# mFinn27/Template-Matching-and-Regression-MapReduce

Measured on AMD Instinct MI355X. Metric: images/sec (whole node) match+regress+NMS; % HBM/MFMA roofline at 1/2/4/8 GPU, higher is better.
Workload: dtype fp32; 1 GPU; config B: 64x SAM feats 256x64x64 (->128x128), 3 exemplars, templates 3x3-15x15, fp32, cls 0.1, IoU 0.5; config=B, images_per_gpu=64, exemplars=3, parallelism=dp1, decoder=split, decoder_precision=fp32

## Files before the change

include/tmr.h:

```cpp
#ifndef TMR_H_
#define TMR_H_

#include <stdint.h>

#ifdef __cplusplus
extern "C" {
#endif

#define TMR_ABI_VERSION 3

enum {
    TMR_OK = 0,
    TMR_E_INVALID = -1,
    TMR_E_HIP = -2,
    TMR_E_UNSUPPORTED = -3
};

enum { TMR_TEMPLATE_ROI_ALIGN = 0, TMR_TEMPLATE_PROTOTYPE = 1 };

typedef struct tmr_unit {
    int32_t image;
    int32_t type;
    int32_t ht, wt;
    float roi[4];
    int32_t pbox[4];
    int64_t tmpl_offset;
    int32_t row_offset;
    int32_t pad_;
} tmr_unit_t;

typedef struct tmr_peak_param {
    float thr;
    float scale_w, scale_h;
    int32_t mask;
    int32_t mode;
    int32_t pad_;
} tmr_peak_param_t;

int tmr_version(void);
const char *tmr_strerror(int rc);

enum {
    TMR_SIZE_TEMPLATE_SPLIT = 1,
    TMR_SIZE_HEADS_PARTIALS = 2,
    TMR_SIZE_XPACK = 3,
    TMR_SIZE_WPACK = 4,
    TMR_SIZE_ACC = 5,
    TMR_SIZE_NMS_WORK = 6,
    TMR_SIZE_STATS_WORK = 7,
    TMR_SIZE_GT_WORK = 8
};
int64_t tmr_size(int kind, int64_t d0, int64_t d1, int64_t d2, int64_t d3, int64_t d4, int64_t d5);

int tmr_upsample2x(const float *feat, int BC, int Hin, int Win, float *out, void *stream);

int tmr_templates(const float *f, int B, int C, int H, int W, const tmr_unit_t *units, int U,
                  int max_ht, int max_wt, float *templates, void *stream);

#define TMR_XCORR_AUTO 0
#define TMR_XCORR_VALU 1
#define TMR_XCORR_MFMA 2
typedef struct tmr_xcorr_args {
    const float *f;
    const float *templates;
    const tmr_unit_t *units;
    const int32_t *img_units;
    const float *scale;
    void *out;
    float *relu_out;
    float *work;
    float *out_absmax;
    const void *tmpl_split;
    int64_t total_rows;
    int32_t B, C, H, W;
    int32_t U, max_ht, max_wt;
    int32_t squeeze;
    int32_t algo, min_k, prec, out_bf16;
} tmr_xcorr_args_t;
int tmr_xcorr(const tmr_xcorr_args_t *args, void *stream);
#define TMR_XCORR_KERNEL_VALU 0
#define TMR_XCORR_KERNEL_ROWS15 1
#define TMR_XCORR_KERNEL_ROWS31 2
#define TMR_XCORR_KERNEL_MFMA 3
typedef struct tmr_xcorr_plan {
    int32_t kernel, band_rows, col_groups, out16;
} tmr_xcorr_plan_t;
int tmr_xcorr_plan(const tmr_xcorr_args_t *args, tmr_xcorr_plan_t *plan);
int tmr_template_split(const float *templates, const tmr_unit_t *units, int U, int C,
                       int64_t total_rows, int prec, void *out, void *stream);

int tmr_heads_reduce(const float *partials, int N, int tile_n, int U, int H, int W,
                     const float *head_bias, float *o, float *b, void *stream);

#define TMR_PREC_F16X3 0
#define TMR_PREC_BF16 1
#define TMR_PREC_F16 2
int tmr_absmax_rows(const float *x, int S, int64_t n, int accumulate, float *out, void *stream);
int tmr_scale_merge(const float *img_max, const float *unit_max, const int32_t *unit_image, int B, int U,
                    float *out_img, float *out_unit, void *stream);
#define TMR_XPACK_UPSAMPLE 1
#define TMR_XPACK_ONES 2
int tmr_split_xpack(const float *x, int S, int C, int H, int W, int up, int ks, int prec,
                    const float *xmax, int xmax_per_sample, void *out, void *stream);
int tmr_split_xpack16(const void *x, int S, int C, int H, int W, int ks, int prec, void *out,
                      void *stream);
int tmr_split_fold_proj(const float *wd, int N, int Cw, int Cp, int ks, const float *proj_w,
                        const float *proj_b, int Cin, float *out, void *stream);
int tmr_split_wpack(const float *w, int N, int C0, int C1, int ks, int prec, const float *wmax,
                    void *out, void *stream);
#define TMR_SPLIT_TILED_OUT 1
#define TMR_SPLIT_TILED_INIT 2
#define TMR_SPLIT_INIT_BCAST 4
#define TMR_SPLIT_OUT_BF16 8
#define TMR_SPLIT_INIT_BF16 16
#define TMR_SPLIT_XMAX_PER_UNIT 32
#define TMR_SPLIT_XMAX_PER_PIXEL 64
#define TMR_SPLIT_UNITS_PER_IMAGE_SHIFT 8
#define TMR_SPLIT_TILE_FIRST_SHIFT 16
#define TMR_SPLIT_TILE_COUNT_SHIFT 24
#define TMR_SPLIT_TILE_WINDOW(first, count) \
    (((first) << TMR_SPLIT_TILE_FIRST_SHIFT) | ((count) << TMR_SPLIT_TILE_COUNT_SHIFT))
int tmr_pixel_absmax(const float *x, int S, int C, int64_t HW, float *out, void *stream);
int tmr_split_conv(const void *xp0, int C0, const int32_t *unit_image, const void *xp1, int C1, int U,
                   int H, int W, int ks, int prec, const void *wpack, const float *wmax, const float *xmax,
                   const float *bias, int N, int leaky, const float *headw, const float *acc_init,
                   float *out, int flags, void *stream);

#define TMR_POINTS_TILE 64
int tmr_split_conv_points(const void *xp0, int C0, const int32_t *unit_image, const void *xp1, int C1, int U,
                          int H, int W, int ks, int prec, const void *wpack, const float *wmax, const float *xmax,
                          const float *bias, int N, int leaky, const float *headw, const float *head_bias,
                          const float *acc_init, const float *box, const int32_t *tiles, int ntiles, float *b,
                          int flags, void *stream);

int tmr_maxpool3x3(const float *x, int64_t planes, int H, int W, int mask9, float *out, void *stream);

#define TMR_PEAKS_PROB_SCRATCH 2
#define TMR_PEAKS_FIND_ONLY 8
#define TMR_PEAKS_DECODE_ONLY 16
int tmr_peaks_decode(const float *o, int input_is_prob, const float *reg, int U, int H, int W,
                     const tmr_peak_param_t *params, float *prob, float *logits, float *box,
                     float *ref, int32_t *counts, const void *exp_table, void *stream);

typedef struct tmr_gt_unit {
    int32_t image;
    int32_t pad_x, pad_y;
    int32_t mode;
    float scale_w, scale_h;
    int32_t pad_[2];
} tmr_gt_unit_t;
#define TMR_GT_ASSIGN 1
#define TMR_GT_LOSS 2
#define TMR_GT_GATHER 4
#define TMR_GT_ROWS 8
#define TMR_GT_SLICES 16
typedef struct tmr_gt_loss_args {
    const float *o;
    const float *reg;
    const float *boxes;
    const int32_t *box_off;
    const tmr_gt_unit_t *units;
    const void *exp_table;
    void *work;
    float *gt_map;
    int32_t *target;
    int32_t *counts;
    double *sums;
    const int64_t *samp_off;
    const int64_t *row_off;
    float *obj_out;
    float *label_out;
    float *rows_pred;
    float *rows_gt;
    double positive_threshold, negative_threshold;
    int64_t n_samples, n_rows;
    int32_t U, NI, H, W;
    int32_t G_total, min_boxes;
    int32_t last_level, focal;
    int32_t phase, pad_;
} tmr_gt_loss_args_t;
int tmr_gt_loss(const tmr_gt_loss_args_t *args, void *stream);

int tmr_nms(const float *logits, const float *box, const float *ref, const int32_t *counts,
            const int64_t *unit_off, const int32_t *seg_units, const int64_t *cand_off,
            const int64_t *nb_off,
            int G, int64_t total_cand, int64_t max_cand, int64_t sum_nb, double iou_threshold,
            float *out_logits, float *out_boxes, float *out_refs, int64_t *out_keep,
            int32_t *kept, void *work, void *stream);
#define TMR_NMS_SMALL 256
int tmr_nms_small(const float *logits, const float *box, const float *ref, const int32_t *counts,
                  const int64_t *unit_off, const int32_t *seg_units, int G, double iou_threshold,
                  float *out_logits, float *out_boxes, float *out_refs, int64_t *out_keep,
                  int32_t *kept, void *stream);

int tmr_feature_stats(const float *x, int B, int64_t n, void *work, double *out, void *stream);

int64_t tmr_exp_table_encode(const uint32_t *exc, int64_t n, uint8_t *out, int64_t cap);
int64_t tmr_exp_table_decode(const uint8_t *blob, int64_t nbytes, uint32_t *out, int64_t cap);

#ifdef __cplusplus
}
#endif
#endif
```

profiles/kernel_resources.py:

```python
import json
import os
import re
import subprocess
import sys
import tempfile

REPO = os.path.dirname(os.path.dirname(os.path.abspath(__file__)))
sys.path.insert(0, REPO)
from tmr_import import load_package

CSRC = os.path.join(REPO, "template-matching-and-regression-mapreduce_amd", "csrc")
OUT = os.path.join(REPO, "profiles", "points_kloop", "resources.json")
PRECS = {0: "F16X3", 1: "BF16", 2: "F16"}
PARENT = {
    "F16X3": {"vgprs": 256, "vgpr_spills": 146, "scratch_bytes_per_lane": 252, "occupancy": 2},
    "BF16": {"vgprs": 256, "vgpr_spills": 10, "scratch_bytes_per_lane": 44, "occupancy": 2},
    "F16": {"vgprs": 256, "vgpr_spills": 110, "scratch_bytes_per_lane": 204, "occupancy": 2},
}
FIELDS = {"VGPRs": "vgprs", "AGPRs": "agprs", "VGPRs Spill": "vgpr_spills", "SGPRs Spill": "sgpr_spills",
          "ScratchSize [bytes/lane]": "scratch_bytes_per_lane", "Occupancy [waves/SIMD]": "occupancy"}


def makefile_flags():
    var = {"EXTRA": ""}
    for line in open(os.path.join(CSRC, "Makefile")):
        m = re.match(r"^(\w+)\s*\??=\s*(.*)$", line.rstrip("\n"))
        if m and m.group(1) not in var:
            var[m.group(1)] = m.group(2)
    expand = lambda s: re.sub(r"\$\((\w+)\)", lambda m: expand(var.get(m.group(1), "")), s)
    return os.environ.get("HIPCC", expand(var["HIPCC"])), expand(var["FLAGS"]).split()


def remarks(hipcc, flags):
    with tempfile.TemporaryDirectory() as tmp:
        cmd = [hipcc, *flags, "--cuda-device-only", "-Rpass-analysis=kernel-resource-usage", "-c",
               os.path.join(CSRC, "conv_split.hip"), "-o", os.path.join(tmp, "conv_split.o")]
        return subprocess.run(cmd, check=True, capture_output=True, text=True).stderr


def parse(text):
    out, cur = {}, None
    for line in text.splitlines():
        m = re.search(r"remark: +([^:]+): (.*?) \[-Rpass-analysis", line)
        if not m:
            continue
        key, val = m.group(1).strip(), m.group(2).strip()
        if key == "Function Name":
            k = re.search(r"split_points_kernelILi3ELi(\d)EE", val)
            cur = out.setdefault(PRECS[int(k.group(1))], {}) if k else None
        elif cur is not None and key in FIELDS:
            cur[FIELDS[key]] = int(val)
    return out


def main():
    out_path = sys.argv[1] if len(sys.argv) > 1 else OUT
    hipcc, flags = makefile_flags()
    kernels = parse(remarks(hipcc, flags))
    assert sorted(kernels) == sorted(PRECS.values()), kernels
    load_package()
    from tmr_amd import buildinfo
    rec = {"kernel": "split_points_kernel<3, PREC>", "flags": flags, "source_digest": buildinfo.source_digest("heads"),
           "kernels": kernels, "parent": PARENT}
    os.makedirs(os.path.dirname(out_path), exist_ok=True)
    with open(out_path, "w") as f:
        json.dump(rec, f, indent=1)
        f.write("\n")
    for p, k in kernels.items():
        print(p, json.dumps(k))


if __name__ == "__main__":
    main()
```

profiles/points_crossover.py:

```python
import json
import os
import sys

import numpy as np
import torch

REPO = os.path.dirname(os.path.dirname(os.path.abspath(__file__)))
sys.path.insert(0, REPO)
import bench
from tmr_amd import synth

tmr = bench.tmr


def events(fn, reps=3):
    out = []
    for _ in range(reps):
        s, e = torch.cuda.Event(enable_timing=True), torch.cuda.Event(enable_timing=True)
        s.record()
        fn()
        e.record()
        e.synchronize()
        out.append(s.elapsed_time(e))
    return out


def measure(config):
    cfg = bench.CONFIGS[config]
    dev = torch.device("cuda", 0)
    H = W = 2 * cfg["hf"]
    prec = cfg.get("precision", "fp32")
    eng = tmr.TMREngine(synth.reference_state_dict(0, device=dev), tmr.PathConfig(precision=prec))
    eng.use_graphs = False
    eng.box_at_peaks = "always"
    B, E = cfg["batch"], cfg["E"]
    feats = torch.from_numpy(synth.sam_features(1000, B, bench.CIN, H // 2, W // 2)).to(dev)
    ex, _ = synth.exemplar_set(2000, B, E, H, W, cfg["kmin"], cfg["kmax"])
    eng.detect(feats, ex, cls_ths=cfg["cls"], iou_threshold=cfg["iou"])
    rec = {}
    points, dense = eng.box_at_points, eng.box_dense

    def both(box, tiles):
        rec["points_ms_all"] = events(lambda: points(box, tiles))
        rec["dense_ms_all"] = events(dense)
        rec["tiles"] = len(tiles)
        points(box, tiles)

    eng.box_at_points = both
    eng.detect(feats, ex, cls_ths=cfg["cls"], iou_threshold=cfg["iou"])
    torch.cuda.synchronize()
    assert eng.last_box_route == "points" and "tiles" in rec
    n, pixels = eng.last_points, B * E * H * W
    pm, dm = min(rec["points_ms_all"]), min(rec["dense_ms_all"])
    direct = eng.last_points_flops / (pm * 1e-3) / 1e12
    out = dict(points=n, pixels=pixels, fraction=n / pixels, tiles=rec["tiles"], points_ms=pm, dense_ms=dm,
               ns_per_point=pm * 1e6 / n, ns_per_pixel=dm * 1e6 / pixels,
               crossover=(dm / pixels) / (pm / n), points_direct_tflops=direct,
               points_executed_tflops=direct * bench.SPLIT_TERMS[prec],
               points_ms_all=rec["points_ms_all"], dense_ms_all=rec["dense_ms_all"])
    return out


def main():
    out_path = sys.argv[1]
    res = {}
    for c in sys.argv[2:] or ["B", "C", "D", "E"]:
        res[c] = measure(c)
        print(c, json.dumps({k: res[c][k] for k in ("points", "points_ms", "dense_ms", "crossover")}), flush=True)
        with open(out_path, "w") as f:
            json.dump(res, f, indent=1)
    assert all(np.isfinite(r["crossover"]) for r in res.values())


if __name__ == "__main__":
    main()
```

template-matching-and-regression-mapreduce_amd/_lib.py:

```python
from __future__ import annotations

import ctypes
import os
import threading

import numpy as np
import torch

_HERE = os.path.dirname(os.path.abspath(__file__))
LIB_PATH = os.path.join(_HERE, "libtmr.so")
if os.environ.get("TMR_LIB_VARIANT"):
    LIB_PATH = os.path.join(_HERE, "libtmr_%s.so" % os.environ["TMR_LIB_VARIANT"])
HEADER = os.path.join(os.path.dirname(_HERE), "include", "tmr.h")

_lock = threading.Lock()
_lib = None

UNIT_DTYPE = np.dtype({
    "names": ["image", "type", "ht", "wt", "roi", "pbox", "tmpl_offset", "row_offset", "pad_"],
    "formats": [np.int32, np.int32, np.int32, np.int32, (np.float32, 4), (np.int32, 4), np.int64,
                np.int32, np.int32],
    "offsets": [0, 4, 8, 12, 16, 32, 48, 56, 60],
    "itemsize": 64,
})
PEAK_DTYPE = np.dtype({
    "names": ["thr", "scale_w", "scale_h", "mask", "mode", "pad_"],
    "formats": [np.float32, np.float32, np.float32, np.int32, np.int32, np.int32],
    "offsets": [0, 4, 8, 12, 16, 20],
    "itemsize": 24,
})

GT_UNIT_DTYPE = np.dtype({
    "names": ["image", "pad_x", "pad_y", "mode", "scale_w", "scale_h", "pad_"],
    "formats": [np.int32, np.int32, np.int32, np.int32, np.float32, np.float32, (np.int32, 2)],
    "offsets": [0, 4, 8, 12, 16, 20, 24],
    "itemsize": 32,
})

TEMPLATE_ROI_ALIGN = 0
TEMPLATE_PROTOTYPE = 1

PREC_CODES = {"fp32": 0, "bf16": 1, "f16": 2}
SPLIT_TILED_OUT, SPLIT_TILED_INIT, SPLIT_INIT_BCAST = 1, 2, 4
SPLIT_OUT_BF16, SPLIT_INIT_BF16 = 8, 16
SPLIT_XMAX_PER_UNIT = 32
SPLIT_XMAX_PER_PIXEL = 64
PEAKS_PROB_SCRATCH = 2
SPLIT_UNITS_PER_IMAGE_SHIFT = 8
SPLIT_TILE_FIRST_SHIFT, SPLIT_TILE_COUNT_SHIFT = 16, 24
PEAKS_FIND_ONLY, PEAKS_DECODE_ONLY = 8, 16
POINTS_TILE = 64
XCORR_ALGOS = {"auto": 0, "valu": 1, "mfma": 2}
XPACK_UPSAMPLE, XPACK_ONES = 1, 2
SIZE_KINDS = {"template_split": 1, "heads_partials": 2, "xpack": 3, "wpack": 4, "acc": 5, "nms_work": 6,
              "stats_work": 7, "gt_work": 8}
GT_ASSIGN, GT_LOSS, GT_GATHER, GT_ROWS = 1, 2, 4, 8
GT_SLICES = 16
ABI_VERSION = 3

_P = ctypes.c_void_p
_I = ctypes.c_int
_L = ctypes.c_int64
_D = ctypes.c_double


class XcorrArgs(ctypes.Structure):
    _fields_ = [("f", _P), ("templates", _P), ("units", _P), ("img_units", _P), ("scale", _P), ("out", _P),
                ("relu_out", _P), ("work", _P), ("out_absmax", _P), ("tmpl_split", _P), ("total_rows", _L),
                ("B", ctypes.c_int32), ("C", ctypes.c_int32), ("H", ctypes.c_int32), ("W", ctypes.c_int32),
                ("U", ctypes.c_int32), ("max_ht", ctypes.c_int32), ("max_wt", ctypes.c_int32),
                ("squeeze", ctypes.c_int32), ("algo", ctypes.c_int32), ("min_k", ctypes.c_int32),
                ("prec", ctypes.c_int32), ("out_bf16", ctypes.c_int32)]


class XcorrPlan(ctypes.Structure):
    _fields_ = [("kernel", ctypes.c_int32), ("band_rows", ctypes.c_int32), ("col_groups", ctypes.c_int32),
                ("out16", ctypes.c_int32)]


XCORR_KERNELS = {0: "valu", 1: "rows15", 2: "rows31", 3: "mfma"}


class GtLossArgs(ctypes.Structure):
    _fields_ = [("o", _P), ("reg", _P), ("boxes", _P), ("box_off", _P), ("units", _P), ("exp_table", _P),
                ("work", _P), ("gt_map", _P), ("target", _P), ("counts", _P), ("sums", _P), ("samp_off", _P),
                ("row_off", _P), ("obj_out", _P), ("label_out", _P), ("rows_pred", _P), ("rows_gt", _P),
                ("positive_threshold", _D), ("negative_threshold", _D), ("n_samples", _L), ("n_rows", _L),
                ("U", ctypes.c_int32), ("NI", ctypes.c_int32), ("H", ctypes.c_int32), ("W", ctypes.c_int32),
                ("G_total", ctypes.c_int32), ("min_boxes", ctypes.c_int32), ("last_level", ctypes.c_int32),
                ("focal", ctypes.c_int32), ("phase", ctypes.c_int32), ("pad_", ctypes.c_int32)]


SIGNATURES = {
    "tmr_version": (_I, []),
    "tmr_strerror": (ctypes.c_char_p, [_I]),
    "tmr_upsample2x": (_I, [_P, _I, _I, _I, _P, _P]),
    "tmr_templates": (_I, [_P, _I, _I, _I, _I, _P, _I, _I, _I, _P, _P]),
    "tmr_size": (_L, [_I, _L, _L, _L, _L, _L, _L]),
    "tmr_xcorr": (_I, [ctypes.POINTER(XcorrArgs), _P]),
    "tmr_xcorr_plan": (_I, [ctypes.POINTER(XcorrArgs), ctypes.POINTER(XcorrPlan)]),
    "tmr_template_split": (_I, [_P, _P, _I, _I, _L, _I, _P, _P]),
    "tmr_heads_reduce": (_I, [_P, _I, _I, _I, _I, _I, _P, _P, _P, _P]),
    "tmr_absmax_rows": (_I, [_P, _I, _L, _I, _P, _P]),
    "tmr_scale_merge": (_I, [_P, _P, _P, _I, _I, _P, _P, _P]),
    "tmr_pixel_absmax": (_I, [_P, _I, _I, _L, _P, _P]),
    "tmr_split_xpack": (_I, [_P, _I, _I, _I, _I, _I, _I, _I, _P, _I, _P, _P]),
    "tmr_split_xpack16": (_I, [_P, _I, _I, _I, _I, _I, _I, _P, _P]),
    "tmr_split_fold_proj": (_I, [_P, _I, _I, _I, _I, _P, _P, _I, _P, _P]),
    "tmr_split_wpack": (_I, [_P, _I, _I, _I, _I, _I, _P, _P, _P]),
    "tmr_split_conv": (_I, [_P, _I, _P, _P, _I, _I, _I, _I, _I, _I, _P, _P, _P, _P, _I, _I, _P, _P, _P, _I,
                            _P]),
    "tmr_split_conv_points": (_I, [_P, _I, _P, _P, _I, _I, _I, _I, _I, _I, _P, _P, _P, _P, _I, _I, _P, _P, _P,
                                   _P, _P, _I, _P, _I, _P]),
    "tmr_peaks_decode": (_I, [_P, _I, _P, _I, _I, _I, _P, _P, _P, _P, _P, _P, _P, _P]),
    "tmr_maxpool3x3": (_I, [_P, _L, _I, _I, _I, _P, _P]),
    "tmr_nms": (_I, [_P, _P, _P, _P, _P, _P, _P, _P, _I, _L, _L, _L, _D, _P, _P, _P, _P, _P, _P, _P]),
    "tmr_nms_small": (_I, [_P, _P, _P, _P, _P, _P, _I, _D, _P, _P, _P, _P, _P, _P]),
    "tmr_feature_stats": (_I, [_P, _I, _L, _P, _P, _P]),
    "tmr_gt_loss": (_I, [ctypes.POINTER(GtLossArgs), _P]),
    "tmr_exp_table_encode": (_L, [_P, _L, _P, _L]),
    "tmr_exp_table_decode": (_L, [_P, _L, _P, _L]),
}


class MaskBoxesArgs(ctypes.Structure):
    _fields_ = [("masks", _P), ("logits", _P), ("iou", _P), ("scaler", _P), ("boxes", _P), ("refs", _P),
                ("logits_out", _P), ("work", _P), ("N", _L), ("h", ctypes.c_int32), ("w", ctypes.c_int32),
                ("H", ctypes.c_int32), ("W", ctypes.c_int32), ("mode", ctypes.c_int32), ("pad_", ctypes.c_int32)]


EXT_HEADER = os.path.join(os.path.dirname(_HERE), "include", "tmr_refine.h")
EXT_SIGNATURES = {
    "tmr_mask_boxes": (_I, [ctypes.POINTER(MaskBoxesArgs), _P]),
    "tmr_mask_boxes_plan": (_I, [ctypes.POINTER(MaskBoxesArgs), ctypes.POINTER(ctypes.c_int32),
                                 ctypes.POINTER(ctypes.c_int32), ctypes.POINTER(ctypes.c_int32)]),
}
REFINE_FORWARD, REFINE_SCALED = 0, 1
MASK_BOXES_WORK_PER_MASK = 16


class CocoMatchArgs(ctypes.Structure):
    _fields_ = [("det_off", _P), ("det_box", _P), ("det_area", _P), ("gt_off", _P), ("gt_box", _P),
                ("gt_area", _P), ("gt_crowd", _P), ("area_rng", _P), ("iou_thr", _P), ("dt_match", _P),
                ("dt_ignore", _P), ("gt_ignore", _P), ("gt_match", _P), ("sum_d", _L), ("sum_g", _L),
                ("I", ctypes.c_int32), ("A", ctypes.c_int32), ("T", ctypes.c_int32), ("max_d", ctypes.c_int32),
                ("max_g", ctypes.c_int32), ("pad_", ctypes.c_int32)]


class CocoMatchPlan(ctypes.Structure):
    _fields_ = [("variant", ctypes.c_int32), ("tile_cap", ctypes.c_int32), ("list_cap", ctypes.c_int32),
                ("threads", ctypes.c_int32), ("lds_bytes", ctypes.c_int32), ("blocks", ctypes.c_int32)]


COCO_HEADER = os.path.join(os.path.dirname(_HERE), "include", "tmr_coco.h")
COCO_SIGNATURES = {
    "tmr_coco_match": (_I, [ctypes.POINTER(CocoMatchArgs), _P]),
    "tmr_coco_match_plan": (_I, [ctypes.POINTER(CocoMatchArgs), ctypes.POINTER(CocoMatchPlan)]),
}
COCO_VARIANTS = {0: "lds", 1: "global"}
COCO_T_MAX, COCO_D_MAX, COCO_G_MAX = 16, 4096, 65536


class MaskHeadArgs(ctypes.Structure):
    _fields_ = [("src", _P), ("hyper", _P), ("w1", _P), ("w2", _P), ("wpack", _P), ("b1", _P), ("g", _P),
                ("beta", _P), ("b2", _P), ("masks", _P), ("N", _L), ("h", ctypes.c_int32), ("w", ctypes.c_int32),
                ("C", ctypes.c_int32), ("eps", ctypes.c_float)]


class MaskHeadPlan(ctypes.Structure):
    _fields_ = [("variant", ctypes.c_int32), ("tile_pixels", ctypes.c_int32), ("threads", ctypes.c_int32),
                ("lds_bytes", ctypes.c_int32), ("tiles", ctypes.c_int32), ("blocks", ctypes.c_int32)]


MASKHEAD_HEADER = os.path.join(os.path.dirname(_HERE), "include", "tmr_maskhead.h")
MASKHEAD_SIGNATURES = {
    "tmr_mask_head_prep": (_I, [ctypes.POINTER(MaskHeadArgs), _P]),
    "tmr_mask_head": (_I, [ctypes.POINTER(MaskHeadArgs), _P]),
    "tmr_mask_head_plan": (_I, [ctypes.POINTER(MaskHeadArgs), ctypes.POINTER(MaskHeadPlan)]),
}
MASK_HEAD_VARIANTS = {0: "mfma128"}
MASK_HEAD_WPACK_BYTES = 9 * 32768 + 64
MASK_HEAD_DIM = 256


class TwoWayPoolArgs(ctypes.Structure):
    _fields_ = [("keys", _P), ("pe", _P), ("qf", _P), ("ctx", _P), ("work", _P), ("N", _L), ("Nk", _L), ("P", _L),
                ("C", ctypes.c_int32), ("H", ctypes.c_int32), ("T", ctypes.c_int32), ("pad_", ctypes.c_int32)]


class TwoWayUpdateArgs(ctypes.Structure):
    _fields_ = [("keys_in", _P), ("pe", _P), ("A", _P), ("c", _P), ("B", _P), ("bo", _P), ("g", _P), ("beta", _P),
                ("keys_out", _P), ("N", _L), ("Nk", _L), ("P", _L), ("C", ctypes.c_int32), ("H", ctypes.c_int32),
                ("T", ctypes.c_int32), ("eps", ctypes.c_float)]


class TwoWayPlan(ctypes.Structure):
    _fields_ = [("variant", ctypes.c_int32), ("tile_pixels", ctypes.c_int32), ("chunk_pixels", ctypes.c_int32),
                ("chunks", ctypes.c_int32), ("threads", ctypes.c_int32), ("lds_bytes", ctypes.c_int32),
                ("blocks", ctypes.c_int32), ("pad_", ctypes.c_int32)]


TWOWAY_HEADER = os.path.join(os.path.dirname(_HERE), "include", "tmr_twoway.h")
TWOWAY_SIGNATURES = {
    "tmr_twoway_pool": (_I, [ctypes.POINTER(TwoWayPoolArgs), _P]),
    "tmr_twoway_update": (_I, [ctypes.POINTER(TwoWayUpdateArgs), _P]),
    "tmr_twoway_pool_plan": (_I, [ctypes.POINTER(TwoWayPoolArgs), ctypes.POINTER(TwoWayPlan)]),
    "tmr_twoway_update_plan": (_I, [ctypes.POINTER(TwoWayUpdateArgs), ctypes.POINTER(TwoWayPlan)]),
}
TWOWAY_VARIANTS = {0: "f32mfma"}
TWOWAY_DIM, TWOWAY_HEADS, TWOWAY_ROWS = 256, 8, 64
TWOWAY_POOL_CHUNK = 512


def twoway_pool_work_bytes(N: int, P: int) -> int:
    return N * ((P + TWOWAY_POOL_CHUNK - 1) // TWOWAY_POOL_CHUNK) * TWOWAY_ROWS * (TWOWAY_DIM + 2) * 4


class TMRError(RuntimeError):
    pass


def load() -> ctypes.CDLL:
    global _lib
    if _lib is not None:
        return _lib
    with _lock:
        if _lib is not None:
            return _lib
        if not os.path.exists(LIB_PATH):
            raise TMRError(
                f"libtmr.so not found at {LIB_PATH}; build it with "
                "`python -c 'import __graft_entry__ as g; g.build()'` (no CPU fallback exists)")
        lib = ctypes.CDLL(LIB_PATH)
        for name, (res, args) in (list(SIGNATURES.items()) + list(EXT_SIGNATURES.items())
                                  + list(COCO_SIGNATURES.items()) + list(MASKHEAD_SIGNATURES.items())
                                  + list(TWOWAY_SIGNATURES.items())):
            fn = getattr(lib, name)
            fn.restype = res
            fn.argtypes = args
        if lib.tmr_version() != ABI_VERSION:
            raise TMRError("libtmr.so ABI version mismatch")
        _lib = lib
        return lib


def split_tile_window(first: int, count: int) -> int:
    if not (0 <= first < 256 and 0 <= count < 128):
        raise TMRError("tile window out of range")
    return (first << SPLIT_TILE_FIRST_SHIFT) | (count << SPLIT_TILE_COUNT_SHIFT)


def split_tile_window_of(flags: int):
    return (flags >> SPLIT_TILE_FIRST_SHIFT) & 0xff, (flags >> SPLIT_TILE_COUNT_SHIFT) & 0x7f


def check(rc: int, what: str = "") -> None:
    if rc != 0:
        msg = load().tmr_strerror(rc).decode()
        raise TMRError(f"{what}: {msg} (rc={rc})" if what else msg)


def ptr(t) -> int | None:
    if t is None:
        return None
    if not t.is_cuda:
        raise TMRError("tmr_amd kernels run on the GPU only; got a CPU tensor")
    if not t.is_contiguous():
        raise TMRError("tmr_amd kernels need contiguous tensors")
    return t.data_ptr()


def stream(device=None) -> int:
    return torch.cuda.current_stream(device).cuda_stream


def call(name: str, *args) -> None:
    check(getattr(load(), name)(*args), name)


def size(kind: str, *dims) -> int:
    d = [int(x) for x in dims] + [0] * (6 - len(dims))
    n = int(load().tmr_size(SIZE_KINDS[kind], *d))
    if n < 0:
        raise TMRError(f"tmr_size({kind}, {dims}): invalid dimensions")
    return n


def _fill(struct, what: str, fields: dict):
    unknown = set(fields) - {n for n, _ in struct._fields_ if n != "pad_"}
    if unknown:
        raise TMRError(f"{what} has no field(s) {sorted(unknown)}")
    a = struct()
    for k, v in fields.items():
        if v is not None:
            setattr(a, k, v)
    return a


def xcorr(stream=None, **fields) -> None:
    check(load().tmr_xcorr(ctypes.byref(_fill(XcorrArgs, "tmr_xcorr_args_t", fields)), stream), "tmr_xcorr")


def xcorr_plan_rc(**fields):
    plan = XcorrPlan()
    fields.pop("stream", None)
    rc = load().tmr_xcorr_plan(ctypes.byref(_fill(XcorrArgs, "tmr_xcorr_args_t", fields)), ctypes.byref(plan))
    if rc != 0:
        return rc, None
    return rc, (XCORR_KERNELS[plan.kernel], plan.band_rows, plan.col_groups, plan.out16)


def xcorr_plan(**fields):
    rc, plan = xcorr_plan_rc(**fields)
    check(rc, "tmr_xcorr_plan")
    return plan


def gt_loss_args(**fields) -> GtLossArgs:
    return _fill(GtLossArgs, "tmr_gt_loss_args_t", fields)


def gt_loss(stream_=None, **fields) -> None:
    check(load().tmr_gt_loss(ctypes.byref(gt_loss_args(**fields)), stream_), "tmr_gt_loss")


def mask_boxes(stream_=None, **fields) -> None:
    check(load().tmr_mask_boxes(ctypes.byref(_fill(MaskBoxesArgs, "tmr_mask_boxes_args_t", fields)), stream_),
          "tmr_mask_boxes")


def mask_boxes_plan(**fields):
    out = [ctypes.c_int32() for _ in range(3)]
    check(load().tmr_mask_boxes_plan(ctypes.byref(_fill(MaskBoxesArgs, "tmr_mask_boxes_args_t", fields)),
                                     *(ctypes.byref(o) for o in out)), "tmr_mask_boxes_plan")
    return tuple(o.value for o in out)


def coco_match(stream_=None, **fields) -> None:
    check(load().tmr_coco_match(ctypes.byref(_fill(CocoMatchArgs, "tmr_coco_match_args_t", fields)), stream_),
          "tmr_coco_match")


def coco_match_plan_rc(**fields):
    plan = CocoMatchPlan()
    rc = load().tmr_coco_match_plan(ctypes.byref(_fill(CocoMatchArgs, "tmr_coco_match_args_t", fields)),
                                    ctypes.byref(plan))
    if rc != 0:
        return rc, None
    out = {n: getattr(plan, n) for n, _ in CocoMatchPlan._fields_}
    out["variant"] = COCO_VARIANTS[plan.variant]
    return rc, out


def coco_match_plan(**fields):
    rc, plan = coco_match_plan_rc(**fields)
    check(rc, "tmr_coco_match_plan")
    return plan


def mask_head_prep(stream_=None, **fields) -> None:
    check(load().tmr_mask_head_prep(ctypes.byref(_fill(MaskHeadArgs, "tmr_mask_head_args_t", fields)), stream_),
          "tmr_mask_head_prep")


def mask_head(stream_=None, **fields) -> None:
    check(load().tmr_mask_head(ctypes.byref(_fill(MaskHeadArgs, "tmr_mask_head_args_t", fields)), stream_),
          "tmr_mask_head")


def mask_head_plan_rc(**fields):
    plan = MaskHeadPlan()
    fields.setdefault("C", MASK_HEAD_DIM)
    rc = load().tmr_mask_head_plan(ctypes.byref(_fill(MaskHeadArgs, "tmr_mask_head_args_t", fields)),
                                   ctypes.byref(plan))
    if rc != 0:
        return rc, None
    out = {n: getattr(plan, n) for n, _ in MaskHeadPlan._fields_}
    out["variant"] = MASK_HEAD_VARIANTS[plan.variant]
    return rc, out


def mask_head_plan(**fields):
    rc, plan = mask_head_plan_rc(**fields)
    check(rc, "tmr_mask_head_plan")
    return plan


def _twoway_defaults(fields):
    fields.setdefault("C", TWOWAY_DIM)
    fields.setdefault("H", TWOWAY_HEADS)
    if "Nk" not in fields:
        fields["Nk"] = fields.get("N", 0) or 1
    return fields


def twoway_pool(stream_=None, **fields) -> None:
    a = _fill(TwoWayPoolArgs, "tmr_twoway_pool_args_t", _twoway_defaults(fields))
    check(load().tmr_twoway_pool(ctypes.byref(a), stream_), "tmr_twoway_pool")


def twoway_update(stream_=None, **fields) -> None:
    a = _fill(TwoWayUpdateArgs, "tmr_twoway_update_args_t", _twoway_defaults(fields))
    check(load().tmr_twoway_update(ctypes.byref(a), stream_), "tmr_twoway_update")


def _twoway_plan_rc(fn, struct, what, fields):
    plan = TwoWayPlan()
    rc = getattr(load(), fn)(ctypes.byref(_fill(struct, what, _twoway_defaults(fields))), ctypes.byref(plan))
    if rc != 0:
        return rc, None
    out = {n: getattr(plan, n) for n, _ in TwoWayPlan._fields_ if n != "pad_"}
    out["variant"] = TWOWAY_VARIANTS[plan.variant]
    return rc, out


def twoway_pool_plan_rc(**fields):
    return _twoway_plan_rc("tmr_twoway_pool_plan", TwoWayPoolArgs, "tmr_twoway_pool_args_t", fields)


def twoway_update_plan_rc(**fields):
    return _twoway_plan_rc("tmr_twoway_update_plan", TwoWayUpdateArgs, "tmr_twoway_update_args_t", fields)


def twoway_pool_plan(**fields):
    rc, plan = twoway_pool_plan_rc(**fields)
    check(rc, "tmr_twoway_pool_plan")
    return plan


def twoway_update_plan(**fields):
    rc, plan = twoway_update_plan_rc(**fields)
    check(rc, "tmr_twoway_update_plan")
    return plan


def require_gpu(t: torch.Tensor, name: str = "input") -> None:
    if not isinstance(t, torch.Tensor) or not t.is_cuda:
        raise TMRError(f"{name} must be a tensor on a HIP device (MI355X); no CPU path exists")
```

template-matching-and-regression-mapreduce_amd/csrc/conv_split.hip:

```cpp
#include <algorithm>
#include <type_traits>

#include "tmr_common.h"

namespace {

typedef _Float16 h8 __attribute__((ext_vector_type(8)));
typedef __bf16 b8 __attribute__((ext_vector_type(8)));
typedef float f32x4 __attribute__((ext_vector_type(4)));
typedef __bf16 b4 __attribute__((ext_vector_type(4)));
typedef __attribute__((address_space(3))) void *lds_ptr_t;


constexpr int BM = 128;
constexpr int TH = 16;
constexpr int TW = 32;
constexpr int LDS_KB = 160;
constexpr int PXG = 8, NG = 4;
constexpr int NWAVES = 8;
constexpr int NTHREADS = NWAVES * 64;
constexpr int WNS = (NWAVES == 8 || TH == 8) ? 2 : 1;
static_assert(TH == 4 * NWAVES / WNS, "a wave owns 4 output rows");
constexpr int NIN = 8 / WNS;
constexpr int ACCW = NIN * 8 * 64 * 4;
constexpr int NHEAD = 5;
constexpr int CCH = 32;
constexpr int P = 4;
constexpr int XREC = 64;
constexpr int WPL = BM * 16;

template <int PREC> struct Prec;
template <> struct Prec<TMR_PREC_F16X3> {
    static constexpr int HALVES = 2;
    static constexpr int WREC = 128;
    static constexpr bool SCALED = true;
    typedef _Float16 E;
    typedef h8 V;
};
template <> struct Prec<TMR_PREC_BF16> {
    static constexpr int HALVES = 1;
    static constexpr int WREC = 64;
    static constexpr bool SCALED = false;
    typedef __bf16 E;
    typedef b8 V;
};
template <> struct Prec<TMR_PREC_F16> {
    static constexpr int HALVES = 1;
    static constexpr int WREC = 64;
    static constexpr bool SCALED = true;
    typedef _Float16 E;
    typedef h8 V;
};

__device__ __forceinline__ float split_scale(const float *m) {
    if (!m) return 1.0f;
    const float v = *m;
    if (!(v > 0.0f && v <= 3.0e38f)) return 1.0f;
    int e;
    frexpf(v, &e);
    return ldexpf(1.0f, min(max(14 - e, -63), 63));
}

__device__ __forceinline__ void wait_vmcnt(int n) {
    switch (n) {
        case 0: asm volatile("s_waitcnt vmcnt(0)" ::: "memory"); break;
        case 1: asm volatile("s_waitcnt vmcnt(1)" ::: "memory"); break;
        case 2: asm volatile("s_waitcnt vmcnt(2)" ::: "memory"); break;
        case 3: asm volatile("s_waitcnt vmcnt(3)" ::: "memory"); break;
        case 4: asm volatile("s_waitcnt vmcnt(4)" ::: "memory"); break;
        case 5: asm volatile("s_waitcnt vmcnt(5)" ::: "memory"); break;
        case 6: asm volatile("s_waitcnt vmcnt(6)" ::: "memory"); break;
        case 7: asm volatile("s_waitcnt vmcnt(7)" ::: "memory"); break;
        case 8: asm volatile("s_waitcnt vmcnt(8)" ::: "memory"); break;
        case 9: asm volatile("s_waitcnt vmcnt(9)" ::: "memory"); break;
        case 10: asm volatile("s_waitcnt vmcnt(10)" ::: "memory"); break;
        case 11: asm volatile("s_waitcnt vmcnt(11)" ::: "memory"); break;
        default: asm volatile("s_waitcnt vmcnt(12)" ::: "memory"); break;
    }
}

__device__ __forceinline__ void buffer_lds16(__amdgpu_buffer_rsrc_t r, lds_ptr_t dst, int voff, int soff) {
    __builtin_amdgcn_raw_ptr_buffer_load_lds(r, dst, 16, voff, soff, 0, 0);
}

template <typename V>
__device__ __forceinline__ V buffer_load16(__amdgpu_buffer_rsrc_t r, uint32_t voff, uint32_t soff) {
    return __builtin_bit_cast(V, __builtin_amdgcn_raw_buffer_load_b128(r, (int)voff, (int)soff, 0));
}

__device__ __forceinline__ f32x4 mma(h8 a, h8 b, f32x4 c) {
    return __builtin_amdgcn_mfma_f32_16x16x32_f16(a, b, c, 0, 0, 0);
}
__device__ __forceinline__ f32x4 mma(b8 a, b8 b, f32x4 c) {
    return __builtin_amdgcn_mfma_f32_16x16x32_bf16(a, b, c, 0, 0, 0);
}

template <int PREC>
__device__ __forceinline__ void split_record(const float (&v)[CCH], float s,
                                             typename Prec<PREC>::V (&hi)[P],
                                             typename Prec<PREC>::V (&lo)[P]) {
    typedef typename Prec<PREC>::E E;
#pragma unroll
    for (int g = 0; g < P; ++g)
#pragma unroll
        for (int j = 0; j < 8; ++j) {
            const float xs = v[g * 8 + j] * s;
            const E h = (E)xs;
            hi[g][j] = h;
            if (Prec<PREC>::HALVES == 2) lo[g][j] = (E)(xs - (float)h);
        }
}

constexpr int WH_BITS = 8;

template <int PREC>
__device__ __forceinline__ void split_record_w(const float (&v)[CCH], float s,
                                               typename Prec<PREC>::V (&hi)[P],
                                               typename Prec<PREC>::V (&lo)[P]) {
    typedef typename Prec<PREC>::E E;
    if constexpr (Prec<PREC>::HALVES != 2 || WH_BITS >= 11) {
        split_record<PREC>(v, s, hi, lo);
    } else {
#pragma unroll
        for (int g = 0; g < P; ++g)
#pragma unroll
            for (int j = 0; j < 8; ++j) {
                const float xs = v[g * 8 + j] * s;
                const E h = (E)tmr_round_sig_bits(xs, WH_BITS);
                hi[g][j] = h;
                lo[g][j] = (E)(xs - (float)h);
            }
    }
}

struct SArgs {
    const char *x0;
    const char *x1;
    const int32_t *unit_image;
    const char *wp;
    const float *wmax, *xmax;
    const float *bias, *headw, *acc_init;
    float *out, *partials;
    int NC0, NC1, U, H, W, N, NT, MT, TXN, Hp, Wp, Npad, leaky;
    int flags;
    int EI;
    int NT0, NTW;
};

template <int PREC>
__device__ __forceinline__ float split_sxw(const SArgs &a, int u) {
    const float *xm = (a.xmax && !(a.flags & TMR_SPLIT_XMAX_PER_PIXEL))
                          ? a.xmax + ((a.flags & TMR_SPLIT_XMAX_PER_UNIT) ? u : 0) : nullptr;
    return Prec<PREC>::SCALED ? split_scale(xm) * split_scale(a.wmax) : 1.0f;
}

typedef float f2 __attribute__((ext_vector_type(2)));
__device__ __forceinline__ f2 head_act(f2 acc, f2 inv2, f2 bn2, int leaky) {
    f2 v = __builtin_elementwise_fma(acc, inv2, bn2);
    if (leaky) {
        const f2 m = v * (f2){0.01f, 0.01f};
        v = (f2){fmaxf(v.x, m.x), fmaxf(v.y, m.y)};
    }
    return v;
}
__device__ __forceinline__ void head_fma(f2 v, const f2 (&hw2)[NHEAD], f2 (&hs)[NHEAD]) {
#pragma unroll
    for (int k = 0; k < NHEAD; ++k) hs[k] = __builtin_elementwise_fma(v, hw2[k], hs[k]);
}

template <int KS, int PREC>
struct Geo {
    static constexpr int HR = TH + KS - 1, HC = TW + KS - 1;
    static constexpr int T = KS * KS;
    static constexpr int NPIX = (HR * HC + 15) / 16 * 16;
    static constexpr int HPL = NPIX * 16;
    static constexpr int NIH = (P * HPL + 1023) / 1024;
    static constexpr int MPW = (NIH + NWAVES - 1) / NWAVES;
    static constexpr int HB = MPW * NWAVES * 1024;
    static constexpr int NPLW = Prec<PREC>::WREC / 16;
    static constexpr int WB1 = NPLW * WPL;
    static constexpr bool fits(int tps, int nwb) {
        return 2 * HB + nwb * tps * WB1 <= LDS_KB * 1024;
    }
    static constexpr int TPS = T == 1 ? 1 : fits(3, 2) ? 3 : fits(2, 2) ? 2 : 1;
    static constexpr int NWB = fits(TPS, 3) ? 3 : 2;
    static constexpr int SPC = (T + TPS - 1) / TPS;
    static constexpr int WB = TPS * WB1;
    static constexpr int Q = (MPW + SPC - 1) / SPC;
    static constexpr size_t LDS = 2 * (size_t)HB + NWB * (size_t)WB;
    static constexpr bool LO3 = PREC == TMR_PREC_F16X3 && NWB == 2 && T > 1;
    static constexpr int SPCL = LO3 ? (T + 2 * TPS - 1) / (2 * TPS) : SPC;
    static constexpr int TPSL = LO3 ? (T + SPCL - 1) / SPCL : TPS;
    static constexpr int SPCC = Prec<PREC>::HALVES == 2 ? SPC + SPCL : SPC;
    static constexpr int tps(int part) { return part ? TPSL : TPS; }
    static constexpr int spc(int part) { return part ? SPCL : SPC; }
    static constexpr int wb1(int part) { return (LO3 && part) ? WB1 / 2 : WB1; }
    static constexpr int qh(int part) { return (MPW + spc(part) - 1) / spc(part); }
    static constexpr int nhp(int part, int sg) {
        return MPW - sg * qh(part) < qh(part) ? (MPW - sg * qh(part) > 0 ? MPW - sg * qh(part) : 0) : qh(part);
    }
    static constexpr int ntapp(int part, int sg) { return T - sg * tps(part) < tps(part) ? T - sg * tps(part) : tps(part); }
    static constexpr int ipt(bool lo) { return lo ? 8 : NPLW * 2; }
    static constexpr int nh(int sg) { return MPW - sg * Q < Q ? (MPW - sg * Q > 0 ? MPW - sg * Q : 0) : Q; }
    static constexpr bool lo_of(int sgx, int part, int halves) { return halves == 2 && ((sgx / SPC + part) & 1); }
    static constexpr int nw(int sg, int part, int halves) {
        return (T - ((sg + NWB - 1) % SPC) * TPS < TPS ? T - ((sg + NWB - 1) % SPC) * TPS : TPS) *
               ipt(lo_of(sg + NWB - 1, part, halves)) / NWAVES;
    }
    static constexpr int allowed(int sg, int part, int halves) {
        int n = 0;
        for (int j = 0; j <= NWB - 3; ++j) {
            int s = sg - j, p = part;
            if (s < 0) { s += SPC; p = halves == 2 ? part ^ 1 : part; }
            n += nh(s) + nw(s, p, halves);
        }
        if (sg == SPC - 1) {
            int last = 0;
            for (int s = 0; s < SPC; ++s)
                if (nh(s) > 0) last = s;
            int after = 0;
            for (int s = last; s < SPC; ++s) after += nw(s, part, halves);
            n = n < after ? n : after;
        }
        return n;
    }
    static_assert(fits(TPS, NWB), "LDS");
};

template <int KS, int PREC, int EPI>
__global__ __launch_bounds__(NTHREADS) void split_conv_kernel(SArgs a) {
    typedef Prec<PREC> PR;
    typedef typename PR::V V;
    typedef Geo<KS, PREC> G;
    constexpr int HC = G::HC, T = G::T, MPW = G::MPW, Q = G::Q;
    constexpr int HB = G::HB, WB = G::WB, WB1 = G::WB1, NWB = G::NWB;
    constexpr int TPS = G::TPS, SPC = G::SPC, HPL = G::HPL, NPIX = G::NPIX;
    constexpr int HALVES = PR::HALVES, WREC = PR::WREC;
    constexpr int D = NWB - 1;
    extern __shared__ __attribute__((aligned(16))) char lds[];
    char *Hs = lds;
    char *Ws = lds + 2 * HB;

    const int tid = threadIdx.x;
    const int lane = tid & 63;
    const int wave = __builtin_amdgcn_readfirstlane(tid >> 6);
    const int l16 = lane & 15, kg = lane >> 4;
    const int wn = wave % WNS, wpix = wave / WNS;

    const int nblk = gridDim.x, orig = blockIdx.x;
    const int q8 = nblk >> 3, r8 = nblk & 7, xcd = orig & 7;
    const int L = (xcd < r8 ? xcd * (q8 + 1) : r8 * (q8 + 1) + (xcd - r8) * q8) + (orig >> 3);
    int nt, mt, u;
    {
        const int per_unit = a.NTW * a.MT;
        const int ub = L / (a.EI * per_unit), rr = L - ub * a.EI * per_unit;
        u = ub * a.EI + rr % a.EI;
        const int r = rr / a.EI;
        if (a.MT % PXG == 0 && a.NTW % NG == 0) {
            const int gsz = PXG * a.NTW;
            const int pg = r / gsz, r2 = r - pg * gsz;
            const int ng = r2 / (PXG * NG), r3 = r2 - ng * (PXG * NG);
            mt = pg * PXG + r3 / NG;
            nt = ng * NG + r3 % NG;
        } else {
            nt = r % a.NTW;
            mt = r / a.NTW;
        }
        nt += a.NT0;
    }
    const int ty0 = (mt / a.TXN) * TH, tx0 = (mt % a.TXN) * TW;
    const int img = a.unit_image ? a.unit_image[u] : u;
    const int NC = a.NC0 + a.NC1;


    auto hoff = [&](int m) -> int {
        const int e = (wave + NWAVES * m) * 64 + lane;
        int q = e / NPIX, p = e % NPIX;
        if (q >= P || p >= G::HR * HC) q = p = 0;
        const int hy = p / HC, hx = p % HC;
        return ((q * a.Hp + ty0 + hy) * a.Wp + (tx0 + hx)) * 16;
    };
    const uint32_t cstride = (uint32_t)a.Hp * a.Wp * XREC;
    const int h0 = a.NC0 * HALVES, h1 = a.NC1 * HALVES;
    const __amdgpu_buffer_rsrc_t xr0 = __builtin_amdgcn_make_buffer_rsrc(
        (void *)(h0 ? a.x0 + (size_t)img * h0 * cstride : a.x1), (short)0, h0 * cstride, 0x00020000);
    const __amdgpu_buffer_rsrc_t xr1 = __builtin_amdgcn_make_buffer_rsrc(
        (void *)(h1 ? a.x1 + (size_t)u * h1 * cstride : a.x0), (short)0, h1 * cstride, 0x00020000);
    auto halo_dma1 = [&](int hc, int m) {
        const bool s0 = hc < h0;
        const uint32_t soff = (uint32_t)(s0 ? hc : hc - h0) * cstride;
        char *dst = Hs + (hc & 1) * HB;
        buffer_lds16(s0 ? xr0 : xr1, (lds_ptr_t)(dst + (wave + NWAVES * m) * 1024), hoff(m), soff);
    };
    const uint32_t tapstride = (uint32_t)NC * a.Npad * WREC;
    const __amdgpu_buffer_rsrc_t wr = __builtin_amdgcn_make_buffer_rsrc(
        (void *)a.wp, (short)0, T * tapstride, 0x00020000);
    const int wlane = lane * 16;
    const uint32_t wnt = (uint32_t)nt * BM * 16;
    auto w_src = [&](int g, int ipt, int m) -> uint32_t {
        const int hc = g / SPC, t0 = (g - hc * SPC) * TPS;
        const int c = hc / HALVES;
        const uint32_t src = (uint32_t)t0 * tapstride + (uint32_t)c * a.Npad * WREC + wnt;
        const int i = wave + NWAVES * m;
        const int tl = i / ipt, wi = i - tl * ipt;
        return src + (uint32_t)tl * tapstride + (uint32_t)(wi >> 1) * a.Npad * 16 + (wi & 1) * 64 * 16;
    };
    auto w_dst = [&](int g, int ipt, int m) -> char * {
        const int i = wave + NWAVES * m;
        const int tl = i / ipt, wi = i - tl * ipt;
        return Ws + (g % NWB) * WB + tl * WB1 + wi * 1024;
    };
    auto w_dma1 = [&](int g, int ipt, int m) {
        buffer_lds16(wr, (lds_ptr_t)w_dst(g, ipt, m), wlane, w_src(g, ipt, m));
    };
    auto w_dma3 = [&](int cx, int px, int sgx, int ipt, int m) {
        const int i = wave + NWAVES * m;
        const int tl = i / ipt, wi = i - tl * ipt;
        const uint32_t src = (uint32_t)(sgx * G::tps(px) + tl) * tapstride + (uint32_t)cx * a.Npad * WREC + wnt +
                             (uint32_t)(wi >> 1) * a.Npad * 16 + (wi & 1) * 64 * 16;
        const int gbx = cx * G::SPCC + (px ? SPC : 0) + sgx;
        char *dst = Ws + (gbx % NWB) * WB + tl * G::wb1(px) + wi * 1024;
        buffer_lds16(wr, (lds_ptr_t)dst, wlane, src);
    };

    const float sxw = split_sxw<PREC>(a, u);
    const int HW = a.H * a.W;
    f32x4 acc[NIN][8];
    const int islab = (a.flags & TMR_SPLIT_INIT_BCAST) ? 0 : img;
    const size_t tile_off = ((((size_t)islab * a.NT + nt) * a.MT + mt) * NWAVES + wave) * ACCW;
    if (a.acc_init && (a.flags & TMR_SPLIT_TILED_INIT) && (a.flags & TMR_SPLIT_INIT_BF16)) {
        const b4 *ai = reinterpret_cast<const b4 *>(a.acc_init) + tile_off / 4 + lane;
#pragma unroll
        for (int in = 0; in < NIN; ++in)
#pragma unroll
            for (int jp = 0; jp < 8; ++jp)
                acc[in][jp] = __builtin_convertvector(ai[(in * 8 + jp) * 64], f32x4) * sxw;
    } else if (a.acc_init && (a.flags & TMR_SPLIT_TILED_INIT)) {
        const f32x4 *ai = reinterpret_cast<const f32x4 *>(a.acc_init + tile_off) + lane;
#pragma unroll
        for (int in = 0; in < NIN; ++in)
#pragma unroll
            for (int jp = 0; jp < 8; ++jp) acc[in][jp] = ai[(in * 8 + jp) * 64] * sxw;
    } else if (a.acc_init) {
        const float *ai = a.acc_init + (size_t)islab * a.N * HW;
#pragma unroll
        for (int jp = 0; jp < 8; ++jp) {
            const int y = ty0 + wpix * 4 + (jp >> 1), x = tx0 + (jp & 1) * 16 + l16;
            const bool pin = y < a.H && x < a.W;
            const int pix = min(y, a.H - 1) * a.W + min(x, a.W - 1);
#pragma unroll
            for (int in = 0; in < NIN; ++in)
#pragma unroll
                for (int r = 0; r < 4; ++r) {
                    const int n = nt * BM + wn * 64 + in * 16 + 4 * kg + r;
                    const float v = ai[(size_t)min(n, a.N - 1) * HW + pix];
                    acc[in][jp][r] = (pin && n < a.N) ? v * sxw : 0.0f;
                }
        }
    } else {
#pragma unroll
        for (int in = 0; in < NIN; ++in)
#pragma unroll
            for (int jp = 0; jp < 8; ++jp)
#pragma unroll
                for (int r = 0; r < 4; ++r) acc[in][jp][r] = 0.0f;
    }

    const int aoff = kg * WPL + (wn * 64 + l16) * 16;
    const int boff = kg * HPL + (wpix * 4 * HC + l16) * 16;

    auto ipt_of = [](bool lo_) { return lo_ ? 8 : G::NPLW * 2; };
#pragma unroll
    for (int m = 0; m < MPW; ++m) halo_dma1(0, m);
#pragma unroll
    for (int g0 = 0; g0 < D; ++g0) {
        const bool lo0 = HALVES == 2 && ((g0 / SPC) & 1);
        const int nt0 = min(TPS, T - (g0 % SPC) * TPS) * ipt_of(lo0) / NWAVES;
#pragma unroll
        for (int m = 0; m < nt0; ++m) w_dma1(g0, ipt_of(lo0), m);
    }
    asm volatile("s_waitcnt vmcnt(0)" ::: "memory");
    __builtin_amdgcn_s_barrier();
    for (int c = 0; c < NC; ++c) {
        auto half_chunk = [&](auto part_c) {
            constexpr int part = decltype(part_c)::value;
            constexpr bool lo = part == 1;
            const int hc = c * HALVES + part;
            const char *hl = Hs + (hc & 1) * HB;
            auto step = [&](auto sg_c) {
                constexpr int sg = decltype(sg_c)::value;
                constexpr bool L3 = G::LO3;
                constexpr int TPSx = L3 ? G::tps(part) : TPS;
                const int g = L3 ? c * G::SPCC + (part ? SPC : 0) + sg : hc * SPC + sg;
                constexpr bool lastx = sg + 1 >= G::spc(part);
                constexpr int pn = lastx ? 1 - part : part, sgn = lastx ? 0 : sg + 1;
                constexpr int nh = L3 ? G::nhp(part, sg) : G::nh(sg);
                constexpr bool loD = L3 ? pn == 1 : G::lo_of(sg + D, part, HALVES);
                constexpr int nw = L3 ? G::ntapp(pn, sgn) * G::ipt(pn == 1) / NWAVES : G::nw(sg, part, HALVES);
                constexpr int NSLOT = nh + nw;
                auto dma_slot = [&](int k) {
                    if constexpr (L3) {
                        if (k < nh)
                            halo_dma1(hc + 1, sg * G::qh(part) + k);
                        else
                            w_dma3(lastx && part == 1 ? c + 1 : c, pn, sgn, ipt_of(loD), k - nh);
                    } else {
                        if (k < nh)
                            halo_dma1(hc + 1, sg * Q + k);
                        else
                            w_dma1(g + D, ipt_of(loD), k - nh);
                    }
                };
                const char *wl = Ws + (g % NWB) * WB;
                constexpr int NA = (HALVES == 2 && !lo) ? 2 * NIN : NIN;
                constexpr int DB = NA >= 8 ? 1 : 2;
                constexpr int APG = NA >= 8 ? NA / 8 : 1;
                constexpr int NB = DB + 1;
                constexpr int ntap = L3 ? G::ntapp(part, sg) : (T - sg * TPS < TPS ? T - sg * TPS : TPS);
                constexpr int WB1x = L3 ? G::wb1(part) : WB1;
                auto afrag = [&](int tl, int i) -> V {
                    return *reinterpret_cast<const V *>(wl + tl * WB1x + (i / NIN) * 4 * WPL + aoff +
                                                        (i % NIN) * 256);
                };
                auto bfrag = [&](int tap, int jp) -> V {
                    const int ky = tap / KS, kx = tap % KS;
                    return *reinterpret_cast<const V *>(
                        hl + boff + (((jp >> 1) + ky) * HC + kx + (jp & 1) * 16) * 16);
                };
                V aw[2][NA];
                V bx[NB];
#pragma unroll
                for (int i = 0; i < NA; ++i) aw[0][i] = afrag(0, i);
#pragma unroll
                for (int d = 0; d < DB; ++d) bx[d] = bfrag(sg * TPSx, d);
                __builtin_amdgcn_sched_group_barrier(0x100, NA + DB, 0);
#pragma unroll
                for (int tl = 0; tl < TPSx; ++tl) {
                    if (tl >= ntap) break;
                    const int tap = sg * TPSx + tl;
                    const bool more = tl + 1 < ntap;
#pragma unroll
                    for (int jp = 0; jp < 8; ++jp) {
                        const int q = tl * 8 + jp, qn = q + DB;
                        const bool rb = jp + DB < 8 || more;
                        if (rb) bx[qn % NB] = jp + DB < 8 ? bfrag(tap, jp + DB) : bfrag(tap + 1, jp + DB - 8);
                        const int na = (more && jp * APG < NA) ? APG : 0;
#pragma unroll
                        for (int j = 0; j < APG; ++j)
                            if (j < na) aw[(tl + 1) & 1][jp * APG + j] = afrag(tl + 1, jp * APG + j);
                        const int k = q - 1;
                        const bool dm = k >= 0 && k < NSLOT;
                        if (dm) dma_slot(k);
                        const V b = bx[q % NB];
#pragma unroll
                        for (int i = 0; i < NA; ++i)
                            acc[i % NIN][jp] = mma(aw[tl & 1][i], b, acc[i % NIN][jp]);
                        const int nr = (rb ? 1 : 0) + na;
                        if (nr == 3)
                            __builtin_amdgcn_sched_group_barrier(0x100, 3, 0);
                        else if (nr == 2)
                            __builtin_amdgcn_sched_group_barrier(0x100, 2, 0);
                        else if (nr == 1)
                            __builtin_amdgcn_sched_group_barrier(0x100, 1, 0);
                        if (dm) __builtin_amdgcn_sched_group_barrier(0x020, 1, 0);
                        __builtin_amdgcn_sched_group_barrier(0x008, NA, 0);
                    }
                }
#pragma unroll
                for (int k = 0; k < 16; ++k)
                    if (k >= ntap * 8 - 1 && k < NSLOT) dma_slot(k);
                __builtin_amdgcn_sched_barrier(0);
                if constexpr (D == 1)
                    asm volatile("s_waitcnt vmcnt(0)" ::: "memory");
                else
                    wait_vmcnt(G::allowed(sg, part, HALVES));
                __builtin_amdgcn_s_barrier();
            };
            [&]<int... SG>(std::integer_sequence<int, SG...>) {
                (step(std::integral_constant<int, SG>{}), ...);
            }(std::make_integer_sequence<int, G::LO3 ? G::spc(part) : SPC>{});
        };
        half_chunk(std::integral_constant<int, 0>{});
        if constexpr (HALVES == 2) half_chunk(std::integral_constant<int, 1>{});
    }
    asm volatile("s_waitcnt vmcnt(0)" ::: "memory");

    const float inv = 1.0f / sxw;
    if (EPI == 0 && (a.flags & TMR_SPLIT_TILED_OUT) && (a.flags & TMR_SPLIT_OUT_BF16)) {
        b4 *o = reinterpret_cast<b4 *>(a.out) + ((((size_t)u * a.NT + nt) * a.MT + mt) * NWAVES + wave) * ACCW / 4 +
                lane;
#pragma unroll
        for (int in = 0; in < NIN; ++in)
#pragma unroll
            for (int jp = 0; jp < 8; ++jp)
                __builtin_nontemporal_store(__builtin_convertvector(acc[in][jp] * inv, b4), o + (in * 8 + jp) * 64);
        return;
    }
    if (EPI == 0 && (a.flags & TMR_SPLIT_TILED_OUT)) {
        f32x4 *o = reinterpret_cast<f32x4 *>(
                       a.out + ((((size_t)u * a.NT + nt) * a.MT + mt) * NWAVES + wave) * ACCW) +
                   lane;
#pragma unroll
        for (int in = 0; in < NIN; ++in)
#pragma unroll
            for (int jp = 0; jp < 8; ++jp) {
                __builtin_nontemporal_store(acc[in][jp] * inv, o + (in * 8 + jp) * 64);
            }
        return;
    }
    float *red = reinterpret_cast<float *>(lds);
    float *sb = red + 4 * 8 * NHEAD * 16;
    float *shw = sb + BM;
    if (tid < BM) {
        const int n = nt * BM + tid;
        sb[tid] = n < a.N ? a.bias[n] : 0.0f;
    }
    if (EPI == 1)
        for (int e = tid; e < BM * NHEAD; e += NTHREADS) shw[e] = a.headw[(size_t)nt * BM * NHEAD + e];
    __syncthreads();
    if constexpr (EPI == 0) {
        float invp[8];
#pragma unroll
        for (int jp = 0; jp < 8; ++jp) {
            invp[jp] = inv;
            const int y = ty0 + wpix * 4 + (jp >> 1), x = tx0 + (jp & 1) * 16 + l16;
            if (PR::SCALED && (a.flags & TMR_SPLIT_XMAX_PER_PIXEL) && y < a.H && x < a.W)
                invp[jp] = 1.0f / (split_scale(a.xmax + ((size_t)u * a.H + y) * a.W + x) * split_scale(a.wmax));
        }
#pragma unroll
        for (int in = 0; in < NIN; ++in)
#pragma unroll
            for (int r = 0; r < 4; ++r) {
                const int nl = wn * 64 + in * 16 + 4 * kg + r;
                const int n = nt * BM + nl;
                const bool nin = n < a.N;
                const float bn = sb[nl];
#pragma unroll
                for (int jp = 0; jp < 8; ++jp) {
                    const int y = ty0 + wpix * 4 + (jp >> 1), x = tx0 + (jp & 1) * 16 + l16;
                    float v = acc[in][jp][r] * invp[jp] + bn;
                    if (a.leaky) v = v >= 0.0f ? v : v * 0.01f;
                    if (nin && y < a.H && x < a.W) a.out[((size_t)u * a.N + n) * HW + (size_t)y * a.W + x] = v;
                }
            }
        return;
    }
    f2 hs2[4][NHEAD];
#pragma unroll
    for (int q = 0; q < 4; ++q)
#pragma unroll
        for (int k = 0; k < NHEAD; ++k) hs2[q][k] = (f2){0.0f, 0.0f};
    const f2 inv2 = {inv, inv};
#pragma unroll
    for (int in = 0; in < NIN; ++in)
#pragma unroll
        for (int r = 0; r < 4; ++r) {
            const int nl = wn * 64 + in * 16 + 4 * kg + r;
            const f2 bn2 = {sb[nl], sb[nl]};
            f2 hw2[NHEAD];
#pragma unroll
            for (int k = 0; k < NHEAD; ++k) hw2[k] = (f2){shw[nl * NHEAD + k], shw[nl * NHEAD + k]};
#pragma unroll
            for (int q = 0; q < 4; ++q)
                head_fma(head_act((f2){acc[in][2 * q][r], acc[in][2 * q + 1][r]}, inv2, bn2, a.leaky), hw2, hs2[q]);
            __builtin_amdgcn_sched_barrier(0);
        }
    float X[40];
#pragma unroll
    for (int q = 0; q < 4; ++q)
#pragma unroll
        for (int k = 0; k < NHEAD; ++k) {
            X[2 * (5 * q + k)] = hs2[q][k].x;
            X[2 * (5 * q + k) + 1] = hs2[q][k].y;
        }
    float Y[20], Z[10];
#pragma unroll
    for (int m = 0; m < 20; ++m) {
        const auto s = __builtin_amdgcn_permlane16_swap(__float_as_uint(X[2 * m]), __float_as_uint(X[2 * m + 1]),
                                                         false, false);
        Y[m] = __uint_as_float(s[0]) + __uint_as_float(s[1]);
    }
#pragma unroll
    for (int p = 0; p < 10; ++p) {
        const auto s = __builtin_amdgcn_permlane32_swap(__float_as_uint(Y[2 * p]), __float_as_uint(Y[2 * p + 1]),
                                                         false, false);
        Z[p] = __uint_as_float(s[0]) + __uint_as_float(s[1]);
    }
    __syncthreads();
    if (WNS == 2 && wn == 1) {
#pragma unroll
        for (int p = 0; p < 10; ++p) red[((wpix * 10 + p) * 4 + kg) * 16 + l16] = Z[p];
    }
    __syncthreads();
    if (wn == 0) {
#pragma unroll
        for (int p = 0; p < 10; ++p) {
            const int j = 4 * p + kg, m = j >> 1, q = m / NHEAD, k = m - q * NHEAD;
            const int jp = 2 * q + (j & 1);
            const int y = ty0 + wpix * 4 + (jp >> 1), x = tx0 + (jp & 1) * 16 + l16;
            const float v = Z[p] + (WNS == 2 ? red[((wpix * 10 + p) * 4 + kg) * 16 + l16] : 0.0f);
            if (y < a.H && x < a.W) a.partials[(((size_t)nt * NHEAD + k) * a.U + u) * HW + (size_t)y * a.W + x] = v;
        }
    }
}

template <int KS, int PREC, int EPI>
int launch_split(SArgs a, hipStream_t s) {
    constexpr size_t lds = Geo<KS, PREC>::LDS;
    static_assert(lds <= 160 * 1024, "LDS");
    static_assert((4 * 8 * NHEAD * 16 + BM * (NHEAD + 1)) * 4 <= lds, "epilogue scratch");
    auto kern = split_conv_kernel<KS, PREC, EPI>;
    if (tmr_set_max_lds((const void *)kern, lds) !=
        hipSuccess)
        return TMR_E_HIP;
    const int64_t blocks = (int64_t)a.NTW * a.MT * a.U;
    if (blocks <= 0) return TMR_OK;
    TMR_REQUIRE(blocks < (1ll << 31));
    hipLaunchKernelGGL(kern, dim3((unsigned)blocks), dim3(NTHREADS), lds, s, a);
    TMR_CHECK_LAUNCH();
    return TMR_OK;
}

template <int KS, int EPI>
int dispatch_prec(int prec, const SArgs &a, hipStream_t s) {
    switch (prec) {
        case TMR_PREC_F16X3: return launch_split<KS, TMR_PREC_F16X3, EPI>(a, s);
        case TMR_PREC_BF16: return launch_split<KS, TMR_PREC_BF16, EPI>(a, s);
        case TMR_PREC_F16: return launch_split<KS, TMR_PREC_F16, EPI>(a, s);
        default: return TMR_E_INVALID;
    }
}

template <int EPI>
int dispatch_ks(int ks, int prec, const SArgs &a, hipStream_t s) {
    switch (ks) {
        case 1: return dispatch_prec<1, EPI>(prec, a, s);
        case 3: return dispatch_prec<3, EPI>(prec, a, s);
        case 5: return dispatch_prec<5, EPI>(prec, a, s);
        case 7: return dispatch_prec<7, EPI>(prec, a, s);
        default: return TMR_E_INVALID;
    }
}

constexpr int PT = TMR_POINTS_TILE;
constexpr int PP = 2 * PT;
constexpr int PCG = PP / 16;
constexpr int PTW = NWAVES / WNS;
static_assert(PT == 64 && 4 * PP == NTHREADS, "points block: one store lane per head and point");
static_assert(WNS == 2 && NWAVES == 2 * P, "points block: a wave per 64-channel half; gathers dealt by (piece, half)");

__device__ __forceinline__ int lane_now() {
    int l;
    asm volatile("v_mbcnt_lo_u32_b32 %0, -1, 0\n\tv_mbcnt_hi_u32_b32 %0, -1, %0" : "=v"(l));
    return l;
}
__device__ __forceinline__ int lane_read(int v, int src) { return __builtin_amdgcn_ds_bpermute(src << 2, v); }
__device__ __forceinline__ float lane_read(float v, int src) {
    return __builtin_bit_cast(float, lane_read(__builtin_bit_cast(int, v), src));
}

struct PArgs {
    SArgs s;
    const float *head_bias;
    const float *box;
    const int32_t *tiles;
    int ntiles;
    float *b;
};

template <int KS, int PREC>
__global__ __launch_bounds__(NTHREADS) void split_points_kernel(PArgs pa) {
    typedef Prec<PREC> PR;
    typedef typename PR::V V;
    constexpr int T = KS * KS, HALVES = PR::HALVES, WREC = PR::WREC;
    constexpr int NF = NIN;
    constexpr int NS = HALVES == 2 ? 3 * T : T;
    const SArgs &a = pa.s;
    constexpr int BB = T * P * PP * 16;
    extern __shared__ __attribute__((aligned(16))) char plds[];
    char *Bs = plds;
    float(*red)[4][PP] = reinterpret_cast<float(*)[4][PP]>(plds + 2 * BB);
    float(*xch)[4][PP] = reinterpret_cast<float(*)[4][PP]>(plds + BB);
    static_assert(PTW * 4 * PP * sizeof(float) <= BB, "the odd waves' sums fit a B buffer");

    const int tid = threadIdx.x;
    const int lane = tid & 63;
    const int wave = __builtin_amdgcn_readfirstlane(tid >> 6);
    const int wh = wave & 1, wt = wave >> 1;
    const int l16 = lane & 15, kg = lane >> 4;
    const int HW = a.H * a.W;
    int tu[2], tfirst[2], tcnt[2], timg[2];
    float sxw[2];
#pragma unroll
    for (int hh = 0; hh < 2; ++hh) {
        const int64_t ti = 2 * (int64_t)blockIdx.x + hh;
        const bool have = ti < pa.ntiles;
        const int32_t *tl = pa.tiles + 3 * (have ? ti : ti - hh);
        tu[hh] = __builtin_amdgcn_readfirstlane(min(max(tl[0], 0), a.U - 1));
        tfirst[hh] = __builtin_amdgcn_readfirstlane(min(max(tl[1], 0), HW - 1));
        tcnt[hh] = __builtin_amdgcn_readfirstlane(have ? min(max(tl[2], 0), PT) : 0);
        timg[hh] = __builtin_amdgcn_readfirstlane(a.unit_image ? a.unit_image[tu[hh]] : tu[hh]);
        sxw[hh] = __builtin_bit_cast(
            float, __builtin_amdgcn_readfirstlane(__builtin_bit_cast(int, split_sxw<PREC>(a, tu[hh]))));
    }
    const int NC = a.NC0 + a.NC1, NHC = NC * HALVES;
    auto pixel = [&](int u, int first, int cnt, int p) {
        const int *pixi = reinterpret_cast<const int *>(pa.box) + 4 * (size_t)u * HW;
        return min(max(pixi[4 * (size_t)min(first + (p < cnt ? p : 0), HW - 1)], 0), HW - 1);
    };
    const int gu = wh ? tu[1] : tu[0], gfirst = wh ? tfirst[1] : tfirst[0], gcnt = wh ? tcnt[1] : tcnt[0];
    const int gimg = wh ? timg[1] : timg[0];

    const uint32_t cstride = (uint32_t)a.Hp * a.Wp * XREC;
    const int h0 = a.NC0 * HALVES, h1 = a.NC1 * HALVES;
    auto uniform_ptr = [](const char *p) {
        const uint64_t v = (uint64_t)p;
        return (const char *)((uint64_t)(uint32_t)__builtin_amdgcn_readfirstlane((int)(uint32_t)v) |
                              (uint64_t)(uint32_t)__builtin_amdgcn_readfirstlane((int)(uint32_t)(v >> 32)) << 32);
    };
    const char *xb0 = uniform_ptr(h0 ? a.x0 + (size_t)gimg * h0 * cstride : a.x1);
    const char *xb1 = uniform_ptr(h1 ? a.x1 + (size_t)gu * h1 * cstride : a.x0);
    const uint32_t tapstride = (uint32_t)NC * a.Npad * WREC;
    const __amdgpu_buffer_rsrc_t wr = __builtin_amdgcn_make_buffer_rsrc(
        (void *)a.wp, (short)0, T * tapstride, 0x00020000);
    const int gpix0 = pixel(gu, gfirst, gcnt, lane);
    uint32_t goff[KS];
#pragma unroll
    for (int i = 0; i < KS; ++i) {
        const int g = 64 * i + lane;
        const int pix = lane_read(gpix0, g / KS), y = pix / a.W;
        goff[i] = (uint32_t)(y * a.Wp + (pix - y * a.W) + g % KS) * 16;
    }
    const uint32_t qstride = (uint32_t)a.Hp * a.Wp * 16;
    auto gather = [&](int hc, bool live = true) {
        const int hcl = min(hc, NHC - 1);
        const bool s0 = hcl < h0;
        const uint32_t hs_ = (uint32_t)(s0 ? hcl : hcl - h0) * cstride + wt * qstride;
        const __amdgpu_buffer_rsrc_t xr = __builtin_amdgcn_make_buffer_rsrc(
            (void *)(s0 ? xb0 : xb1), (short)0, live ? (s0 ? h0 : h1) * cstride : 0, 0x00020000);
#pragma unroll
        for (int ky = 0; ky < KS; ++ky)
#pragma unroll
            for (int i = 0; i < KS; ++i)
                buffer_lds16(xr, (lds_ptr_t)(Bs + (hc & 1) * BB + (((ky * P + wt) * PP + wh * PT) * KS + 64 * i) * 16),
                             goff[i], hs_ + (uint32_t)(ky * a.Wp) * 16);
    };
    const int bfo = kg * (PP * KS * 16) + l16 * (KS * 16);
    auto bfrag = [&](int hc, int tap, int j) -> V {
        return *reinterpret_cast<const V *>(Bs + (hc & 1) * BB + (tap / KS) * (P * PP * KS * 16) + bfo +
                                            j * (16 * KS * 16) + (tap % KS) * 16);
    };

    const int npass = a.NTW > PTW ? 2 : 1;
    for (int pass = 0; pass < npass; ++pass) {
        const int wtile = pass * PTW + wt;
        const bool active = wtile < a.NTW;
        const int nt = a.NT0 + (active ? wtile : 0);
        const int lp = lane_now(), l16p = lp & 15, kgp = lp >> 4;
        uint32_t aoff = (uint32_t)kgp * a.Npad * 16 + ((uint32_t)nt * BM + wh * (BM / 2) + l16p) * 16;
        gather(0);

        f32x4 acc[NF][PCG];
        if (a.acc_init) {
            constexpr int HJ = PCG / 2;
            int Wd = a.W, fl = a.flags;
            asm volatile("" : "+s"(Wd), "+s"(fl));
            const int ppix[2] = {pixel(tu[0], tfirst[0], tcnt[0], lp), pixel(tu[1], tfirst[1], tcnt[1], lp)};
            auto group4 = [&](int j) {
                const int hh = j / HJ;
                const int pix = lane_read(ppix[hh], (j % HJ) * 16 + l16p);
                const int py = pix / Wd, px = pix - py * Wd;
                const int islab = (fl & TMR_SPLIT_INIT_BCAST) ? 0 : timg[hh];
                const int mt = (py / TH) * a.TXN + px / TW;
                const int wpix = (py % TH) >> 2, jp = ((py & 3) << 1) | ((px % TW) >> 4);
                static_assert(ACCW / 4 == 1 << 11 && 8 * 64 <= ACCW / 4, "the shifts below");
                const uint32_t row = (uint32_t)(mt * NWAVES + wpix * WNS + wh), in = jp * 64 + kgp * 16 + (px & 15);
                typedef uint32_t u2 __attribute__((ext_vector_type(2)));
                u2 lh = {row << 11 | in, row >> 21};
                asm volatile("" : "+v"(lh));
                return ((size_t)islab * a.NT + nt) * a.MT * NWAVES * (ACCW / 4) + __builtin_bit_cast(uint64_t, lh);
            };
            if (fl & TMR_SPLIT_INIT_BF16) {
#pragma unroll
                for (int j = 0; j < PCG; ++j) {
                    const b4 *ai = reinterpret_cast<const b4 *>(a.acc_init) + group4(j);
#pragma unroll
                    for (int f = 0; f < NF; ++f) {
                        const f2 raw = __builtin_bit_cast(f2, ai[f * 8 * 64]);
                        acc[f][j] = (f32x4){raw.x, raw.y, 0.0f, 0.0f};
                    }
                    __builtin_amdgcn_sched_barrier(0);
                }
#pragma unroll
                for (int j = 0; j < PCG; ++j)
#pragma unroll
                    for (int f = 0; f < NF; ++f)
                        acc[f][j] = __builtin_convertvector(__builtin_bit_cast(b4, (f2){acc[f][j][0], acc[f][j][1]}),
                                                            f32x4) * sxw[j / HJ];
            } else {
#pragma unroll
                for (int j = 0; j < PCG; ++j) {
                    const f32x4 *ai = reinterpret_cast<const f32x4 *>(a.acc_init) + group4(j);
#pragma unroll
                    for (int f = 0; f < NF; ++f) acc[f][j] = ai[f * 8 * 64];
                    __builtin_amdgcn_sched_barrier(0);
                }
#pragma unroll
                for (int j = 0; j < PCG; ++j)
#pragma unroll
                    for (int f = 0; f < NF; ++f) acc[f][j] = acc[f][j] * sxw[j / HJ];
            }
        } else {
            float zf = 0.0f;
            asm volatile("" : "+v"(zf));
#pragma unroll
            for (int f = 0; f < NF; ++f)
#pragma unroll
                for (int j = 0; j < PCG; ++j) acc[f][j] = (f32x4){zf, zf, zf, zf};
        }

        auto st_part = [](int s) { return HALVES == 2 && s >= 2 * T ? 1 : 0; };
        auto st_tap = [](int s) { return HALVES == 2 ? (s >= 2 * T ? s - 2 * T : s / 2) : s; };
        auto st_term = [](int s) { return HALVES == 2 && s < 2 * T ? s & 1 : 0; };
        auto st_newb = [](int s) { return !(HALVES == 2 && s < 2 * T && (s & 1)); };
        auto st_first = [](int s) { return s == 0 || (HALVES == 2 && s == 2 * T); };
        auto st_last = [](int s) { return s == NS - 1 || (HALVES == 2 && s == 2 * T - 1); };
        constexpr int AR = 3;
        static_assert(NS % AR == 0 && NS >= AR, "weight ring");
        V ar[AR][NF];
        uint32_t ts = tapstride, npl = (uint32_t)a.Npad * 16;
        auto load_stage = [&](int c, int s) {
            if (s >= NS) {
                s -= NS;
                c = c + 1 < NC ? c + 1 : c;
            }
            const uint32_t as = (uint32_t)st_tap(s) * ts + (uint32_t)c * npl * (WREC / 16) +
                                (uint32_t)st_term(s) * 4 * npl;
#pragma unroll
            for (int f = 0; f < NF; ++f) ar[s % AR][f] = buffer_load16<V>(wr, aoff + f * 256, as);
        };
#pragma unroll
        for (int s = 0; s < AR - 1; ++s) load_stage(0, s);
        asm volatile("s_waitcnt vmcnt(0)" ::: "memory");
        __syncthreads();
        constexpr int BW = HALVES == 2 ? PCG : PCG / 2;
        static_assert(PCG % BW == 0, "a group's slot is j % BW in every stage");
        V bc[BW];
        for (int c = 0; c < NC; ++c) {
            asm volatile("" : "+v"(aoff));
            asm volatile("" : "+s"(ts), "+s"(npl));
#pragma unroll
            for (int s = 0; s < NS; ++s) {
                const int hc = c * HALVES + st_part(s);
                load_stage(c, s + AR - 1);
                if (st_first(s)) {
                    gather(hc + 1, hc + 1 < NHC);
#pragma unroll
                    for (int j = 0; j < BW; ++j) bc[j] = bfrag(hc, st_tap(s), j);
                }
                __builtin_amdgcn_sched_barrier(0);
#pragma unroll
                for (int j = 0; j < PCG; ++j) {
#pragma unroll
                    for (int f = 0; f < NF; ++f) acc[f][j] = mma(ar[s % AR][f], bc[j % BW], acc[f][j]);
                    if (j + BW < PCG) {
                        bc[j % BW] = bfrag(hc, st_tap(s), j + BW);
                        __builtin_amdgcn_sched_barrier(0);
                    } else if (!st_last(s) && (BW < PCG || st_newb(s + 1))) {
                        bc[j % BW] = bfrag(hc, st_tap(s + 1), j + BW - PCG);
                        __builtin_amdgcn_sched_barrier(0);
                    }
                }
                __builtin_amdgcn_sched_barrier(0);
                if (st_last(s)) {
                    static_assert((AR - 1) * NF == 8 && T > AR - 1, "the counted wait below");
                    asm volatile("s_waitcnt vmcnt(8)" ::: "memory");
                    __syncthreads();
                }
            }
        }

        const int le = lane_now(), kge = le >> 4, l16e = le & 15;
        float se[2] = {sxw[0], sxw[1]};
        asm volatile("" : "+s"(se[0]), "+s"(se[1]));
        f2 hs[PCG / 2][NHEAD];
#pragma unroll
        for (int q = 0; q < PCG / 2; ++q)
#pragma unroll
            for (int k = 0; k < NHEAD; ++k) hs[q][k] = (f2){0.0f, 0.0f};
        float bvs[2][4], hws[2][4][NHEAD];
        auto load_hw = [&](int f) {
#pragma unroll
            for (int r = 0; r < 4; ++r) {
                const int n = nt * BM + wh * (BM / 2) + f * 16 + 4 * kge + r;
                const float bl = a.bias[min(n, a.N - 1)];
                bvs[f & 1][r] = n < a.N ? bl : 0.0f;
#pragma unroll
                for (int k = 0; k < NHEAD; ++k) hws[f & 1][r][k] = a.headw[(size_t)n * NHEAD + k];
            }
        };
        load_hw(0);
#pragma unroll
        for (int f = 0; f < NF; ++f) {
            if (f + 1 < NF) load_hw(f + 1);
            __builtin_amdgcn_sched_barrier(0);
#pragma unroll
            for (int r = 0; r < 4; ++r) {
                const float bv = bvs[f & 1][r];
                const f2 bn2 = {bv, bv};
                f2 hw2[NHEAD];
#pragma unroll
                for (int k = 0; k < NHEAD; ++k) {
                    const float h = hws[f & 1][r][k];
                    hw2[k] = (f2){h, h};
                }
#pragma unroll
                for (int q = 0; q < PCG / 2; ++q) {
                    const float inv = 1.0f / se[q / (PCG / 4)];
                    head_fma(head_act((f2){acc[f][2 * q][r], acc[f][2 * q + 1][r]}, (f2){inv, inv}, bn2, a.leaky), hw2,
                             hs[q]);
                }
            }
            __builtin_amdgcn_sched_barrier(0);
        }
        float z[PCG / 2][4][2];
#pragma unroll
        for (int q = 0; q < PCG / 2; ++q)
#pragma unroll
            for (int k = 0; k < 4; ++k)
#pragma unroll
                for (int e = 0; e < 2; ++e) {
                    const float x = hs[q][k][e];
                    const float y = x + lane_read(x, le ^ 16);
                    z[q][k][e] = y + lane_read(y, le ^ 32);
                }
        if (wh == 1 && kge == 0 && active) {
#pragma unroll
            for (int q = 0; q < PCG / 2; ++q)
#pragma unroll
                for (int k = 0; k < 4; ++k)
#pragma unroll
                    for (int e = 0; e < 2; ++e) xch[wt][k][(2 * q + e) * 16 + l16e] = z[q][k][e];
        }
        __syncthreads();
        if (wh == 0 && kge == 0 && active) {
#pragma unroll
            for (int q = 0; q < PCG / 2; ++q)
#pragma unroll
                for (int k = 0; k < 4; ++k)
#pragma unroll
                    for (int e = 0; e < 2; ++e) {
                        const int p = (2 * q + e) * 16 + l16e;
                        red[wtile][k][p] = z[q][k][e] + xch[wt][k][p];
                    }
        }
    }
    __syncthreads();
    {
        const int te = wave * 64 + lane_now();
        const int k = te / PP, p = te % PP, pl = p % PT;
        if (pl < gcnt) {
            const int pix = pixel(gu, gfirst, gcnt, pl);
            float s = 0.0f;
            for (int t = 0; t < a.NTW; ++t) s += red[t][k][p];
            pa.b[((size_t)gu * 4 + k) * HW + pix] = s + pa.head_bias[k];
        }
    }
}

template <int PREC>
int launch_points(const PArgs &pa, int ntiles, hipStream_t s) {
    constexpr size_t lds = 2 * 9 * P * PP * 16 + NWAVES * 4 * PP * sizeof(float);
    static_assert(lds <= LDS_KB * 1024, "LDS");
    auto kern = split_points_kernel<3, PREC>;
    if (tmr_set_max_lds((const void *)kern, lds) != hipSuccess) return TMR_E_HIP;
    hipLaunchKernelGGL(kern, dim3((unsigned)((ntiles + 1) / 2)), dim3(NTHREADS), lds, s, pa);
    TMR_CHECK_LAUNCH();
    return TMR_OK;
}

inline int prec_halves(int prec) { return prec == TMR_PREC_F16X3 ? 2 : 1; }
inline int prec_wrec(int prec) { return prec == TMR_PREC_F16X3 ? 128 : 64; }
inline bool prec_ok(int prec) {
    return prec == TMR_PREC_F16X3 || prec == TMR_PREC_BF16 || prec == TMR_PREC_F16;
}
inline bool ks_ok(int ks) { return ks == 1 || ks == 3 || ks == 5 || ks == 7; }
inline bool tile_window(int flags, int NT, int &first, int &count) {
    first = (flags >> TMR_SPLIT_TILE_FIRST_SHIFT) & 0xff;
    count = (flags >> TMR_SPLIT_TILE_COUNT_SHIFT) & 0x7f;
    if (count == 0) {
        if (first != 0) return false;
        count = NT;
    }
    return first + count <= NT;
}
inline int pad_h(int H, int ks) { return (int)tmr_cdiv(H, TH) * TH + ks - 1; }
inline int pad_w(int W, int ks) { return (int)tmr_cdiv(W, TW) * TW + ks - 1; }

__device__ __forceinline__ void absmax_commit(float m, unsigned *out) {
    __shared__ float red[4];
    for (int o = 32; o > 0; o >>= 1) m = fmaxf(m, __shfl_xor(m, o));
    if ((threadIdx.x & 63) == 0) red[threadIdx.x >> 6] = m;
    __syncthreads();
    if (threadIdx.x == 0) atomicMax(out, __float_as_uint(fmaxf(fmaxf(red[0], red[1]), fmaxf(red[2], red[3]))));
}

__global__ __launch_bounds__(256) void absmax_rows_kernel(const float *__restrict__ x, int64_t n, int vec,
                                                          unsigned *__restrict__ out) {
    const float *xr = x + (size_t)blockIdx.y * n;
    float m = 0.0f;
    const int64_t step = (int64_t)gridDim.x * blockDim.x;
    if (vec) {
        const float4 *x4 = reinterpret_cast<const float4 *>(xr);
        for (int64_t i = (int64_t)blockIdx.x * blockDim.x + threadIdx.x; i < n / 4; i += step) {
            const float4 v = x4[i];
            m = fmaxf(m, fmaxf(fmaxf(fabsf(v.x), fabsf(v.y)), fmaxf(fabsf(v.z), fabsf(v.w))));
        }
    } else {
        for (int64_t i = (int64_t)blockIdx.x * blockDim.x + threadIdx.x; i < n; i += step)
            m = fmaxf(m, fabsf(xr[i]));
    }
    absmax_commit(m, out + blockIdx.y);
}

constexpr int PA_PIX = 64, PA_GRP = 8;
__global__ __launch_bounds__(PA_PIX * PA_GRP) void pixel_absmax_kernel(const float *__restrict__ x, int S, int C,
                                                                       int64_t HW, float *__restrict__ out) {
    __shared__ float part[PA_GRP][PA_PIX];
    const int lane = threadIdx.x & (PA_PIX - 1), grp = threadIdx.x / PA_PIX;
    const int64_t i = (int64_t)blockIdx.x * PA_PIX + lane;
    float m = 0.0f;
    if (i < (int64_t)S * HW) {
        const int64_t s = i / HW, p = i - s * HW;
        const float *xp = x + (size_t)s * C * HW + p;
#pragma unroll 8
        for (int c = grp; c < C; c += PA_GRP) m = fmaxf(m, fabsf(xp[(size_t)c * HW]));
    }
    part[grp][lane] = m;
    __syncthreads();
    if (grp == 0 && i < (int64_t)S * HW) {
#pragma unroll
        for (int g = 1; g < PA_GRP; ++g) m = fmaxf(m, part[g][lane]);
        out[i] = m;
    }
}

__global__ __launch_bounds__(256) void scale_merge_kernel(const float *__restrict__ img_max,
                                                          const float *__restrict__ unit_max,
                                                          const int32_t *__restrict__ unit_image, int U,
                                                          float *__restrict__ out_img,
                                                          float *__restrict__ out_unit) {
    __shared__ float red[4];
    const int b = blockIdx.x;
    float m = 0.0f;
    for (int u = threadIdx.x; u < U; u += blockDim.x)
        if (unit_image[u] == b) m = fmaxf(m, unit_max[u]);
    for (int o = 32; o > 0; o >>= 1) m = fmaxf(m, __shfl_xor(m, o));
    if ((threadIdx.x & 63) == 0) red[threadIdx.x >> 6] = m;
    __syncthreads();
    m = fmaxf(fmaxf(red[0], red[1]), fmaxf(red[2], red[3]));
    if (img_max) m = fmaxf(m, img_max[b]);
    if (threadIdx.x == 0 && out_img) out_img[b] = m;
    for (int u = threadIdx.x; u < U; u += blockDim.x)
        if (unit_image[u] == b) out_unit[u] = m;
}

template <int PREC, int MODE>
__global__ void xpack_kernel(const float *__restrict__ x, int S, int Cin, int Hin, int Win, int ups,
                             int ones, int H, int W, int NCc, int Hp, int Wp, int pad,
                             const float *__restrict__ xmax, int xms,
                             typename Prec<PREC>::V *__restrict__ out) {
    constexpr int HALVES = Prec<PREC>::HALVES;
    const int64_t total = (int64_t)S * NCc * Hp * Wp;
    const int64_t i = (int64_t)blockIdx.x * blockDim.x + threadIdx.x;
    if (i >= total) return;
    const int xp = (int)(i % Wp);
    int64_t r = i / Wp;
    const int yp = (int)(r % Hp);
    r /= Hp;
    const int c = (int)(r % NCc);
    const int s = (int)(r / NCc);
    const int y = yp - pad, xx = xp - pad;
    const bool in = y >= 0 && y < H && xx >= 0 && xx < W;
    const float *xm = !xmax ? nullptr
                      : xms == 2 ? (in ? xmax + ((size_t)s * H + y) * W + xx : nullptr)
                                 : xmax + (size_t)s * xms;
    const float sc = Prec<PREC>::SCALED ? split_scale(xm) : 1.0f;
    float v[CCH];
#pragma unroll
    for (int k = 0; k < CCH; ++k) {
        const int ch = c * CCH + k;
        float val = 0.0f;
        if (in) {
            if (MODE == 0) {
                if (ch < Cin) val = x[(((size_t)s * Cin + ch) * H + y) * W + xx];
            } else if (ch < Cin) {
                const float *pl = x + ((size_t)s * Cin + ch) * Hin * Win;
                val = ups ? up_value(pl, Hin, Win, y, xx) : pl[(size_t)y * Win + xx];
            } else if (ones && ch == Cin) {
                val = 1.0f;
            }
        }
        v[k] = val;
    }
    typename Prec<PREC>::V hi[P], lo[P];
    split_record<PREC>(v, sc, hi, lo);
    const size_t plane = (size_t)Hp * Wp;
    typename Prec<PREC>::V *o = out + ((size_t)s * NCc + c) * HALVES * P * plane + (size_t)yp * Wp + xp;
#pragma unroll
    for (int q = 0; q < P; ++q) o[q * plane] = hi[q];
    if (HALVES == 2) {
#pragma unroll
        for (int q = 0; q < P; ++q) o[(P + q) * plane] = lo[q];
    }
}

constexpr int XSEG = 128;
constexpr int XPACK16_RPB = 4;
template <int PREC, typename IN = float, int RPB = 1>
__global__ __launch_bounds__(256) void xpack4_kernel(const IN *__restrict__ x, int S, int Cin, int H, int W,
                                                     int NCc, int Hp, int Wp, int pad, int64_t nseg,
                                                     int64_t nbord, const float *__restrict__ xmax, int xms,
                                                     typename Prec<PREC>::V *__restrict__ out) {
    constexpr int HALVES = Prec<PREC>::HALVES;
    typedef typename Prec<PREC>::V V;
    typedef typename Prec<PREC>::E E;
    constexpr int VE = 16 / sizeof(IN);
    constexpr int LPR = CCH * XSEG / VE;
    typedef IN INV __attribute__((ext_vector_type(VE)));
    static_assert(RPB * LPR % 256 == 0 && RPB * XSEG * P % 256 == 0 && XSEG % VE == 0, "xpack4 tiling");
    __shared__ __attribute__((aligned(16))) IN tile[RPB][CCH][XSEG];
    const size_t plane = (size_t)Hp * Wp;
    const int t = threadIdx.x;
    if ((int64_t)blockIdx.x < nseg) {
        const int nsx = (W + XSEG - 1) / XSEG, nyg = (H + RPB - 1) / RPB;
        int64_t r = blockIdx.x;
        const int sx = (int)(r % nsx);
        r /= nsx;
        const int y0 = (int)(r % nyg) * RPB;
        r /= nyg;
        const int c = (int)(r % NCc);
        const int s = (int)(r / NCc);
        const int x0 = sx * XSEG, nx = min(XSEG, W - x0);
        const IN *src = x + ((size_t)s * Cin + (size_t)c * CCH) * H * W + (size_t)y0 * W + x0;
#pragma unroll
        for (int k = 0; k < RPB * LPR / 256; ++k) {
            const int e = t + 256 * k, rr = e / LPR, ch = (e % LPR) / (XSEG / VE), xv = e % (XSEG / VE);
            INV v = {};
            if (VE * xv < nx && c * CCH + ch < Cin && y0 + rr < H)
                v = *reinterpret_cast<const INV *>(src + (size_t)ch * H * W + (size_t)rr * W + VE * xv);
            *reinterpret_cast<INV *>(&tile[rr][ch][VE * xv]) = v;
        }
        __syncthreads();
        const float sc = Prec<PREC>::SCALED ? split_scale(xmax ? xmax + (size_t)s * xms : nullptr) : 1.0f;
        V *o = out + ((size_t)s * NCc + c) * HALVES * P * plane + (size_t)(y0 + pad) * Wp + x0 + pad;
#pragma unroll
        for (int k = 0; k < RPB * XSEG * P / 256; ++k) {
            const int e = t + 256 * k, rr = e / (XSEG * P), q = (e % (XSEG * P)) / XSEG, px = e % XSEG;
            if (px < nx && y0 + rr < H) {
                V hi, lo;
#pragma unroll
                for (int m = 0; m < 8; ++m) {
                    const float xs = (float)tile[rr][q * 8 + m][px] * sc;
                    const E h = (E)xs;
                    hi[m] = h;
                    if (HALVES == 2) lo[m] = (E)(xs - (float)h);
                }
                o[q * plane + (size_t)rr * Wp + px] = hi;
                if (HALVES == 2) o[(P + q) * plane + (size_t)rr * Wp + px] = lo;
            }
        }
        return;
    }
    const int64_t b0 = ((int64_t)blockIdx.x - nseg) * 256 + t;
    if (b0 >= nbord * S * NCc) return;
    const int64_t sc_i = b0 / nbord;
    int64_t b = b0 - sc_i * nbord;
    const int64_t top = (int64_t)pad * Wp, bot = (int64_t)(Hp - H - pad) * Wp;
    int yp, xp;
    if (b < top) {
        yp = (int)(b / Wp), xp = (int)(b % Wp);
    } else if ((b -= top) < bot) {
        yp = H + pad + (int)(b / Wp), xp = (int)(b % Wp);
    } else {
        b -= bot;
        const int side = Wp - W, k = (int)(b % side);
        yp = pad + (int)(b / side), xp = k < pad ? k : W + k;
    }
    V *o = out + (size_t)sc_i * HALVES * P * plane + (size_t)yp * Wp + xp;
    const V z = {};
#pragma unroll
    for (int q = 0; q < HALVES * P; ++q) o[q * plane] = z;
}

__global__ void fold_proj_kernel(const float *__restrict__ wd, int N, int Cw, int Cp, int T,
                                 const float *__restrict__ pw, const float *__restrict__ pb,
                                 int Cin, float *__restrict__ out) {
    const int64_t total = (int64_t)N * (Cin + 1) * T;
    const int64_t i = (int64_t)blockIdx.x * blockDim.x + threadIdx.x;
    if (i >= total) return;
    const int t = (int)(i % T);
    const int64_t r = i / T;
    const int c = (int)(r % (Cin + 1));
    const int n = (int)(r / (Cin + 1));
    const float *w = wd + (size_t)n * Cw * T + t;
    double acc = 0.0;
    if (c < Cin) {
        for (int k = 0; k < Cp; ++k) acc += (double)w[(size_t)k * T] * (double)pw[(size_t)k * Cin + c];
    } else {
        for (int k = 0; k < Cp; ++k) acc += (double)w[(size_t)k * T] * (double)pb[k];
    }
    out[i] = (float)acc;
}

template <int PREC>
__global__ void wpack_kernel(const float *__restrict__ w, int N, int C0, int C1, int ks, int NC0,
                             int NC, int Npad, const float *__restrict__ wmax,
                             typename Prec<PREC>::V *__restrict__ out) {
    const int T = ks * ks;
    const int64_t total = (int64_t)T * NC * Npad;
    const int64_t i = (int64_t)blockIdx.x * blockDim.x + threadIdx.x;
    if (i >= total) return;
    const int n = (int)(i % Npad);
    int64_t r = i / Npad;
    const int c = (int)(r % NC);
    const int tap = (int)(r / NC);
    const int C = C0 + C1;
    const float sc = Prec<PREC>::SCALED ? split_scale(wmax) : 1.0f;
    float v[CCH];
#pragma unroll
    for (int k = 0; k < CCH; ++k) {
        int ch;
        bool ok;
        if (c < NC0) {
            ch = c * CCH + k;
            ok = ch < C0;
        } else {
            const int c1 = (c - NC0) * CCH + k;
            ch = C0 + c1;
            ok = c1 < C1;
        }
        v[k] = (ok && n < N) ? w[((size_t)n * C + ch) * T + tap] : 0.0f;
    }
    typename Prec<PREC>::V hi[P], lo[P];
    split_record_w<PREC>(v, sc, hi, lo);
    constexpr int NP = Prec<PREC>::WREC / 16;
    typename Prec<PREC>::V *o = out + ((size_t)tap * NC + c) * NP * Npad + n;
#pragma unroll
    for (int q = 0; q < P; ++q) o[(size_t)q * Npad] = hi[q];
    if (NP == 8) {
#pragma unroll
        for (int q = 0; q < P; ++q) o[(size_t)(P + q) * Npad] = lo[q];
    }
}

int split_common(const void *xp0, int C0, const int32_t *unit_image, const void *xp1, int C1, int U,
                 int H, int W, int ks, int prec, const void *wpack, const float *wmax,
                 const float *xmax, const float *bias, int N, int leaky, const float *acc_init,
                 float *out, const float *headw, float *partials, int epi, int flags, void *stream) {
    TMR_REQUIRE(prec_ok(prec) && ks_ok(ks));
    TMR_REQUIRE(wpack && bias && U > 0 && H > 0 && W > 0 && N > 0 && C0 >= 0 && C1 >= 0);
    TMR_REQUIRE(C0 + C1 > 0 && (C0 == 0 || xp0) && (C1 == 0 || xp1));
    TMR_REQUIRE(prec == TMR_PREC_BF16 || (wmax && xmax));
    TMR_REQUIRE(!(flags & (TMR_SPLIT_OUT_BF16 | TMR_SPLIT_INIT_BF16)) || prec != TMR_PREC_F16X3);
    TMR_REQUIRE(!(flags & TMR_SPLIT_OUT_BF16) || (flags & TMR_SPLIT_TILED_OUT));
    TMR_REQUIRE(!(flags & TMR_SPLIT_INIT_BF16) || (flags & TMR_SPLIT_TILED_INIT));
    TMR_REQUIRE(!(flags & TMR_SPLIT_XMAX_PER_PIXEL) ||
                (ks == 1 && !epi && !acc_init && !(flags & (TMR_SPLIT_TILED_OUT | TMR_SPLIT_XMAX_PER_UNIT))));
    SArgs a = {};
    a.x0 = static_cast<const char *>(xp0);
    a.x1 = static_cast<const char *>(xp1);
    a.unit_image = unit_image;
    a.wp = static_cast<const char *>(wpack);
    a.wmax = prec == TMR_PREC_BF16 ? nullptr : wmax;
    a.xmax = prec == TMR_PREC_BF16 ? nullptr : xmax;
    a.bias = bias;
    a.headw = headw;
    a.acc_init = acc_init;
    a.out = out;
    a.partials = partials;
    a.NC0 = (int)tmr_cdiv(C0, CCH);
    a.NC1 = (int)tmr_cdiv(C1, CCH);
    a.U = U;
    a.H = H;
    a.W = W;
    a.N = N;
    a.NT = (int)tmr_cdiv(N, BM);
    a.Npad = a.NT * BM;
    a.TXN = (int)tmr_cdiv(W, TW);
    a.MT = a.TXN * (int)tmr_cdiv(H, TH);
    a.Hp = pad_h(H, ks);
    a.Wp = pad_w(W, ks);
    a.leaky = leaky;
    a.flags = flags & 0xff;
    a.EI = std::max(1, (flags >> TMR_SPLIT_UNITS_PER_IMAGE_SHIFT) & 0xff);
    TMR_REQUIRE(U % a.EI == 0);
    TMR_REQUIRE(tile_window(flags, a.NT, a.NT0, a.NTW));
    hipStream_t s = tmr_stream(stream);
    return epi ? dispatch_ks<1>(ks, prec, a, s) : dispatch_ks<0>(ks, prec, a, s);
}

template <int MODE>
int xpack_launch(const float *x, int S, int Cin, int Hin, int Win, int ups, int ones, int H, int W,
                 int ks, int prec, const float *xmax, int xms, void *out, void *stream) {
    const int C = Cin + (MODE == 1 && ones ? 1 : 0);
    const int NCc = (int)tmr_cdiv(C, CCH), Hp = pad_h(H, ks), Wp = pad_w(W, ks);
    const int64_t total = (int64_t)S * NCc * Hp * Wp;
    const dim3 grid((unsigned)tmr_cdiv(total, 256)), blk(256);
    hipStream_t s = tmr_stream(stream);
    if (MODE == 0 && W % 4 == 0 && prec != TMR_PREC_F16X3 && xms != 2) {
        const int64_t nseg = (int64_t)S * NCc * H * tmr_cdiv(W, XSEG), nbord = (int64_t)Hp * Wp - (int64_t)H * W;
        const dim3 g4((unsigned)(nseg + tmr_cdiv(nbord * S * NCc, 256)));
        switch (prec) {
            case TMR_PREC_BF16:
                hipLaunchKernelGGL(xpack4_kernel<TMR_PREC_BF16>, g4, blk, 0, s, x, S, Cin, H, W, NCc, Hp, Wp,
                                   ks / 2, nseg, nbord, nullptr, 0, static_cast<b8 *>(out));
                break;
            default:
                hipLaunchKernelGGL(xpack4_kernel<TMR_PREC_F16>, g4, blk, 0, s, x, S, Cin, H, W, NCc, Hp, Wp,
                                   ks / 2, nseg, nbord, xmax, xms, static_cast<h8 *>(out));
                break;
        }
        TMR_CHECK_LAUNCH();
        return TMR_OK;
    }
    switch (prec) {
        case TMR_PREC_F16X3:
            hipLaunchKernelGGL((xpack_kernel<TMR_PREC_F16X3, MODE>), grid, blk, 0, s, x, S, Cin, Hin, Win,
                               ups, ones, H, W, NCc, Hp, Wp, ks / 2, xmax, xms, static_cast<h8 *>(out));
            break;
        case TMR_PREC_BF16:
            hipLaunchKernelGGL((xpack_kernel<TMR_PREC_BF16, MODE>), grid, blk, 0, s, x, S, Cin, Hin, Win,
                               ups, ones, H, W, NCc, Hp, Wp, ks / 2, nullptr, 0, static_cast<b8 *>(out));
            break;
        default:
            hipLaunchKernelGGL((xpack_kernel<TMR_PREC_F16, MODE>), grid, blk, 0, s, x, S, Cin, Hin, Win,
                               ups, ones, H, W, NCc, Hp, Wp, ks / 2, xmax, xms, static_cast<h8 *>(out));
            break;
    }
    TMR_CHECK_LAUNCH();
    return TMR_OK;
}

}

extern "C" int tmr_absmax_rows(const float *x, int S, int64_t n, int accumulate, float *out, void *stream) {
    TMR_REQUIRE(out && S > 0 && S < 65536 && n >= 0 && (n == 0 || x));
    hipStream_t s = tmr_stream(stream);
    if (!accumulate && hipMemsetAsync(out, 0, sizeof(float) * (size_t)S, s) != hipSuccess) return TMR_E_HIP;
    if (n == 0) return TMR_OK;
    const int vec = (reinterpret_cast<uintptr_t>(x) & 15) == 0 && (n & 3) == 0;
    const int64_t per = vec ? n / 4 : n;
    const int bpr = (int)std::max<int64_t>(1, std::min<int64_t>(tmr_cdiv(per, 256 * 8), std::max(1, 2048 / S)));
    hipLaunchKernelGGL(absmax_rows_kernel, dim3(bpr, S), dim3(256), 0, s, x, n, vec,
                       reinterpret_cast<unsigned *>(out));
    TMR_CHECK_LAUNCH();
    return TMR_OK;
}

extern "C" int tmr_pixel_absmax(const float *x, int S, int C, int64_t HW, float *out, void *stream) {
    TMR_REQUIRE(x && out && S > 0 && C > 0 && HW > 0);
    const int64_t n = (int64_t)S * HW;
    TMR_REQUIRE(tmr_cdiv(n, PA_PIX) < (1LL << 31));
    hipLaunchKernelGGL(pixel_absmax_kernel, dim3((unsigned)tmr_cdiv(n, PA_PIX)), dim3(PA_PIX * PA_GRP), 0,
                       tmr_stream(stream), x, S, C, HW, out);
    TMR_CHECK_LAUNCH();
    return TMR_OK;
}

extern "C" int tmr_scale_merge(const float *img_max, const float *unit_max, const int32_t *unit_image, int B,
                               int U, float *out_img, float *out_unit, void *stream) {
    TMR_REQUIRE(unit_max && unit_image && out_unit && B > 0 && U > 0 && B < (1 << 24));
    hipLaunchKernelGGL(scale_merge_kernel, dim3(B), dim3(256), 0, tmr_stream(stream), img_max, unit_max,
                       unit_image, U, out_img, out_unit);
    TMR_CHECK_LAUNCH();
    return TMR_OK;
}

int64_t tmr_xpack_bytes(int S, int C, int H, int W, int ks, int prec) {
    if (S <= 0 || C <= 0 || H <= 0 || W <= 0 || !ks_ok(ks) || !prec_ok(prec)) return -1;
    return (int64_t)S * tmr_cdiv(C, CCH) * prec_halves(prec) * pad_h(H, ks) * pad_w(W, ks) * XREC;
}

extern "C" int tmr_split_xpack(const float *x, int S, int C, int H, int W, int up, int ks, int prec,
                               const float *xmax, int xmax_per_sample, void *out, void *stream) {
    TMR_REQUIRE(x && out && S > 0 && C > 0 && H > 0 && W > 0 && ks_ok(ks) && prec_ok(prec));
    TMR_REQUIRE((up & ~(TMR_XPACK_UPSAMPLE | TMR_XPACK_ONES)) == 0);
    TMR_REQUIRE(prec == TMR_PREC_BF16 || xmax);
    TMR_REQUIRE(xmax_per_sample >= 0 && xmax_per_sample <= 2);
    if (up == 0) return xpack_launch<0>(x, S, C, H, W, 0, 0, H, W, ks, prec, xmax, xmax_per_sample, out, stream);
    const int ups = (up & TMR_XPACK_UPSAMPLE) ? 1 : 0, ones = (up & TMR_XPACK_ONES) ? 1 : 0;
    return xpack_launch<1>(x, S, C, H, W, ups, ones, ups ? 2 * H : H, ups ? 2 * W : W, ks, prec, xmax,
                           xmax_per_sample, out, stream);
}

extern "C" int tmr_split_xpack16(const void *x, int S, int C, int H, int W, int ks, int prec, void *out,
                                 void *stream) {
    TMR_REQUIRE(x && out && S > 0 && C > 0 && H > 0 && W > 0 && ks_ok(ks) && prec == TMR_PREC_BF16);
    TMR_REQUIRE(W % 8 == 0);
    constexpr int RPB = XPACK16_RPB;
    const int NCc = (int)tmr_cdiv(C, CCH), Hp = pad_h(H, ks), Wp = pad_w(W, ks);
    const int64_t nseg = (int64_t)S * NCc * tmr_cdiv(H, RPB) * tmr_cdiv(W, XSEG);
    const int64_t nbord = (int64_t)Hp * Wp - (int64_t)H * W;
    const dim3 g4((unsigned)(nseg + tmr_cdiv(nbord * S * NCc, 256)));
    hipLaunchKernelGGL((xpack4_kernel<TMR_PREC_BF16, __bf16, RPB>), g4, dim3(256), 0, tmr_stream(stream),
                       static_cast<const __bf16 *>(x), S, C, H, W, NCc, Hp, Wp, ks / 2, nseg, nbord, nullptr, 0,
                       static_cast<b8 *>(out));
    TMR_CHECK_LAUNCH();
    return TMR_OK;
}

extern "C" int tmr_split_fold_proj(const float *wd, int N, int Cw, int Cp, int ks, const float *proj_w,
                                   const float *proj_b, int Cin, float *out, void *stream) {
    TMR_REQUIRE(wd && proj_w && proj_b && out && N > 0 && Cp > 0 && Cw >= Cp && Cin > 0 && ks > 0);
    const int64_t total = (int64_t)N * (Cin + 1) * ks * ks;
    hipLaunchKernelGGL(fold_proj_kernel, dim3((unsigned)tmr_cdiv(total, 256)), dim3(256), 0,
                       tmr_stream(stream), wd, N, Cw, Cp, ks * ks, proj_w, proj_b, Cin, out);
    TMR_CHECK_LAUNCH();
    return TMR_OK;
}

int64_t tmr_acc_floats(int U, int N, int H, int W) {
    if (U <= 0 || N <= 0 || H <= 0 || W <= 0) return -1;
    return (int64_t)U * tmr_cdiv(N, BM) * BM * tmr_cdiv(H, TH) * TH * tmr_cdiv(W, TW) * TW;
}

int64_t tmr_wpack_bytes(int N, int C0, int C1, int ks, int prec) {
    if (N <= 0 || C0 < 0 || C1 < 0 || C0 + C1 <= 0 || !ks_ok(ks) || !prec_ok(prec)) return -1;
    return (int64_t)ks * ks * (tmr_cdiv(C0, CCH) + tmr_cdiv(C1, CCH)) * tmr_cdiv(N, BM) * BM *
           prec_wrec(prec);
}

extern "C" int tmr_split_wpack(const float *w, int N, int C0, int C1, int ks, int prec,
                               const float *wmax, void *out, void *stream) {
    TMR_REQUIRE(w && out && N > 0 && C0 >= 0 && C1 >= 0 && C0 + C1 > 0 && ks_ok(ks) && prec_ok(prec));
    TMR_REQUIRE(prec == TMR_PREC_BF16 || wmax);
    const int NC0 = (int)tmr_cdiv(C0, CCH), NC = NC0 + (int)tmr_cdiv(C1, CCH);
    const int Npad = (int)tmr_cdiv(N, BM) * BM;
    const int64_t total = (int64_t)ks * ks * NC * Npad;
    const dim3 grid((unsigned)tmr_cdiv(total, 256)), blk(256);
    hipStream_t s = tmr_stream(stream);
    switch (prec) {
        case TMR_PREC_F16X3:
            hipLaunchKernelGGL(wpack_kernel<TMR_PREC_F16X3>, grid, blk, 0, s, w, N, C0, C1, ks, NC0,
                               NC, Npad, wmax, static_cast<h8 *>(out));
            break;
        case TMR_PREC_BF16:
            hipLaunchKernelGGL(wpack_kernel<TMR_PREC_BF16>, grid, blk, 0, s, w, N, C0, C1, ks, NC0,
                               NC, Npad, nullptr, static_cast<b8 *>(out));
            break;
        default:
            hipLaunchKernelGGL(wpack_kernel<TMR_PREC_F16>, grid, blk, 0, s, w, N, C0, C1, ks, NC0,
                               NC, Npad, wmax, static_cast<h8 *>(out));
            break;
    }
    TMR_CHECK_LAUNCH();
    return TMR_OK;
}

extern "C" int tmr_split_conv(const void *xp0, int C0, const int32_t *unit_image, const void *xp1, int C1, int U,
                              int H, int W, int ks, int prec, const void *wpack, const float *wmax, const float *xmax,
                              const float *bias, int N, int leaky, const float *headw, const float *acc_init,
                              float *out, int flags, void *stream) {
    TMR_REQUIRE(out);
    if (!headw)
        return split_common(xp0, C0, unit_image, xp1, C1, U, H, W, ks, prec, wpack, wmax, xmax, bias, N, leaky,
                            acc_init, out, nullptr, nullptr, 0, flags, stream);
    TMR_REQUIRE(!(flags & TMR_SPLIT_TILED_OUT));
    return split_common(xp0, C0, unit_image, xp1, C1, U, H, W, ks, prec, wpack, wmax, xmax, bias, N, leaky, acc_init,
                        nullptr, headw, out, 1, flags, stream);
}

extern "C" int tmr_split_conv_points(const void *xp0, int C0, const int32_t *unit_image, const void *xp1, int C1,
                                     int U, int H, int W, int ks, int prec, const void *wpack, const float *wmax,
                                     const float *xmax, const float *bias, int N, int leaky, const float *headw,
                                     const float *head_bias, const float *acc_init, const float *box,
                                     const int32_t *tiles, int ntiles, float *b, int flags, void *stream) {
    TMR_REQUIRE(prec_ok(prec) && ks_ok(ks));
    TMR_REQUIRE(wpack && bias && headw && head_bias && box && b && U > 0 && H > 0 && W > 0 && N > 0);
    TMR_REQUIRE(C0 >= 0 && C1 >= 0 && C0 + C1 > 0 && (C0 == 0 || xp0) && (C1 == 0 || xp1));
    TMR_REQUIRE(prec == TMR_PREC_BF16 || (wmax && xmax));
    TMR_REQUIRE(ntiles >= 0 && (ntiles == 0 || tiles));
    TMR_REQUIRE(!(flags & (TMR_SPLIT_TILED_OUT | TMR_SPLIT_OUT_BF16 | TMR_SPLIT_XMAX_PER_PIXEL)));
    TMR_REQUIRE(!acc_init || (flags & TMR_SPLIT_TILED_INIT));
    TMR_REQUIRE(!(flags & TMR_SPLIT_INIT_BF16) || ((flags & TMR_SPLIT_TILED_INIT) && prec != TMR_PREC_F16X3));
    TMR_REQUIRE((int64_t)H * W < (1ll << 29));
    PArgs pa = {};
    SArgs &a = pa.s;
    a.x0 = static_cast<const char *>(xp0);
    a.x1 = static_cast<const char *>(xp1);
    a.unit_image = unit_image;
    a.wp = static_cast<const char *>(wpack);
    a.wmax = prec == TMR_PREC_BF16 ? nullptr : wmax;
    a.xmax = prec == TMR_PREC_BF16 ? nullptr : xmax;
    a.bias = bias;
    a.headw = headw;
    a.acc_init = acc_init;
    a.NC0 = (int)tmr_cdiv(C0, CCH);
    a.NC1 = (int)tmr_cdiv(C1, CCH);
    a.U = U;
    a.H = H;
    a.W = W;
    a.N = N;
    a.NT = (int)tmr_cdiv(N, BM);
    a.Npad = a.NT * BM;
    a.TXN = (int)tmr_cdiv(W, TW);
    a.MT = a.TXN * (int)tmr_cdiv(H, TH);
    a.Hp = pad_h(H, ks);
    a.Wp = pad_w(W, ks);
    a.leaky = leaky;
    a.flags = flags & 0xff;
    a.EI = 1;
    TMR_REQUIRE(tile_window(flags, a.NT, a.NT0, a.NTW));
    if (ks != 3 || a.NTW > 2 * PTW) return TMR_E_UNSUPPORTED;
    pa.head_bias = head_bias;
    pa.box = box;
    pa.tiles = tiles;
    pa.ntiles = ntiles;
    pa.b = b;
    if (ntiles == 0) return TMR_OK;
    hipStream_t s = tmr_stream(stream);
    switch (prec) {
        case TMR_PREC_F16X3: return launch_points<TMR_PREC_F16X3>(pa, ntiles, s);
        case TMR_PREC_BF16: return launch_points<TMR_PREC_BF16>(pa, ntiles, s);
        default: return launch_points<TMR_PREC_F16>(pa, ntiles, s);
    }
}
```

template-matching-and-regression-mapreduce_amd/decoder_plan.py:

```python
from __future__ import annotations

import os
from dataclasses import dataclass
from typing import Optional, Tuple

import numpy as np
import torch

from ._lib import (SPLIT_INIT_BCAST, SPLIT_INIT_BF16, SPLIT_OUT_BF16, SPLIT_TILED_INIT, SPLIT_TILED_OUT,
                   SPLIT_UNITS_PER_IMAGE_SHIFT, SPLIT_XMAX_PER_UNIT, call, ptr, split_tile_window, stream)

HEADS_IMAGE_MAJOR_MAX = min(255, int(os.environ.get("TMR_HEADS_IMAGE_MAJOR_MAX", "4")))

SCALES_OWN = "own"
SCALES_MERGED = "merged"
SCALES_FTM = "ftm"


def units_per_image(unit_image, B: int) -> int:
    U = len(unit_image)
    E = U // max(B, 1)
    if E <= 1 or E > HEADS_IMAGE_MAJOR_MAX or E * B != U:
        return 1
    ui = np.asarray(unit_image)
    return E if np.array_equal(ui, np.repeat(np.arange(B), E)) else 1


@dataclass(frozen=True)
class DecoderPlan:
    fold: bool
    share: bool
    acc16: bool
    unscaled: bool
    scales: str
    fp_flags: int
    init_flags: int
    epi: int
    skip_tiles: int

    def window(self, ntiles: int) -> Tuple[int, int]:
        return (self.skip_tiles, ntiles - self.skip_tiles) if self.skip_tiles else (0, 0)

    def heads_flags(self, first: int = 0, count: int = 0) -> int:
        return self.init_flags | self.epi | split_tile_window(first, count)

    def points_flags(self) -> int:
        return self.init_flags | split_tile_window(0, self.skip_tiles)


def decoder_plan(cfg, fold_proj: bool, share_fp_half: bool, reuse_image_work: bool, have_feats: bool, U: int,
                 B: int, unit_image, box_later: bool = False, nbt: int = 0) -> DecoderPlan:
    fold = bool(cfg.fusion and fold_proj and have_feats)
    share = bool(share_fp_half and cfg.fusion and (U >= 2 * B or (reuse_image_work and fold)))
    bf16 = cfg.precision == "bf16"
    acc16 = share and bf16
    xpu = 0 if bf16 else SPLIT_XMAX_PER_UNIT
    plane = (SPLIT_TILED_INIT | SPLIT_INIT_BCAST | (SPLIT_INIT_BF16 if bf16 else 0)) if fold else 0
    if share:
        fp_flags = SPLIT_TILED_OUT | (SPLIT_OUT_BF16 if acc16 else 0) | xpu | plane
        init = SPLIT_TILED_INIT | (SPLIT_INIT_BF16 if acc16 else 0)
    else:
        fp_flags, init = 0, plane
    return DecoderPlan(fold, share, acc16, bf16, SCALES_OWN if share else SCALES_MERGED if cfg.fusion else SCALES_FTM,
                       fp_flags, init | xpu, units_per_image(unit_image, B) << SPLIT_UNITS_PER_IMAGE_SHIFT,
                       nbt if box_later else 0)


@dataclass
class HeadsLaunch:
    xp0: Optional[torch.Tensor]
    C0: int
    ui: torch.Tensor
    xp1: torch.Tensor
    C1: int
    U: int
    H: int
    W: int
    ks: int
    pc: int
    wp: tuple
    xmax1: Optional[torch.Tensor]
    bias: torch.Tensor
    N: int
    hw: torch.Tensor
    hb: torch.Tensor
    a0: Optional[torch.Tensor]
    part: torch.Tensor
    plan: DecoderPlan
    b: Optional[torch.Tensor] = None

    def _conv_args(self):
        return (ptr(self.xp0) if self.C0 else None, self.C0, ptr(self.ui), ptr(self.xp1), self.C1, self.U, self.H,
                self.W, self.ks, self.pc, ptr(self.wp[0]), ptr(self.wp[1]), ptr(self.xmax1), ptr(self.bias), self.N,
                1, ptr(self.hw))

    def run(self, first: int = 0, count: int = 0) -> None:
        call("tmr_split_conv", *self._conv_args(), ptr(self.a0), ptr(self.part),
             self.plan.heads_flags(first, count), stream())

    def run_points(self, box: torch.Tensor, tiles: torch.Tensor, ntiles: int) -> None:
        call("tmr_split_conv_points", *self._conv_args(), ptr(self.hb), ptr(self.a0), ptr(box), ptr(tiles), ntiles,
             ptr(self.b), self.plan.points_flags(), stream())
```

template-matching-and-regression-mapreduce_amd/engine.py:

```python
from __future__ import annotations

import contextlib
import weakref
from dataclasses import dataclass
from typing import Dict, Optional, Sequence, Tuple

import numpy as np
import torch

from . import exp_table, graphs, host
from ._lib import (PEAKS_DECODE_ONLY, PEAKS_FIND_ONLY, PEAKS_PROB_SCRATCH, POINTS_TILE, PREC_CODES, SPLIT_OUT_BF16,
                   SPLIT_TILED_OUT, SPLIT_XMAX_PER_PIXEL, UNIT_DTYPE, XCORR_ALGOS, TMRError, call, ptr, require_gpu,
                   size, stream, xcorr)
from .decoder_plan import SCALES_FTM, SCALES_MERGED, HeadsLaunch, decoder_plan
from .graphs import _clone_outputs, _GraphBook, _h2d, _units_to_device
from .operands import absmax
from .operands import (absmax_rows, conv2d_split, fold_proj, pack_split_up, pack_split_w, pack_split_x, pixel_absmax,
                       prec_code, scale_merge)
from .xcorr_cost import mfma_fits, xcorr_choice

NHEAD = 5
NMS_SMALL = 256


@dataclass
class PathConfig:
    emb_dim: int = 512
    fusion: bool = True
    squeeze: bool = False
    box_reg: bool = True
    template_type: str = "roi_align"
    feature_upsample: bool = True
    decoder_num_layer: int = 1
    decoder_kernel_size: int = 3
    no_matcher: bool = False
    precision: str = "fp32"

    @classmethod
    def from_args(cls, args) -> "PathConfig":
        return cls(emb_dim=args.emb_dim, fusion=bool(args.fusion), squeeze=bool(args.squeeze),
                   box_reg=not args.ablation_no_box_regression, template_type=args.template_type,
                   feature_upsample=bool(args.feature_upsample),
                   decoder_num_layer=args.decoder_num_layer,
                   decoder_kernel_size=args.decoder_kernel_size, no_matcher=bool(args.no_matcher),
                   precision=getattr(args, "precision", "fp32"))


@contextlib.contextmanager
def _timed(events: Optional[list]):
    if events is None:
        yield
        return
    ev = (torch.cuda.Event(enable_timing=True), torch.cuda.Event(enable_timing=True))
    ev[0].record()
    yield
    ev[1].record()
    events.append(ev)


def _version_key(ts: Sequence[torch.Tensor]):
    return tuple((t.data_ptr(), t._version, tuple(t.shape)) for t in ts)


class _PackCache:

    def __init__(self):
        self._d: Dict[str, Tuple[tuple, tuple, object]] = {}

    def get(self, name: str, tensors: Sequence[torch.Tensor], build):
        key = _version_key(tensors)
        hit = self._d.get(name)
        if hit is not None and hit[0] == key and all(r() is t for r, t in zip(hit[1], tensors)):
            return hit[2]
        val = build()
        self._d[name] = (key, tuple(weakref.ref(t) for t in tensors), val)
        return val


@dataclass
class _ImageMemo:
    feats: "weakref.ref"
    version: int
    data_ptr: int
    pkey: tuple
    params: tuple
    fp: Optional[torch.Tensor]
    split: object = None
    size: Optional[tuple] = None
    acc0: Optional[torch.Tensor] = None

    def is_for(self, feats: torch.Tensor) -> bool:
        return self.feats() is feats and self.version == feats._version and self.data_ptr == feats.data_ptr()


class TMREngine:

    def __init__(self, params: Dict[str, torch.Tensor], cfg: PathConfig):
        self.P = params
        self.cfg = cfg
        self._cache = _PackCache()
        self.decoder_events = self.xcorr_events = None
        self.xcorr_split_events = []
        self.last_xcorr_flops = self.last_xcorr_bytes = self.last_xcorr_dram_bytes = 0.0
        self.share_fp_half = True
        prec_code(cfg.precision)
        self.fold_proj = True
        self._absmax_memo: Dict[tuple, tuple] = {}
        self.xcorr_algo = "auto"
        self.last_xcorr_algo = None
        self.last_nms_small = False
        self.out_bf16 = True
        self.last_xcorr_out16 = False
        self.reuse_image_work = False
        self._memo: Optional[_ImageMemo] = None
        self._graphs = _GraphBook(self.GRAPH_CACHE)
        self._pnames = None
        self.last_graph = self.last_graph_error = self.last_decoder_algo = None
        self.last_decoder_flops = self.last_shared_flops = 0.0
        self.last_box_route = None
        self.last_points = 0
        self.last_points_flops = 0.0
        self._box_ctx: Optional[HeadsLaunch] = None
        if cfg.decoder_kernel_size not in (1, 3, 5, 7):
            raise TMRError("decoder_kernel_size must be 1, 3, 5 or 7")

    def _dec_layers(self, pre: str):
        return [(self.P[f"{pre}.layer.{2 * l}.weight"], self.P[f"{pre}.layer.{2 * l}.bias"])
                for l in range(self.cfg.decoder_num_layer)]

    def _fused_decoders(self, split_c0: int = 0, fold: bool = False):
        cfg = self.cfg
        layers = [self._dec_layers(pre)[0] for pre in (["decoder_b"] if cfg.box_reg else []) + ["decoder_o"]]
        ow, ob = self.P["objectness_head.head.0.weight"], self.P["objectness_head.head.0.bias"]
        heads = [ow, ob]
        if cfg.box_reg:
            lw, lb = self.P["ltrbs_head.head.0.weight"], self.P["ltrbs_head.head.0.bias"]
            heads += [lw, lb]
        tensors = [t for wb in layers for t in wb] + heads
        if fold:
            pw_, pb_ = self.P["input_proj.0.weight"], self.P["input_proj.0.bias"]
            tensors += [pw_, pb_]

        def build():
            W = torch.cat([w.detach().float() for w, _ in layers], 0).contiguous()
            Bv = torch.cat([b.detach().float() for _, b in layers], 0).contiguous()
            N = W.shape[0]
            npad = ((N + 127) // 128) * 128
            hw = torch.zeros((npad, NHEAD), device=W.device, dtype=torch.float32)
            hb = torch.zeros(NHEAD, device=W.device, dtype=torch.float32)
            n0 = 0
            if cfg.box_reg:
                nb = layers[0][0].shape[0]
                hw[:nb, 0:4] = lw.detach().float().reshape(4, nb).t()
                hb[0:4] = lb.detach().float()
                n0 = nb
            no = layers[-1][0].shape[0]
            hw[n0:n0 + no, 4] = ow.detach().float().reshape(no)
            hb[4] = ob.detach().float().reshape(())
            c0_full = split_c0 or (cfg.emb_dim if cfg.fusion else 0)
            W0, W1, wbias = W[:, :c0_full], W[:, c0_full:], None
            if fold:
                Wf = fold_proj(W, c0_full, pw_, pb_)
                W0, wbias = Wf[:, :-1], Wf[:, -1:].contiguous()
            c0 = W0.shape[1]
            full = split = None
            if split_c0:
                split = (pack_split_w(W0, c0, cfg.precision), pack_split_w(W1, 0, cfg.precision),
                         torch.zeros(N, device=W.device, dtype=torch.float32))
            else:
                full = pack_split_w(torch.cat([W0, W1], 1), c0, cfg.precision)
            return full, Bv, N, W.shape[1], hw.contiguous(), hb.contiguous(), split, wbias

        return self._cache.get(f"fused_dec{split_c0}_{cfg.precision}_{int(fold)}", tensors, build)

    def _bias_plane(self, wbias: torch.Tensor, H: int, W: int) -> torch.Tensor:
        N, _, ks, _ = wbias.shape
        prec = self.cfg.precision

        def build():
            dev = wbias.device
            ones = torch.ones((1, 1, H, W), device=dev, dtype=torch.float32)
            one = torch.ones(1, device=dev, dtype=torch.float32)
            xp = pack_split_x(ones, ks, prec, one)
            wp, wmax = pack_split_w(wbias, 1, prec)
            plane = torch.empty(size("acc", 1, N, H, W), device=dev, dtype=torch.float32)
            zero = torch.zeros(N, device=dev, dtype=torch.float32)
            call("tmr_split_conv", ptr(xp), 1, None, None, 0, 1, H, W, ks, prec_code(prec),
                 ptr(wp), ptr(wmax), ptr(one), ptr(zero), N, 0, None, None, ptr(plane),
                 SPLIT_TILED_OUT | (SPLIT_OUT_BF16 if prec == "bf16" else 0), stream())
            return plane

        return self._cache.get(f"bias_plane_{H}x{W}_{prec}", [wbias], build)

    def _conv(self, name: str, x: torch.Tensor, w: torch.Tensor, b: torch.Tensor, leaky: bool):
        prec = self.cfg.precision
        wp = self._cache.get(f"{name}_split_{prec}", [w], lambda: pack_split_w(w, w.shape[1], prec))
        return conv2d_split(x, w, b, leaky, prec, wp)

    def _feat_absmax(self, feats: torch.Tensor) -> torch.Tensor:
        if self.cfg.precision == "bf16":
            return None
        return self._memo_absmax(feats, "feat", lambda: absmax_rows(feats))

    def _memo_absmax(self, t: torch.Tensor, tag: str, compute):
        key = (t.data_ptr(), tag)
        hit = self._absmax_memo.get(key)
        if hit is not None and hit[0]() is t and hit[1] == t._version:
            return hit[2]
        val = compute()
        self._absmax_memo[key] = (weakref.ref(t), t._version, val)
        return val

    def project(self, feats: torch.Tensor, want_f0: bool = False):
        require_gpu(feats, "features")
        feats = feats.float().contiguous()
        B, Cin, Hin, Win = feats.shape
        self._absmax_memo = {}
        up = self.cfg.feature_upsample
        H, W = (2 * Hin, 2 * Win) if up else (Hin, Win)
        pprec = "bf16" if self.cfg.precision == "bf16" else "fp32"
        pcode = prec_code(pprec)
        pw, pb = self.P["input_proj.0.weight"], self.P["input_proj.0.bias"]
        N, Cw = pw.shape[0], pw.shape[1]
        if Cw != Cin:
            raise TMRError(f"input_proj expects {Cw} channels, got {Cin}")
        wp, wmax = self._cache.get(f"proj_split_{pprec}", [pw], lambda: pack_split_w(pw, Cin, pprec))
        xmax = None if pprec == "bf16" else pixel_absmax(feats)
        if xmax is not None and self.cfg.precision != "bf16":
            self._memo_absmax(feats, "feat", lambda: absmax_rows(xmax))
        xp = pack_split_up(feats, False, 1, pprec, xmax, ones=False)
        fq = torch.empty((B, N, Hin, Win), device=feats.device, dtype=torch.float32)
        call("tmr_split_conv", ptr(xp), Cin, None, None, 0, B, Hin, Win, 1, pcode, ptr(wp),
             ptr(wmax), ptr(xmax), ptr(pb.detach().float().contiguous()), N, 0, None, None, ptr(fq),
             SPLIT_XMAX_PER_PIXEL if xmax is not None else 0, stream())
        if up:
            fp = torch.empty((B, N, H, W), device=feats.device, dtype=torch.float32)
            call("tmr_upsample2x", ptr(fq), B * N, Hin, Win, ptr(fp), stream())
        else:
            fp = fq
        return fp, (self._f0(feats) if want_f0 else None)

    def _f0(self, feats: torch.Tensor) -> torch.Tensor:
        if not self.cfg.feature_upsample:
            return feats
        B, Cin, Hin, Win = feats.shape
        f0 = torch.empty((B, Cin, 2 * Hin, 2 * Win), device=feats.device, dtype=torch.float32)
        call("tmr_upsample2x", ptr(feats.float().contiguous()), B * Cin, Hin, Win, ptr(f0), stream())
        return f0

    def match(self, fp: torch.Tensor, unit_image: Sequence[int], unit_boxes: np.ndarray,
              want_relu: bool = False, allow_bf16: bool = False):
        B, C, H, W = fp.shape
        U = len(unit_image)
        cfg = self.cfg
        units, tfl, mh, mw = host.build_units(unit_boxes, unit_image, H, W, C, cfg.template_type)
        dev = fp.device
        units_d = _units_to_device(units, dev, tag="units")
        img_units = host.image_ranges(unit_image, B)
        img_units_d = _h2d(np.asarray(img_units), dev, tag="img_units")
        tmpl = torch.empty(max(tfl, 1), device=dev, dtype=torch.float32)
        call("tmr_templates", ptr(fp), B, C, H, W, ptr(units_d), U, mh, mw, ptr(tmpl), stream())
        Co = 1 if cfg.squeeze else C
        work = torch.empty((U, C, H, W), device=dev, dtype=torch.float32) if cfg.squeeze else None
        scale = self.P["matcher.scale"].detach().float().contiguous()
        slots = torch.zeros(U, device=dev, dtype=torch.float32)
        min_k = int(min(units["ht"].min(), units["wt"].min()))
        pc = prec_code(cfg.precision)
        choice = self.xcorr_algo
        if choice == "auto":
            choice = xcorr_choice(units["ht"], units["wt"], U / max(1, len(set(unit_image))),
                                  mfma_fits(W, mh, mw), one_term=pc != PREC_CODES["fp32"])
        self.last_xcorr_algo = choice
        algo = XCORR_ALGOS[choice]
        out16 = (allow_bf16 and self.out_bf16 and pc == PREC_CODES["bf16"] and algo == XCORR_ALGOS["mfma"]
                 and not cfg.squeeze and not want_relu and W % 8 == 0)
        self.last_xcorr_out16 = out16
        out = torch.empty((U, Co, H, W), device=dev, dtype=torch.bfloat16 if out16 else torch.float32)
        relu = torch.empty_like(out) if want_relu else None
        tsplit, rows = None, 0
        if algo != XCORR_ALGOS["valu"] and tfl > 0:
            rows = host.tsplit_rows(units)
            tsplit = torch.empty(size("template_split", U, C, rows), device=dev, dtype=torch.uint8)
            with _timed(self.xcorr_split_events if self.xcorr_events is not None else None):
                call("tmr_template_split", ptr(tmpl), ptr(units_d), U, C, rows, pc, ptr(tsplit), stream())
        with _timed(self.xcorr_events):
            xcorr(f=ptr(fp), templates=ptr(tmpl), units=ptr(units_d), img_units=ptr(img_units_d), scale=ptr(scale),
                  out=ptr(out), relu_out=ptr(relu), work=ptr(work), out_absmax=ptr(slots), tmpl_split=ptr(tsplit),
                  total_rows=rows, B=B, C=C, H=H, W=W, U=U, max_ht=mh, max_wt=mw, squeeze=int(cfg.squeeze),
                  algo=algo, min_k=min_k, prec=pc, out_bf16=int(out16), stream=stream())
        ht, wt = units["ht"].astype(np.float64), units["wt"].astype(np.float64)
        self.last_xcorr_flops = float(np.sum(2.0 * C * (H - ht + 1) * (W - wt + 1) * ht * wt))
        self.last_xcorr_bytes = 2.0 * 4 * C * H * W * U
        nimg = len(set(int(i) for i in unit_image))
        self.last_xcorr_dram_bytes = float(C * H * W) * (4.0 * nimg + (2.0 if out16 else 4.0) * U)
        self._memo_absmax(out, "ftm", lambda: slots)
        return out, relu

    def decode(self, fp: torch.Tensor, f_tm: torch.Tensor, unit_image: Sequence[int],
               feats: Optional[torch.Tensor] = None, box_later: bool = False):
        cfg = self.cfg
        ui = _h2d(np.asarray(unit_image, np.int32), f_tm.device, tag="unit_image")
        if cfg.decoder_num_layer != 1:
            return self._decode_stack(fp, f_tm, ui)
        U, C1, H, W = f_tm.shape
        B, dev = fp.shape[0], f_tm.device
        ks, prec, pc = cfg.decoder_kernel_size, cfg.precision, prec_code(cfg.precision)
        p = decoder_plan(cfg, self.fold_proj, self.share_fp_half, self.reuse_image_work, feats is not None, U, B,
                         unit_image, box_later, self._box_tiles() if box_later else 0)
        Cfp = fp.shape[1] if cfg.fusion else 0
        wp, bias, N, Cw, hw, hb, split, wbias = self._fused_decoders(Cfp if p.share else 0, p.fold)
        if Cw != Cfp + C1:
            raise TMRError(f"decoders expect {Cw} input channels, got {Cfp + C1}")
        C0 = feats.shape[1] if p.fold else Cfp
        bplane = self._bias_plane(wbias, H, W) if p.fold else None
        xmax1 = None if p.unscaled else self._memo_absmax(f_tm, "ftm", lambda: absmax_rows(f_tm))
        xp0 = xmax0 = acc0 = None
        if p.scales != SCALES_FTM:
            xmax0 = None if p.unscaled else self._feat_absmax(feats) if p.fold else absmax_rows(fp)
            if p.scales == SCALES_MERGED and not p.unscaled:
                xmax0, xmax1 = scale_merge(xmax0, xmax1, ui, B)
            if p.share and p.fold:
                acc0 = self._acc0_lookup(feats, split, H, W)
            if acc0 is None:
                xp0 = pack_split_up(feats, cfg.feature_upsample, ks, prec, xmax0, ones=False) if p.fold else \
                    pack_split_x(fp, ks, prec, xmax0)
        xp1 = pack_split_x(f_tm, ks, prec, xmax1)
        if p.share:
            wp_fp, wp, zero_b = split
            if acc0 is None:
                acc0 = torch.empty(size("acc", B, N, H, W), device=dev, dtype=torch.float32)
                call("tmr_split_conv", ptr(xp0), C0, None, None, 0, B, H, W, ks, pc, ptr(wp_fp[0]), ptr(wp_fp[1]),
                     ptr(xmax0), ptr(zero_b), N, 0, None, ptr(bplane), ptr(acc0), p.fp_flags, stream())
                if p.fold and self.reuse_image_work:
                    self._acc0_store(feats, split, H, W, acc0)
        part = torch.empty(size("heads_partials", N, U, H, W), device=dev, dtype=torch.float32)
        heads = HeadsLaunch(xp0=None if p.share else xp0, C0=0 if p.share else C0, ui=ui, xp1=xp1, C1=C1, U=U, H=H, W=W,
                            ks=ks, pc=pc, wp=wp, xmax1=xmax1, bias=bias, N=N, hw=hw, hb=hb,
                            a0=acc0 if p.share else bplane, part=part, plan=p)
        first, count = p.window((N + 127) // 128)
        with _timed(self.decoder_events):
            heads.run(first, count)
        n_run = 128 * count if box_later else N
        self.last_decoder_flops = 2.0 * H * W * n_run * (heads.C0 + C1) * ks ** 2 * U
        self.last_shared_flops = 2.0 * H * W * N * C0 * ks ** 2 * B if p.share else 0.0
        self.last_decoder_algo = "split"
        ob = torch.empty(U * (5 if cfg.box_reg else 1) * H * W, device=dev, dtype=torch.float32)
        o = ob[:U * H * W].view(U, 1, H, W)
        b = ob[U * H * W:].view(U, 4, H, W) if cfg.box_reg else None
        call("tmr_heads_reduce", ptr(part[first * NHEAD * U * H * W:]), n_run, 128, U, H, W, ptr(hb), ptr(o),
             None if box_later else ptr(b), stream())
        if box_later:
            heads.b = b
            self._box_ctx = heads
        return o, b

    def _decode_stack(self, fp, f_tm, ui):
        cfg = self.cfg
        x0 = torch.cat([fp.index_select(0, ui.long()), f_tm], 1) if cfg.fusion else f_tm
        res = {}
        for pre in (["decoder_b"] if cfg.box_reg else []) + ["decoder_o"]:
            x = x0
            for l, (w, bb) in enumerate(self._dec_layers(pre)):
                x = self._conv(f"{pre}.{l}", x, w, bb, True)
            res[pre] = x
        ow, ob = self.P["objectness_head.head.0.weight"], self.P["objectness_head.head.0.bias"]
        o = self._conv("obj", res["decoder_o"], ow, ob, False)
        b = None
        if cfg.box_reg:
            lw, lb = self.P["ltrbs_head.head.0.weight"], self.P["ltrbs_head.head.0.bias"]
            b = self._conv("ltrbs", res["decoder_b"], lw, lb, False)
        return o, b

    box_at_peaks = "auto"
    BOX_POINTS_CROSSOVER = {"fp32": 0.57, "bf16": 0.47, "f16": 0.47}

    def _box_tiles(self) -> int:
        return int(self.P["decoder_b.layer.0.weight"].shape[0]) // 128

    def box_at_peaks_ok(self) -> bool:
        cfg = self.cfg
        if self.box_at_peaks == "never" or cfg.decoder_num_layer != 1 or not cfg.box_reg or \
                cfg.decoder_kernel_size != 3 or self.reuse_image_work:
            return False
        if self.box_at_peaks not in ("auto", "always"):
            raise TMRError("box_at_peaks must be 'auto', 'always' or 'never'")
        nb = int(self.P["decoder_b.layer.0.weight"].shape[0])
        return nb % 128 == 0 and 1 <= nb // 128 <= 8

    def box_at_points(self, box: torch.Tensor, tiles: np.ndarray) -> None:
        if len(tiles):
            td = _h2d(np.ascontiguousarray(tiles, np.int32).reshape(-1), box.device)
            self._box_ctx.run_points(box, td, len(tiles))

    def box_dense(self) -> None:
        h = self._box_ctx
        nbt = h.plan.skip_tiles
        h.run(0, nbt)
        scratch_o = torch.empty(h.U * h.H * h.W, device=h.b.device, dtype=torch.float32)
        call("tmr_heads_reduce", ptr(h.part), 128 * nbt, 128, h.U, h.H, h.W, ptr(h.hb), ptr(scratch_o), ptr(h.b),
             stream())

    def _detect_box_at_peaks(self, feats, unit_image, boxes, params):
        r = self._forward_units_eager(feats, [int(i) for i in unit_image], boxes, box_later=True)
        o, b = r["o"], r["b"]
        U, _, H, W = o.shape
        logits, box, ref, counts, _ = self.peaks(o, None, params, want_prob=False, phase="find")
        counts_host = counts.cpu().numpy()
        need = np.where(params["mode"] != 2, counts_host, 0)
        self.last_points = int(need.sum())
        dense = self.box_at_peaks == "auto" and \
            self.last_points > self.BOX_POINTS_CROSSOVER[self.cfg.precision] * U * H * W
        self.last_box_route = "dense" if dense else "points"
        if dense:
            self.box_dense()
            self.last_points_flops = 0.0
        else:
            tiles = host.point_tiles(need, POINTS_TILE)
            self.box_at_points(box, tiles)
            h = self._box_ctx
            self.last_points_flops = 2.0 * 128 * h.plan.skip_tiles * (h.C0 + h.C1) * h.ks ** 2 * POINTS_TILE * len(tiles)
        self._box_ctx = None
        self.peaks(o, b, params, want_prob=False, phase="decode", found=(logits, box, ref, counts))
        return logits, box, ref, counts, counts_host

    def _proj_key(self):
        params = (self.P["input_proj.0.weight"], self.P["input_proj.0.bias"])
        return params, (_version_key(params), self.cfg.precision, self.cfg.feature_upsample)

    def _bind_memo(self, feats: torch.Tensor, fp, split=None, size_=None, acc0=None):
        params, pkey = self._proj_key()
        self._memo = _ImageMemo(weakref.ref(feats), feats._version, feats.data_ptr(), pkey,
                                tuple(weakref.ref(t) for t in params), fp, split, size_, acc0)

    def _fp_lookup(self, feats: torch.Tensor):
        m = self._memo
        params, pkey = self._proj_key()
        hit = m is not None and m.is_for(feats) and m.fp is not None and m.pkey == pkey and \
            all(r() is t for r, t in zip(m.params, params))
        return m.fp if hit else None

    def _acc0_lookup(self, feats, split, H, W):
        m = self._memo
        hit = self.reuse_image_work and m is not None and m.is_for(feats) and m.split is split and m.size == (H, W)
        return m.acc0 if hit else None

    def _acc0_store(self, feats, split, H, W, acc0):
        m = self._memo
        if m is not None and m.is_for(feats):
            m.split, m.size, m.acc0 = split, (H, W), acc0
        else:
            self._bind_memo(feats, None, split, (H, W), acc0)

    def _memo_hit(self, feats: torch.Tensor) -> Optional[_ImageMemo]:
        return self._memo if self._fp_lookup(feats) is not None and self._memo.acc0 is not None else None

    def _forward_units_graphed(self, feats, unit_image, unit_boxes, want_aux):
        if not (self.use_graphs and feats.is_cuda and len(unit_image) <= self.GRAPH_MAX_UNITS) or \
                self.decoder_events is not None or self.xcorr_events is not None or self.cfg.no_matcher or \
                self.cfg.decoder_num_layer != 1 or not (self.cfg.fusion and self.fold_proj):
            return None
        B, Cin, Hin, Win = feats.shape
        H, W = (2 * Hin, 2 * Win) if self.cfg.feature_upsample else (Hin, Win)
        C = int(self.P["input_proj.0.weight"].shape[0])
        boxes = np.asarray(unit_boxes, np.float32).reshape(-1, 4)
        units = host.build_units(boxes, unit_image, H, W, C, self.cfg.template_type)[0]
        hit = self._memo_hit(feats)
        base = self._graph_signature(feats, units, unit_image, False, False, module=True)
        if base is None:
            return None
        sig = base + (bool(want_aux), None if hit is None else (hit.fp.data_ptr(), hit.acc0.data_ptr()))
        g = self._graphs.get(sig)
        self.last_graph = "replay" if g is not None else "eager"
        if g is None:
            if not self._graphs.want_capture(sig):
                return None
            g = self._capture_module(feats, unit_image, boxes, want_aux, hit, self._detect_host_inputs(
                units, unit_image, B, np.zeros(0, np.uint8)))
            self._graphs.put(sig, g)
            if g is None:
                return None
            self.last_graph = "captured"
        host_in = self._detect_host_inputs(units, unit_image, B, np.zeros(0, np.uint8))
        out = g.replay(self, feats.float().contiguous(), host_in, reuse_feats=True)
        if hit is None:
            m = g.memo
            self._bind_memo(feats, m.fp, m.split, m.size, m.acc0)
        return _clone_outputs(out)

    def _capture_module(self, feats, unit_image, boxes, want_aux, hit, host_in):
        saved = self._memo

        def run(static):
            if hit is not None:
                self._bind_memo(static, hit.fp, hit.split, hit.size, hit.acc0)
            else:
                self._memo = None
            return self._forward_units_eager(static, unit_image, boxes, want_aux)

        try:
            g = graphs.capture(self, feats, host_in, run)
            if g is not None and hit is None:
                g.memo = self._memo
                if g.memo is None or g.memo.acc0 is None:
                    self.last_graph_error, g = "the image's first call kept no fp half: the signature stays eager", None
        finally:
            self._memo = saved
        return g

    def forward_units(self, feats: torch.Tensor, unit_image: Sequence[int], unit_boxes,
                      want_aux: bool = False):
        unit_image = [int(i) for i in unit_image]
        if self.reuse_image_work and not graphs.capturing():
            r = self._forward_units_graphed(feats, unit_image, unit_boxes, want_aux)
            if r is not None:
                return r
        return self._forward_units_eager(feats, unit_image, unit_boxes, want_aux)

    def _forward_units_eager(self, feats: torch.Tensor, unit_image: Sequence[int], unit_boxes,
                             want_aux: bool = False, box_later: bool = False):
        fp = self._fp_lookup(feats) if self.reuse_image_work else None
        if fp is not None:
            f0 = self._f0(feats) if want_aux else None
        else:
            fp, f0 = self.project(feats, want_f0=want_aux)
            if self.reuse_image_work:
                m = self._memo
                self._bind_memo(feats, fp, *((m.split, m.size, m.acc0) if m is not None and m.is_for(feats) else ()))
        if self.cfg.no_matcher:
            ui = _h2d(np.asarray(unit_image, np.int64), fp.device, tag="unit_image64")
            f_tm = fp.index_select(0, ui).contiguous()
            relu = torch.relu(f_tm) if want_aux else None
        else:
            split1 = self.cfg.decoder_num_layer == 1
            f_tm, relu = self.match(fp, unit_image, np.asarray(unit_boxes, np.float32), want_aux,
                                    allow_bf16=split1 and not want_aux)
        o, b = self.decode(fp, f_tm, unit_image, feats, box_later=box_later)
        return dict(o=o, b=b, f_tm_relu=relu, f0=f0, fp=fp)

    exp_mode = "reference"

    @staticmethod
    def peaks(o: torch.Tensor, b: Optional[torch.Tensor], params: np.ndarray,
              input_is_prob: bool = False, want_prob: bool = True, phase: Optional[str] = None,
              found=None):
        require_gpu(o, "objectness")
        o = o.float().contiguous()
        U = o.shape[0]
        H, W = o.shape[-2:]
        dev = o.device
        cap = H * W
        prm = _h2d(params.view(np.uint8), dev, tag="peak_params")
        bb = b.float().contiguous() if b is not None else None
        tab = exp_table.device_table(dev) if TMREngine.exp_mode == "reference" else None
        flags = int(input_is_prob) | (0 if want_prob else PEAKS_PROB_SCRATCH)
        if phase == "decode":
            (logits, box, ref, counts), prob, want_prob = found, o, False
            flags |= PEAKS_DECODE_ONLY
        else:
            prob = torch.empty((U, H, W), device=dev, dtype=torch.float32)
            logits = torch.empty((U * cap, 2), device=dev, dtype=torch.float32)
            box = torch.empty((U * cap, 4), device=dev, dtype=torch.float32)
            ref = torch.empty((U * cap, 2), device=dev, dtype=torch.float32)
            counts = torch.empty(U, device=dev, dtype=torch.int32)
            if phase == "find":
                flags |= PEAKS_FIND_ONLY
        call("tmr_peaks_decode", ptr(o), flags, ptr(bb), U, H, W, ptr(prm), ptr(prob), ptr(logits), ptr(box),
             ptr(ref), ptr(counts), ptr(tab), stream())
        return logits, box, ref, counts, (prob if want_prob else None)

    @staticmethod
    def eval_loss(o, b, unit_image: Sequence[int], unit_boxes, gt_boxes, *, positive_threshold: float,
                  negative_threshold: float, focal: bool = False, ablation_no_box_regression: bool = False,
                  regression_scaling_imgsize: bool = False, regression_scaling_WH_only: bool = False,
                  groups: Optional[Sequence[int]] = None):
        from . import gt_loss as gl

        os_ = list(o) if isinstance(o, (list, tuple)) else [o]
        bs_ = list(b) if isinstance(b, (list, tuple)) else [b] * len(os_)
        boxes = np.asarray(unit_boxes, np.float32).reshape(-1, 4)
        gtb = gl.host_boxes(gt_boxes)
        ces, gis, maps = [], [], []
        for lv, (ol, bl) in enumerate(zip(os_, bs_)):
            H, W = ol.shape[-2:]
            units = host.gt_units(boxes, unit_image, H, W, not ablation_no_box_regression,
                                  regression_scaling_imgsize, regression_scaling_WH_only)
            st = gl.assign(ol, None if ablation_no_box_regression else bl, units, gtb, positive_threshold,
                           negative_threshold, lv == len(os_) - 1, focal, with_loss=True)
            ce, gi = gl.group_losses(st.sums, st.counts, groups)
            ces.append(ce); gis.append(gi); maps.append(st.gt_map)
        return dict(loss_ce=torch.stack(ces).mean(0), loss_giou=torch.stack(gis).mean(0),
                    gt_map=maps if isinstance(o, (list, tuple)) else maps[0],
                    sums=st.sums, counts=st.counts, target=st.target)

    @staticmethod
    def nms(logits, box, ref, counts: torch.Tensor, counts_host: np.ndarray,
            unit_off: torch.Tensor, seg_units: np.ndarray, iou_threshold: float,
            want_keep: bool = False):
        dev = logits.device
        G = len(seg_units) - 1
        cand_off, nb_off, max_cand = host.nms_offsets(counts_host, seg_units)
        T = int(cand_off[-1])
        sum_nb = int(nb_off[-1])
        work = torch.empty(max(size("nms_work", T, sum_nb, max_cand, G), 1), device=dev,
                           dtype=torch.uint8)
        parts = [np.asarray(seg_units, np.int32), np.asarray(cand_off, np.int64), np.asarray(nb_off, np.int64)]
        if counts is None:
            parts.append(np.asarray(counts_host, np.int32))
        host_off = not isinstance(unit_off, torch.Tensor)
        if host_off:
            parts.append(np.asarray(unit_off, np.int64))
        offs, o = [], 0
        for a in parts:
            offs.append(o)
            o += (a.nbytes + 7) // 8 * 8
        blob = np.zeros(max(o, 8), np.uint8)
        for a, q in zip(parts, offs):
            blob[q:q + a.nbytes] = a.view(np.uint8)
        blob_d = _h2d(blob, dev)
        views = [blob_d[q:q + a.nbytes].view(torch.int32 if a.dtype == np.int32 else torch.int64)
                 for a, q in zip(parts, offs)]
        seg_d, coff_d, nboff_d = views[:3]
        rest = views[3:]
        if counts is None:
            counts = rest.pop(0)
        if host_off:
            unit_off = rest.pop(0)
        out_l = torch.empty((T, 2), device=dev, dtype=torch.float32)
        out_b = torch.empty((T, 4), device=dev, dtype=torch.float32)
        out_r = torch.empty((T, 2), device=dev, dtype=torch.float32)
        kept = torch.empty(G, device=dev, dtype=torch.int32)
        keep = torch.empty(T, device=dev, dtype=torch.int64) if want_keep else None
        call("tmr_nms", ptr(logits), ptr(box), ptr(ref), ptr(counts), ptr(unit_off), ptr(seg_d),
             ptr(coff_d), ptr(nboff_d), G, T, max_cand, sum_nb, float(iou_threshold), ptr(out_l), ptr(out_b),
             ptr(out_r), ptr(keep) if keep is not None else None, ptr(kept), ptr(work), stream())
        k = kept.cpu().numpy()
        L, Bx, R, K = [], [], [], []
        for g in range(G):
            s, e = int(cand_off[g]), int(cand_off[g]) + int(k[g])
            L.append(out_l[s:e]); Bx.append(out_b[s:e]); R.append(out_r[s:e])
            if keep is not None:
                K.append(keep[s:e])
        return (L, Bx, R, K) if want_keep else (L, Bx, R)

    use_graphs = True
    GRAPH_MAX_UNITS = 32
    GRAPH_CACHE = 8

    def _graph_signature(self, feats: torch.Tensor, units: np.ndarray, unit_image, ablation_b, ablation_c,
                         module: bool = False):
        if not (self.use_graphs and feats.is_cuda and len(unit_image) <= self.GRAPH_MAX_UNITS):
            return None
        if self.decoder_events is not None or self.xcorr_events is not None or \
                (self.reuse_image_work and not module):
            return None
        return (tuple(feats.shape), feats.dtype, str(feats.device), tuple(int(i) for i in unit_image),
                tuple(units["ht"].tolist()), tuple(units["wt"].tolist()), tuple(sorted(vars(self.cfg).items())),
                self.fold_proj, self.share_fp_half, self.xcorr_algo, self.out_bf16, TMREngine.exp_mode,
                bool(ablation_b), bool(ablation_c), self._param_key())

    def _param_key(self):
        P = self.P
        names = self._pnames
        if names is None or names[1] is not P or len(names[0]) != len(P):
            names = self._pnames = (tuple(sorted(P)), P)
        try:
            return tuple((k, P[k].data_ptr(), P[k]._version) for k in names[0])
        except KeyError:
            self._pnames = None
            return self._param_key()

    @staticmethod
    def _detect_host_inputs(units, unit_image, B, params, nms=None) -> Dict[str, np.ndarray]:
        d = {"units": units.view(np.uint8), "img_units": np.asarray(host.image_ranges(unit_image, B)),
             "unit_image": np.asarray(unit_image, np.int32), "unit_image64": np.asarray(unit_image, np.int64),
             "peak_params": params.view(np.uint8)}
        if nms is not None:
            d["nms_unit_off"], d["nms_seg"] = nms[:2]
        return d

    def _forward_peaks(self, feats, unit_image, boxes, params, nms=None):
        r = self.forward_units(feats, unit_image, boxes)
        logits, box, ref, counts, _ = self.peaks(r["o"], r["b"], params, want_prob=False)
        if nms is None:
            return logits, box, ref, counts
        unit_off, seg, iou = nms
        dev = logits.device
        G = len(seg) - 1
        uo = _h2d(unit_off, dev, tag="nms_unit_off")
        sg = _h2d(seg, dev, tag="nms_seg")
        out_l = torch.empty((G * NMS_SMALL, 2), device=dev, dtype=torch.float32)
        out_b = torch.empty((G * NMS_SMALL, 4), device=dev, dtype=torch.float32)
        out_r = torch.empty((G * NMS_SMALL, 2), device=dev, dtype=torch.float32)
        kept = torch.empty(G, device=dev, dtype=torch.int32)
        call("tmr_nms_small", ptr(logits), ptr(box), ptr(ref), ptr(counts), ptr(uo), ptr(sg), G, float(iou),
             ptr(out_l), ptr(out_b), ptr(out_r), None, ptr(kept), stream())
        return logits, box, ref, counts, torch.cat([counts, kept]), out_l, out_b, out_r

    def _detect_refined(self, feats, unit_image, boxes, params, shape, iou_threshold, refiner, image,
                        sam_features, refine_exemplars):
        from .tm_utils import NMS

        if image is None or sam_features is None:
            raise TMRError("detect(refiner=...) needs image and sam_features")
        B, E, cap = shape
        self.last_graph, self.last_nms_small = "eager", False
        if self.box_at_peaks_ok():
            logits, box, ref, _, counts_host = self._detect_box_at_peaks(feats, unit_image, boxes, params)
        else:
            self.last_box_route = None
            logits, box, ref, counts = self._forward_peaks(feats, unit_image, boxes, params)
            counts_host = counts.cpu().numpy()
        rows = np.maximum(counts_host, 1)
        L, Bx, R = [], [], []
        for i in range(B):
            us = range(i * E, (i + 1) * E)
            L.append(torch.cat([logits[u * cap:u * cap + int(rows[u])] for u in us]))
            Bx.append(torch.cat([box[u * cap:u * cap + int(rows[u])] for u in us]))
            R.append(torch.cat([ref[u * cap:u * cap + int(rows[u])] for u in us]))
        if refine_exemplars is not None:
            L, Bx, R = refiner.forward_refine(L, Bx, R, image, refine_exemplars, sam_features)
        else:
            L, Bx, R = refiner(L, Bx, R, image, sam_features)
        return NMS(L, Bx, R, iou_threshold)

    def detect(self, feats: torch.Tensor, exemplars, cls_ths: float, iou_threshold: float,
               ablation_b: bool = False, ablation_c: bool = False, refiner=None, image=None,
               sam_features=None, refine_exemplars=None):
        ex = exemplars.detach().cpu().numpy() if isinstance(exemplars, torch.Tensor) else \
            np.asarray(exemplars)
        ex = ex.astype(np.float32)
        B, E = ex.shape[:2]
        unit_image = np.repeat(np.arange(B), E)
        boxes = ex.reshape(B * E, 4)
        require_gpu(feats, "features")
        Hin, Win = feats.shape[-2:]
        H, W = (2 * Hin, 2 * Win) if self.cfg.feature_upsample else (Hin, Win)
        params = host.peak_params(boxes, H, W, cls_ths, self.cfg.box_reg, ablation_b, ablation_c)
        C = int(self.P["input_proj.0.weight"].shape[0])
        U = B * E
        unit_off = np.arange(U, dtype=np.int64) * (H * W)
        seg = np.arange(0, U + 1, E, dtype=np.int64)
        if refiner is not None:
            return self._detect_refined(feats, unit_image, boxes, params, (B, E, H * W), iou_threshold, refiner,
                                        image, sam_features, refine_exemplars)
        if not (self.use_graphs and U <= self.GRAPH_MAX_UNITS):
            self.last_graph, self.last_nms_small = "eager", False
            if self.box_at_peaks_ok():
                logits, box, ref, counts, counts_host = self._detect_box_at_peaks(feats, unit_image, boxes, params)
            else:
                self.last_box_route = None
                logits, box, ref, counts = self._forward_peaks(feats, unit_image, boxes, params)
                counts_host = counts.cpu().numpy()
            return self.nms(logits, box, ref, counts, counts_host, unit_off, seg, iou_threshold)
        spec = (unit_off, seg.astype(np.int32), iou_threshold)
        units = host.build_units(boxes, unit_image, H, W, C, self.cfg.template_type)[0] \
            if not self.cfg.no_matcher else np.zeros(0, UNIT_DTYPE)
        sig = self._graph_signature(feats, units, unit_image, ablation_b, ablation_c)
        if sig is not None:
            sig = sig + (float(iou_threshold),)
        g = self._graphs.get(sig) if sig is not None else None
        self.last_graph = "replay" if g is not None else "eager"
        if g is None and sig is not None and self._graphs.want_capture(sig):
            g = graphs.capture(self, feats, self._detect_host_inputs(units, unit_image, B, params, spec),
                               lambda static: self._forward_peaks(static, unit_image, boxes, params, spec))
            self._graphs.put(sig, g)
            if g is not None:
                self.last_graph = "captured"
        if g is not None:
            out = g.replay(self, feats.float().contiguous(), self._detect_host_inputs(units, unit_image, B, params, spec))
        else:
            self.last_box_route = None
            out = self._forward_peaks(feats, unit_image, boxes, params, spec)
        logits, box, ref, counts = out[:4]
        ck = out[4].cpu().numpy()
        counts_host, kept = ck[:U], ck[U:]
        self.last_nms_small = bool((kept >= 0).all())
        if not self.last_nms_small:
            return self.nms(logits, box, ref, counts, counts_host, unit_off, seg, iou_threshold)
        ol, ob, orf = (t.clone() for t in out[5:8]) if g is not None else out[5:8]
        s0 = [int(i) * NMS_SMALL for i in range(B)]
        return ([ol[a:a + int(k)] for a, k in zip(s0, kept)], [ob[a:a + int(k)] for a, k in zip(s0, kept)],
                [orf[a:a + int(k)] for a, k in zip(s0, kept)])
```

Baseline: 708.0 images/s.

## Compute box-branch shared feature half only at peak points via chained kernel

Adds a points-chain kernel that runs the shared fp-half conv and the per-unit half together, and only at the detected peak tiles for the box decoder tiles. The dense per-image store of the fp-half for those box output tiles is deferred and skipped when the chain is cheaper. A host cost model picks the route: it compares points times ns-per-point against pixels times ns-per-pixel, applies a MAC floor, and remembers shapes where the chain lost. This removes dense shared-conv work for the box channels but adds a host decision, more kernel complexity and a fallback late store when the chain loses.

```diff
diff --git a/include/tmr.h b/include/tmr.h
--- a/include/tmr.h
+++ b/include/tmr.h
@@ -132,6 +132,7 @@
                           const float *bias, int N, int leaky, const float *headw, const float *head_bias,
                           const float *acc_init, const float *box, const int32_t *tiles, int ntiles, float *b,
                           int flags, void *stream);
+
 
 int tmr_maxpool3x3(const float *x, int64_t planes, int H, int W, int mask9, float *out, void *stream);
 
diff --git a/include/tmr_points_chain.h b/include/tmr_points_chain.h
--- /dev/null
+++ b/include/tmr_points_chain.h
@@ -0,0 +1,21 @@
+#ifndef TMR_POINTS_CHAIN_H
+#define TMR_POINTS_CHAIN_H
+
+#include "tmr.h"
+
+#ifdef __cplusplus
+extern "C" {
+#endif
+
+int tmr_split_conv_points_chain(const void *xp0, int C0, const float *xmax0, const void *wpack_fp,
+                                const float *wmax_fp, const float *bias_plane, const int32_t *unit_image,
+                                const void *xp1, int C1, const float *xmax1, const void *wpack, const float *wmax,
+                                int U, int H, int W, int ks, int prec, const float *bias, int N, int leaky,
+                                const float *headw, const float *head_bias, const float *box,
+                                const int32_t *tiles, int ntiles, float *b, int flags, void *stream);
+
+#ifdef __cplusplus
+}
+#endif
+
+#endif
diff --git a/profiles/kernel_resources.py b/profiles/kernel_resources.py
--- a/profiles/kernel_resources.py
+++ b/profiles/kernel_resources.py
@@ -38,7 +38,11 @@
         return subprocess.run(cmd, check=True, capture_output=True, text=True).stderr
 
 
-def parse(text):
+CHAIN = "split_points_chain_kernel"
+OUT_CHAIN = os.path.join(REPO, "profiles", "points_kloop", "resources_chain.json")
+
+
+def parse(text, kernel="split_points_kernel"):
     out, cur = {}, None
     for line in text.splitlines():
         m = re.search(r"remark: +([^:]+): (.*?) \[-Rpass-analysis", line)
@@ -46,22 +50,31 @@
             continue
         key, val = m.group(1).strip(), m.group(2).strip()
         if key == "Function Name":
-            k = re.search(r"split_points_kernelILi3ELi(\d)EE", val)
-            cur = out.setdefault(PRECS[int(k.group(1))], {}) if k else None
+            if kernel == CHAIN:
+                cur = out.setdefault("F16X3", {}) if re.search(CHAIN + r"ILi3EE", val) else None
+            else:
+                k = re.search(r"split_points_kernelILi3ELi(\d)EE", val)
+                cur = out.setdefault(PRECS[int(k.group(1))], {}) if k else None
         elif cur is not None and key in FIELDS:
             cur[FIELDS[key]] = int(val)
     return out
 
 
 def main():
-    out_path = sys.argv[1] if len(sys.argv) > 1 else OUT
+    argv = sys.argv[1:]
+    chain = argv[:2] == ["--kernel", CHAIN]
+    if chain:
+        argv = argv[2:]
+    out_path = argv[0] if argv else OUT_CHAIN if chain else OUT
     hipcc, flags = makefile_flags()
-    kernels = parse(remarks(hipcc, flags))
-    assert sorted(kernels) == sorted(PRECS.values()), kernels
+    kernels = parse(remarks(hipcc, flags), CHAIN if chain else "split_points_kernel")
+    assert sorted(kernels) == (["F16X3"] if chain else sorted(PRECS.values())), kernels
     load_package()
     from tmr_amd import buildinfo
-    rec = {"kernel": "split_points_kernel<3, PREC>", "flags": flags, "source_digest": buildinfo.source_digest("heads"),
-           "kernels": kernels, "parent": PARENT}
+    rec = {"kernel": "split_points_chain_kernel<3>" if chain else "split_points_kernel<3, PREC>", "flags": flags,
+           "source_digest": buildinfo.source_digest("heads"), "kernels": kernels}
+    if not chain:
+        rec["parent"] = PARENT
     os.makedirs(os.path.dirname(out_path), exist_ok=True)
     with open(out_path, "w") as f:
         json.dump(rec, f, indent=1)
diff --git a/profiles/points_crossover.py b/profiles/points_crossover.py
--- a/profiles/points_crossover.py
+++ b/profiles/points_crossover.py
@@ -61,7 +61,96 @@
     return out
 
 
+CHAIN_CONFIGS = {"B": bench.CONFIGS["B"], "D2": dict(bench.CONFIGS["D"], E=2), "E": bench.CONFIGS["E"]}
+FLOOR_BATCHES = (1, 2, 4, 8, 16, 32, 64)
+
+
+def _chain_engine(cfg, B, mode):
+    dev = torch.device("cuda", 0)
+    H = W = 2 * cfg["hf"]
+    eng = tmr.TMREngine(synth.reference_state_dict(0, device=dev), tmr.PathConfig())
+    eng.use_graphs = False
+    eng.box_at_peaks = "always"
+    eng.box_fp_at_points = mode
+    feats = torch.from_numpy(synth.sam_features(1000, B, bench.CIN, H // 2, W // 2)).to(dev)
+    ex, _ = synth.exemplar_set(2000, B, cfg["E"], H, W, cfg["kmin"], cfg["kmax"])
+    return eng, (lambda: eng.detect(feats, ex, cls_ths=cfg["cls"], iou_threshold=cfg["iou"])), H, W
+
+
+def measure_chain(name):
+    from tmr_amd.decoder_plan import fp_late_bound_macs
+    cfg = CHAIN_CONFIGS[name]
+    B = cfg["batch"]
+    eng, detect, H, W = _chain_engine(cfg, B, "always")
+    detect()
+    rec = {}
+    chain, points, store = eng.box_chain_at_points, eng.box_at_points, eng.box_late_store
+
+    def all_three(box, tiles):
+        rec["chain_ms_all"] = events(lambda: chain(box, tiles))
+        rec["store_ms_all"] = events(store)
+        rec["points_ms_all"] = events(lambda: points(box, tiles))
+        rec["tiles"] = len(tiles)
+        rec["nbt"] = eng._box_ctx.plan.skip_tiles
+
+    eng.box_chain_at_points = all_three
+    detect()
+    torch.cuda.synchronize()
+    assert eng.last_box_route == "points_chain" and "tiles" in rec
+    n, pixels = eng.last_points, B * H * W
+    cm, sm, pm = (min(rec[k]) for k in ("chain_ms_all", "store_ms_all", "points_ms_all"))
+    c_chain, c_store = (cm - pm) * 1e6 / n, sm * 1e6 / pixels
+    return dict(points=n, image_pixels=pixels, fraction_of_unit_pixels=n / (pixels * cfg["E"]), tiles=rec["tiles"],
+                chain_ms=cm, store_ms=sm, points_ms=pm, c_chain_ns_per_point=c_chain, c_store_ns_per_pixel=c_store,
+                rule_takes_chain=bool(n * c_chain < pixels * c_store), saving_ms=sm - (cm - pm),
+                bound_macs=fp_late_bound_macs(B, H, W, rec["nbt"], bench.CIN, 3),
+                **{k: rec[k] for k in rec if k.endswith("_all")})
+
+
+def measure_floor():
+    from tmr_amd.decoder_plan import fp_late_bound_macs
+    cfg, rows = bench.CONFIGS["B"], []
+    for B in FLOOR_BATCHES:
+        row = dict(batch=B)
+        for mode in ("never", "always"):
+            eng, detect, H, W = _chain_engine(cfg, B, mode)
+            detect()
+            detect()
+            torch.cuda.synchronize()
+            row[mode + "_ms_all"] = t = events(detect, reps=5)
+            row[mode + "_route"] = eng.last_box_route
+            row[mode + "_ms"] = float(np.median(t))
+        row["bound_macs"] = fp_late_bound_macs(B, H, W, 8, bench.CIN, 3)
+        row["gain_ms"] = row["never_ms"] - row["always_ms"]
+        row["spread_ms"] = max(max(row[m + "_ms_all"]) - min(row[m + "_ms_all"]) for m in ("never", "always"))
+        row["wins"] = bool(row["gain_ms"] > 3 * row["spread_ms"])
+        rows.append(row)
+        print("floor", json.dumps({k: row[k] for k in ("batch", "never_ms", "always_ms", "spread_ms", "wins")}),
+              flush=True)
+    floor = None
+    for i in range(len(rows) - 1, -1, -1):
+        if not rows[i]["wins"]:
+            break
+        floor = rows[i]["bound_macs"]
+    return dict(rows=rows, floor_macs=floor)
+
+
+def main_chain(out_path):
+    res = {"configs": {}}
+    for c in CHAIN_CONFIGS:
+        res["configs"][c] = r = measure_chain(c)
+        print(c, json.dumps({k: r[k] for k in ("points", "chain_ms", "store_ms", "points_ms", "c_chain_ns_per_point",
+                                               "c_store_ns_per_pixel", "rule_takes_chain")}), flush=True)
+        with open(out_path, "w") as f:
+            json.dump(res, f, indent=1)
+    res["floor"] = measure_floor()
+    with open(out_path, "w") as f:
+        json.dump(res, f, indent=1)
+
+
 def main():
+    if sys.argv[1] == "--chain":
+        return main_chain(sys.argv[2])
     out_path = sys.argv[1]
     res = {}
     for c in sys.argv[2:] or ["B", "C", "D", "E"]:
diff --git a/template-matching-and-regression-mapreduce_amd/_lib.py b/template-matching-and-regression-mapreduce_amd/_lib.py
--- a/template-matching-and-regression-mapreduce_amd/_lib.py
+++ b/template-matching-and-regression-mapreduce_amd/_lib.py
@@ -216,6 +216,13 @@
     return N * ((P + TWOWAY_POOL_CHUNK - 1) // TWOWAY_POOL_CHUNK) * TWOWAY_ROWS * (TWOWAY_DIM + 2) * 4
 
 
+POINTS_CHAIN_HEADER = os.path.join(os.path.dirname(_HERE), "include", "tmr_points_chain.h")
+POINTS_CHAIN_SIGNATURES = {
+    "tmr_split_conv_points_chain": (_I, [_P, _I, _P, _P, _P, _P, _P, _P, _I, _P, _P, _P, _I, _I, _I, _I, _I, _P, _I,
+                                         _I, _P, _P, _P, _P, _I, _P, _I, _P]),
+}
+
+
 class TMRError(RuntimeError):
     pass
 
@@ -234,7 +241,7 @@
         lib = ctypes.CDLL(LIB_PATH)
         for name, (res, args) in (list(SIGNATURES.items()) + list(EXT_SIGNATURES.items())
                                   + list(COCO_SIGNATURES.items()) + list(MASKHEAD_SIGNATURES.items())
-                                  + list(TWOWAY_SIGNATURES.items())):
+                                  + list(TWOWAY_SIGNATURES.items()) + list(POINTS_CHAIN_SIGNATURES.items())):
             fn = getattr(lib, name)
             fn.restype = res
             fn.argtypes = args
diff --git a/template-matching-and-regression-mapreduce_amd/csrc/conv_split.hip b/template-matching-and-regression-mapreduce_amd/csrc/conv_split.hip
--- a/template-matching-and-regression-mapreduce_amd/csrc/conv_split.hip
+++ b/template-matching-and-regression-mapreduce_amd/csrc/conv_split.hip
@@ -2,6 +2,8 @@
 #include <type_traits>
 
 #include "tmr_common.h"
+
+#include "../../include/tmr_points_chain.h"
 
 namespace {
 
@@ -668,8 +670,13 @@
     float *b;
 };
 
-template <int KS, int PREC>
-__global__ __launch_bounds__(NTHREADS) void split_points_kernel(PArgs pa) {
+struct CArgs {
+    const char *wp_fp;
+    const float *wmax_fp, *xmax0;
+};
+
+template <int KS, int PREC, bool CHAIN>
+__device__ __forceinline__ void points_body(const PArgs &pa, const CArgs &ca) {
     typedef Prec<PREC> PR;
     typedef typename PR::V V;
     constexpr int T = KS * KS, HALVES = PR::HALVES, WREC = PR::WREC;
@@ -691,6 +698,7 @@
     const int HW = a.H * a.W;
     int tu[2], tfirst[2], tcnt[2], timg[2];
     float sxw[2];
+    float sx0[2];
 #pragma unroll
     for (int hh = 0; hh < 2; ++hh) {
         const int64_t ti = 2 * (int64_t)blockIdx.x + hh;
@@ -702,8 +710,11 @@
         timg[hh] = __builtin_amdgcn_readfirstlane(a.unit_image ? a.unit_image[tu[hh]] : tu[hh]);
         sxw[hh] = __builtin_bit_cast(
             float, __builtin_amdgcn_readfirstlane(__builtin_bit_cast(int, split_sxw<PREC>(a, tu[hh]))));
-    }
-    const int NC = a.NC0 + a.NC1, NHC = NC * HALVES;
+        sx0[hh] = !CHAIN ? 1.0f : __builtin_bit_cast(
+            float, __builtin_amdgcn_readfirstlane(__builtin_bit_cast(
+                       int, split_scale(ca.xmax0 + timg[hh]) * split_scale(ca.wmax_fp))));
+    }
+    int NC = a.NC0 + a.NC1, NHC = NC * HALVES;
     auto pixel = [&](int u, int first, int cnt, int p) {
         const int *pixi = reinterpret_cast<const int *>(pa.box) + 4 * (size_t)u * HW;
         return min(max(pixi[4 * (size_t)min(first + (p < cnt ? p : 0), HW - 1)], 0), HW - 1);
@@ -720,9 +731,18 @@
     };
     const char *xb0 = uniform_ptr(h0 ? a.x0 + (size_t)gimg * h0 * cstride : a.x1);
     const char *xb1 = uniform_ptr(h1 ? a.x1 + (size_t)gu * h1 * cstride : a.x0);
-    const uint32_t tapstride = (uint32_t)NC * a.Npad * WREC;
-    const __amdgpu_buffer_rsrc_t wr = __builtin_amdgcn_make_buffer_rsrc(
+    uint32_t tapstride = (uint32_t)NC * a.Npad * WREC;
+    __amdgpu_buffer_rsrc_t wr = __builtin_amdgcn_make_buffer_rsrc(
         (void *)a.wp, (short)0, T * tapstride, 0x00020000);
+    int p0 = h0, p1 = h1;
+    auto set_phase = [&](int ph) {
+        NC = ph ? a.NC1 : a.NC0;
+        NHC = NC * HALVES;
+        p0 = ph ? 0 : h0;
+        p1 = ph ? h1 : 0;
+        tapstride = (uint32_t)NC * a.Npad * WREC;
+        wr = __builtin_amdgcn_make_buffer_rsrc((void *)(ph ? a.wp : ca.wp_fp), (short)0, T * tapstride, 0x00020000);
+    };
     const int gpix0 = pixel(gu, gfirst, gcnt, lane);
     uint32_t goff[KS];
 #pragma unroll
@@ -734,10 +754,10 @@
     const uint32_t qstride = (uint32_t)a.Hp * a.Wp * 16;
     auto gather = [&](int hc, bool live = true) {
         const int hcl = min(hc, NHC - 1);
-        const bool s0 = hcl < h0;
-        const uint32_t hs_ = (uint32_t)(s0 ? hcl : hcl - h0) * cstride + wt * qstride;
+        const bool s0 = hcl < p0;
+        const uint32_t hs_ = (uint32_t)(s0 ? hcl : hcl - p0) * cstride + wt * qstride;
         const __amdgpu_buffer_rsrc_t xr = __builtin_amdgcn_make_buffer_rsrc(
-            (void *)(s0 ? xb0 : xb1), (short)0, live ? (s0 ? h0 : h1) * cstride : 0, 0x00020000);
+            (void *)(s0 ? xb0 : xb1), (short)0, live ? (s0 ? p0 : p1) * cstride : 0, 0x00020000);
 #pragma unroll
         for (int ky = 0; ky < KS; ++ky)
 #pragma unroll
@@ -758,67 +778,7 @@
         const int nt = a.NT0 + (active ? wtile : 0);
         const int lp = lane_now(), l16p = lp & 15, kgp = lp >> 4;
         uint32_t aoff = (uint32_t)kgp * a.Npad * 16 + ((uint32_t)nt * BM + wh * (BM / 2) + l16p) * 16;
-        gather(0);
-
         f32x4 acc[NF][PCG];
-        if (a.acc_init) {
-            constexpr int HJ = PCG / 2;
-            int Wd = a.W, fl = a.flags;
-            asm volatile("" : "+s"(Wd), "+s"(fl));
-            const int ppix[2] = {pixel(tu[0], tfirst[0], tcnt[0], lp), pixel(tu[1], tfirst[1], tcnt[1], lp)};
-            auto group4 = [&](int j) {
-                const int hh = j / HJ;
-                const int pix = lane_read(ppix[hh], (j % HJ) * 16 + l16p);
-                const int py = pix / Wd, px = pix - py * Wd;
-                const int islab = (fl & TMR_SPLIT_INIT_BCAST) ? 0 : timg[hh];
-                const int mt = (py / TH) * a.TXN + px / TW;
-                const int wpix = (py % TH) >> 2, jp = ((py & 3) << 1) | ((px % TW) >> 4);
-                static_assert(ACCW / 4 == 1 << 11 && 8 * 64 <= ACCW / 4, "the shifts below");
-                const uint32_t row = (uint32_t)(mt * NWAVES + wpix * WNS + wh), in = jp * 64 + kgp * 16 + (px & 15);
-                typedef uint32_t u2 __attribute__((ext_vector_type(2)));
-                u2 lh = {row << 11 | in, row >> 21};
-                asm volatile("" : "+v"(lh));
-                return ((size_t)islab * a.NT + nt) * a.MT * NWAVES * (ACCW / 4) + __builtin_bit_cast(uint64_t, lh);
-            };
-            if (fl & TMR_SPLIT_INIT_BF16) {
-#pragma unroll
-                for (int j = 0; j < PCG; ++j) {
-                    const b4 *ai = reinterpret_cast<const b4 *>(a.acc_init) + group4(j);
-#pragma unroll
-                    for (int f = 0; f < NF; ++f) {
-                        const f2 raw = __builtin_bit_cast(f2, ai[f * 8 * 64]);
-                        acc[f][j] = (f32x4){raw.x, raw.y, 0.0f, 0.0f};
-                    }
-                    __builtin_amdgcn_sched_barrier(0);
-                }
-#pragma unroll
-                for (int j = 0; j < PCG; ++j)
-#pragma unroll
-                    for (int f = 0; f < NF; ++f)
-                        acc[f][j] = __builtin_convertvector(__builtin_bit_cast(b4, (f2){acc[f][j][0], acc[f][j][1]}),
-                                                            f32x4) * sxw[j / HJ];
-            } else {
-#pragma unroll
-                for (int j = 0; j < PCG; ++j) {
-                    const f32x4 *ai = reinterpret_cast<const f32x4 *>(a.acc_init) + group4(j);
-#pragma unroll
-                    for (int f = 0; f < NF; ++f) acc[f][j] = ai[f * 8 * 64];
-                    __builtin_amdgcn_sched_barrier(0);
-                }
-#pragma unroll
-                for (int j = 0; j < PCG; ++j)
-#pragma unroll
-                    for (int f = 0; f < NF; ++f) acc[f][j] = acc[f][j] * sxw[j / HJ];
-            }
-        } else {
-            float zf = 0.0f;
-            asm volatile("" : "+v"(zf));
-#pragma unroll
-            for (int f = 0; f < NF; ++f)
-#pragma unroll
-                for (int j = 0; j < PCG; ++j) acc[f][j] = (f32x4){zf, zf, zf, zf};
-        }
-
         auto st_part = [](int s) { return HALVES == 2 && s >= 2 * T ? 1 : 0; };
         auto st_tap = [](int s) { return HALVES == 2 ? (s >= 2 * T ? s - 2 * T : s / 2) : s; };
         auto st_term = [](int s) { return HALVES == 2 && s < 2 * T ? s & 1 : 0; };
@@ -839,43 +799,123 @@
 #pragma unroll
             for (int f = 0; f < NF; ++f) ar[s % AR][f] = buffer_load16<V>(wr, aoff + f * 256, as);
         };
-#pragma unroll
-        for (int s = 0; s < AR - 1; ++s) load_stage(0, s);
-        asm volatile("s_waitcnt vmcnt(0)" ::: "memory");
-        __syncthreads();
         constexpr int BW = HALVES == 2 ? PCG : PCG / 2;
         static_assert(PCG % BW == 0, "a group's slot is j % BW in every stage");
         V bc[BW];
-        for (int c = 0; c < NC; ++c) {
-            asm volatile("" : "+v"(aoff));
-            asm volatile("" : "+s"(ts), "+s"(npl));
-#pragma unroll
-            for (int s = 0; s < NS; ++s) {
-                const int hc = c * HALVES + st_part(s);
-                load_stage(c, s + AR - 1);
-                if (st_first(s)) {
-                    gather(hc + 1, hc + 1 < NHC);
-#pragma unroll
-                    for (int j = 0; j < BW; ++j) bc[j] = bfrag(hc, st_tap(s), j);
-                }
-                __builtin_amdgcn_sched_barrier(0);
-#pragma unroll
-                for (int j = 0; j < PCG; ++j) {
-#pragma unroll
-                    for (int f = 0; f < NF; ++f) acc[f][j] = mma(ar[s % AR][f], bc[j % BW], acc[f][j]);
-                    if (j + BW < PCG) {
-                        bc[j % BW] = bfrag(hc, st_tap(s), j + BW);
-                        __builtin_amdgcn_sched_barrier(0);
-                    } else if (!st_last(s) && (BW < PCG || st_newb(s + 1))) {
-                        bc[j % BW] = bfrag(hc, st_tap(s + 1), j + BW - PCG);
+#pragma unroll
+        for (int ph = CHAIN ? 0 : 1; ph < 2; ++ph) {
+            if constexpr (CHAIN) {
+                set_phase(ph);
+                ts = tapstride;
+            }
+            gather(0);
+
+            if (CHAIN && ph) {
+                float i0[2], s1[2] = {sxw[0], sxw[1]};
+#pragma unroll
+                for (int hh = 0; hh < 2; ++hh)
+                    i0[hh] = __builtin_bit_cast(
+                        float, __builtin_amdgcn_readfirstlane(__builtin_bit_cast(int, 1.0f / sx0[hh])));
+#pragma unroll
+                for (int j = 0; j < PCG; ++j)
+#pragma unroll
+                    for (int f = 0; f < NF; ++f) acc[f][j] = acc[f][j] * i0[j / (PCG / 2)];
+#pragma unroll
+                for (int j = 0; j < PCG; ++j)
+#pragma unroll
+                    for (int f = 0; f < NF; ++f) acc[f][j] = acc[f][j] * s1[j / (PCG / 2)];
+            } else if (a.acc_init) {
+                constexpr int HJ = PCG / 2;
+                int Wd = a.W, fl = a.flags;
+                asm volatile("" : "+s"(Wd), "+s"(fl));
+                const int ppix[2] = {pixel(tu[0], tfirst[0], tcnt[0], lp), pixel(tu[1], tfirst[1], tcnt[1], lp)};
+                auto group4 = [&](int j) {
+                    const int hh = j / HJ;
+                    const int pix = lane_read(ppix[hh], (j % HJ) * 16 + l16p);
+                    const int py = pix / Wd, px = pix - py * Wd;
+                    const int islab = (fl & TMR_SPLIT_INIT_BCAST) ? 0 : timg[hh];
+                    const int mt = (py / TH) * a.TXN + px / TW;
+                    const int wpix = (py % TH) >> 2, jp = ((py & 3) << 1) | ((px % TW) >> 4);
+                    static_assert(ACCW / 4 == 1 << 11 && 8 * 64 <= ACCW / 4, "the shifts below");
+                    const uint32_t row = (uint32_t)(mt * NWAVES + wpix * WNS + wh), in = jp * 64 + kgp * 16 + (px & 15);
+                    typedef uint32_t u2 __attribute__((ext_vector_type(2)));
+                    u2 lh = {row << 11 | in, row >> 21};
+                    asm volatile("" : "+v"(lh));
+                    return ((size_t)islab * a.NT + nt) * a.MT * NWAVES * (ACCW / 4) + __builtin_bit_cast(uint64_t, lh);
+                };
+                if (fl & TMR_SPLIT_INIT_BF16) {
+#pragma unroll
+                    for (int j = 0; j < PCG; ++j) {
+                        const b4 *ai = reinterpret_cast<const b4 *>(a.acc_init) + group4(j);
+#pragma unroll
+                        for (int f = 0; f < NF; ++f) {
+                            const f2 raw = __builtin_bit_cast(f2, ai[f * 8 * 64]);
+                            acc[f][j] = (f32x4){raw.x, raw.y, 0.0f, 0.0f};
+                        }
                         __builtin_amdgcn_sched_barrier(0);
                     }
+#pragma unroll
+                    for (int j = 0; j < PCG; ++j)
+#pragma unroll
+                        for (int f = 0; f < NF; ++f)
+                            acc[f][j] = __builtin_convertvector(__builtin_bit_cast(b4, (f2){acc[f][j][0], acc[f][j][1]}),
+                                                                f32x4) * (CHAIN ? sx0[j / HJ] : sxw[j / HJ]);
+                } else {
+#pragma unroll
+                    for (int j = 0; j < PCG; ++j) {
+                        const f32x4 *ai = reinterpret_cast<const f32x4 *>(a.acc_init) + group4(j);
+#pragma unroll
+                        for (int f = 0; f < NF; ++f) acc[f][j] = ai[f * 8 * 64];
+                        __builtin_amdgcn_sched_barrier(0);
+                    }
+#pragma unroll
+                    for (int j = 0; j < PCG; ++j)
+#pragma unroll
+                        for (int f = 0; f < NF; ++f) acc[f][j] = acc[f][j] * (CHAIN ? sx0[j / HJ] : sxw[j / HJ]);
                 }
-                __builtin_amdgcn_sched_barrier(0);
-                if (st_last(s)) {
-                    static_assert((AR - 1) * NF == 8 && T > AR - 1, "the counted wait below");
-                    asm volatile("s_waitcnt vmcnt(8)" ::: "memory");
-                    __syncthreads();
+            } else {
+                float zf = 0.0f;
+                asm volatile("" : "+v"(zf));
+#pragma unroll
+                for (int f = 0; f < NF; ++f)
+#pragma unroll
+                    for (int j = 0; j < PCG; ++j) acc[f][j] = (f32x4){zf, zf, zf, zf};
+            }
+#pragma unroll
+            for (int s = 0; s < AR - 1; ++s) load_stage(0, s);
+            asm volatile("s_waitcnt vmcnt(0)" ::: "memory");
+            __syncthreads();
+            for (int c = 0; c < NC; ++c) {
+                asm volatile("" : "+v"(aoff));
+                asm volatile("" : "+s"(ts), "+s"(npl));
+#pragma unroll
+                for (int s = 0; s < NS; ++s) {
+                    const int hc = c * HALVES + st_part(s);
+                    load_stage(c, s + AR - 1);
+                    if (st_first(s)) {
+                        gather(hc + 1, hc + 1 < NHC);
+#pragma unroll
+                        for (int j = 0; j < BW; ++j) bc[j] = bfrag(hc, st_tap(s), j);
+                    }
+                    __builtin_amdgcn_sched_barrier(0);
+#pragma unroll
+                    for (int j = 0; j < PCG; ++j) {
+#pragma unroll
+                        for (int f = 0; f < NF; ++f) acc[f][j] = mma(ar[s % AR][f], bc[j % BW], acc[f][j]);
+                        if (j + BW < PCG) {
+                            bc[j % BW] = bfrag(hc, st_tap(s), j + BW);
+                            __builtin_amdgcn_sched_barrier(0);
+                        } else if (!st_last(s) && (BW < PCG || st_newb(s + 1))) {
+                            bc[j % BW] = bfrag(hc, st_tap(s + 1), j + BW - PCG);
+                            __builtin_amdgcn_sched_barrier(0);
+                        }
+                    }
+                    __builtin_amdgcn_sched_barrier(0);
+                    if (st_last(s)) {
+                        static_assert((AR - 1) * NF == 8 && T > AR - 1, "the counted wait below");
+                        asm volatile("s_waitcnt vmcnt(8)" ::: "memory");
+                        __syncthreads();
+                    }
                 }
             }
         }
@@ -968,13 +1008,34 @@
     }
 }
 
+template <int KS, int PREC>
+__global__ __launch_bounds__(NTHREADS) void split_points_kernel(PArgs pa) {
+    points_body<KS, PREC, false>(pa, CArgs{});
+}
+
+template <int KS>
+__global__ __launch_bounds__(NTHREADS) void split_points_chain_kernel(PArgs pa, CArgs ca) {
+    points_body<KS, TMR_PREC_F16X3, true>(pa, ca);
+}
+
+constexpr size_t POINTS_LDS = 2 * 9 * P * PP * 16 + NWAVES * 4 * PP * sizeof(float);
+static_assert(POINTS_LDS <= LDS_KB * 1024, "LDS");
+
 template <int PREC>
 int launch_points(const PArgs &pa, int ntiles, hipStream_t s) {
-    constexpr size_t lds = 2 * 9 * P * PP * 16 + NWAVES * 4 * PP * sizeof(float);
-    static_assert(lds <= LDS_KB * 1024, "LDS");
+    constexpr size_t lds = POINTS_LDS;
     auto kern = split_points_kernel<3, PREC>;
     if (tmr_set_max_lds((const void *)kern, lds) != hipSuccess) return TMR_E_HIP;
     hipLaunchKernelGGL(kern, dim3((unsigned)((ntiles + 1) / 2)), dim3(NTHREADS), lds, s, pa);
+    TMR_CHECK_LAUNCH();
+    return TMR_OK;
+}
+
+int launch_points_chain(const PArgs &pa, const CArgs &ca, int ntiles, hipStream_t s) {
+    constexpr size_t lds = POINTS_LDS;
+    auto kern = split_points_chain_kernel<3>;
+    if (tmr_set_max_lds((const void *)kern, lds) != hipSuccess) return TMR_E_HIP;
+    hipLaunchKernelGGL(kern, dim3((unsigned)((ntiles + 1) / 2)), dim3(NTHREADS), lds, s, pa, ca);
     TMR_CHECK_LAUNCH();
     return TMR_OK;
 }
@@ -1526,3 +1587,54 @@
         default: return launch_points<TMR_PREC_F16>(pa, ntiles, s);
     }
 }
+
+extern "C" int tmr_split_conv_points_chain(const void *xp0, int C0, const float *xmax0, const void *wpack_fp,
+                                           const float *wmax_fp, const float *bias_plane,
+                                           const int32_t *unit_image, const void *xp1, int C1, const float *xmax1,
+                                           const void *wpack, const float *wmax, int U, int H, int W, int ks,
+                                           int prec, const float *bias, int N, int leaky, const float *headw,
+                                           const float *head_bias, const float *box, const int32_t *tiles,
+                                           int ntiles, float *b, int flags, void *stream) {
+    TMR_REQUIRE(prec_ok(prec) && ks_ok(ks));
+    TMR_REQUIRE(xp0 && xmax0 && wpack_fp && wmax_fp && unit_image && xp1 && xmax1 && wpack && wmax);
+    TMR_REQUIRE(bias && headw && head_bias && box && b && U > 0 && H > 0 && W > 0 && N > 0 && C0 > 0 && C1 > 0);
+    TMR_REQUIRE(ntiles >= 0 && (ntiles == 0 || tiles));
+    TMR_REQUIRE((flags & 0xffff) == 0);
+    TMR_REQUIRE((int64_t)H * W < (1ll << 29));
+    PArgs pa = {};
+    SArgs &a = pa.s;
+    a.x0 = static_cast<const char *>(xp0);
+    a.x1 = static_cast<const char *>(xp1);
+    a.unit_image = unit_image;
+    a.wp = static_cast<const char *>(wpack);
+    a.wmax = wmax;
+    a.xmax = xmax1;
+    a.bias = bias;
+    a.headw = headw;
+    a.acc_init = bias_plane;
+    a.NC0 = (int)tmr_cdiv(C0, CCH);
+    a.NC1 = (int)tmr_cdiv(C1, CCH);
+    a.U = U;
+    a.H = H;
+    a.W = W;
+    a.N = N;
+    a.NT = (int)tmr_cdiv(N, BM);
+    a.Npad = a.NT * BM;
+    a.TXN = (int)tmr_cdiv(W, TW);
+    a.MT = a.TXN * (int)tmr_cdiv(H, TH);
+    a.Hp = pad_h(H, ks);
+    a.Wp = pad_w(W, ks);
+    a.leaky = leaky;
+    a.flags = TMR_SPLIT_XMAX_PER_UNIT | (bias_plane ? TMR_SPLIT_TILED_INIT | TMR_SPLIT_INIT_BCAST : 0);
+    a.EI = 1;
+    TMR_REQUIRE(tile_window(flags, a.NT, a.NT0, a.NTW));
+    if (prec != TMR_PREC_F16X3 || ks != 3 || a.NTW > 2 * PTW) return TMR_E_UNSUPPORTED;
+    pa.head_bias = head_bias;
+    pa.box = box;
+    pa.tiles = tiles;
+    pa.ntiles = ntiles;
+    pa.b = b;
+    CArgs ca = {static_cast<const char *>(wpack_fp), wmax_fp, xmax0};
+    if (ntiles == 0) return TMR_OK;
+    return launch_points_chain(pa, ca, ntiles, tmr_stream(stream));
+}
diff --git a/template-matching-and-regression-mapreduce_amd/decoder_plan.py b/template-matching-and-regression-mapreduce_amd/decoder_plan.py
--- a/template-matching-and-regression-mapreduce_amd/decoder_plan.py
+++ b/template-matching-and-regression-mapreduce_amd/decoder_plan.py
@@ -37,6 +37,7 @@
     init_flags: int
     epi: int
     skip_tiles: int
+    fp_late: bool = False
 
     def window(self, ntiles: int) -> Tuple[int, int]:
         return (self.skip_tiles, ntiles - self.skip_tiles) if self.skip_tiles else (0, 0)
@@ -47,9 +48,17 @@
     def points_flags(self) -> int:
         return self.init_flags | split_tile_window(0, self.skip_tiles)
 
+    def fp_window(self, ntiles: int, late: bool = False) -> Tuple[int, int]:
+        if not self.fp_late:
+            return (0, 0)
+        return (0, self.skip_tiles) if late else (self.skip_tiles, ntiles - self.skip_tiles)
+
+    def fp_store_flags(self, ntiles: int, late: bool = False) -> int:
+        return self.fp_flags | split_tile_window(*self.fp_window(ntiles, late))
+
 
 def decoder_plan(cfg, fold_proj: bool, share_fp_half: bool, reuse_image_work: bool, have_feats: bool, U: int,
-                 B: int, unit_image, box_later: bool = False, nbt: int = 0) -> DecoderPlan:
+                 B: int, unit_image, box_later: bool = False, nbt: int = 0, fp_late: bool = False) -> DecoderPlan:
     fold = bool(cfg.fusion and fold_proj and have_feats)
     share = bool(share_fp_half and cfg.fusion and (U >= 2 * B or (reuse_image_work and fold)))
     bf16 = cfg.precision == "bf16"
@@ -63,7 +72,12 @@
         fp_flags, init = 0, plane
     return DecoderPlan(fold, share, acc16, bf16, SCALES_OWN if share else SCALES_MERGED if cfg.fusion else SCALES_FTM,
                        fp_flags, init | xpu, units_per_image(unit_image, B) << SPLIT_UNITS_PER_IMAGE_SHIFT,
-                       nbt if box_later else 0)
+                       nbt if box_later else 0,
+                       bool(fp_late and box_later and nbt > 0 and share and fold and cfg.precision == "fp32"))
+
+
+def fp_late_bound_macs(B: int, H: int, W: int, nbt: int, C0: int, ks: int) -> int:
+    return B * H * W * 128 * nbt * C0 * ks * ks
 
 
 @dataclass
@@ -88,6 +102,7 @@
     part: torch.Tensor
     plan: DecoderPlan
     b: Optional[torch.Tensor] = None
+    fp: Optional["FpHalf"] = None
 
     def _conv_args(self):
         return (ptr(self.xp0) if self.C0 else None, self.C0, ptr(self.ui), ptr(self.xp1), self.C1, self.U, self.H,
@@ -101,3 +116,32 @@
     def run_points(self, box: torch.Tensor, tiles: torch.Tensor, ntiles: int) -> None:
         call("tmr_split_conv_points", *self._conv_args(), ptr(self.hb), ptr(self.a0), ptr(box), ptr(tiles), ntiles,
              ptr(self.b), self.plan.points_flags(), stream())
+
+    def run_points_chain(self, box: torch.Tensor, tiles: torch.Tensor, ntiles: int) -> None:
+        f = self.fp
+        call("tmr_split_conv_points_chain", ptr(f.xp0), f.C0, ptr(f.xmax0), ptr(f.wp[0]), ptr(f.wp[1]),
+             ptr(f.bplane), ptr(self.ui), ptr(self.xp1), self.C1, ptr(self.xmax1), ptr(self.wp[0]), ptr(self.wp[1]),
+             self.U, self.H, self.W, self.ks, self.pc, ptr(self.bias), self.N, 1, ptr(self.hw), ptr(self.hb), ptr(box),
+             ptr(tiles), ntiles, ptr(self.b), split_tile_window(0, self.plan.skip_tiles), stream())
+
+
+@dataclass
+class FpHalf:
+    xp0: torch.Tensor
+    C0: int
+    B: int
+    H: int
+    W: int
+    ks: int
+    pc: int
+    wp: tuple
+    xmax0: Optional[torch.Tensor]
+    zero_b: torch.Tensor
+    N: int
+    bplane: Optional[torch.Tensor]
+    acc0: torch.Tensor
+
+    def run(self, flags: int) -> None:
+        call("tmr_split_conv", ptr(self.xp0), self.C0, None, None, 0, self.B, self.H, self.W, self.ks, self.pc,
+             ptr(self.wp[0]), ptr(self.wp[1]), ptr(self.xmax0), ptr(self.zero_b), self.N, 0, None, ptr(self.bplane),
+             ptr(self.acc0), flags, stream())
diff --git a/template-matching-and-regression-mapreduce_amd/engine.py b/template-matching-and-regression-mapreduce_amd/engine.py
--- a/template-matching-and-regression-mapreduce_amd/engine.py
+++ b/template-matching-and-regression-mapreduce_amd/engine.py
@@ -12,7 +12,7 @@
 from ._lib import (PEAKS_DECODE_ONLY, PEAKS_FIND_ONLY, PEAKS_PROB_SCRATCH, POINTS_TILE, PREC_CODES, SPLIT_OUT_BF16,
                    SPLIT_TILED_OUT, SPLIT_XMAX_PER_PIXEL, UNIT_DTYPE, XCORR_ALGOS, TMRError, call, ptr, require_gpu,
                    size, stream, xcorr)
-from .decoder_plan import SCALES_FTM, SCALES_MERGED, HeadsLaunch, decoder_plan
+from .decoder_plan import SCALES_FTM, SCALES_MERGED, FpHalf, HeadsLaunch, decoder_plan, fp_late_bound_macs
 from .graphs import _clone_outputs, _GraphBook, _h2d, _units_to_device
 from .operands import absmax
 from .operands import (absmax_rows, conv2d_split, fold_proj, pack_split_up, pack_split_w, pack_split_x, pixel_absmax,
@@ -121,6 +121,7 @@
         self.last_points = 0
         self.last_points_flops = 0.0
         self._box_ctx: Optional[HeadsLaunch] = None
+        self._fp_late_lost: Dict[tuple, bool] = {}
         if cfg.decoder_kernel_size not in (1, 3, 5, 7):
             raise TMRError("decoder_kernel_size must be 1, 3, 5 or 7")
 
@@ -305,8 +306,10 @@
         U, C1, H, W = f_tm.shape
         B, dev = fp.shape[0], f_tm.device
         ks, prec, pc = cfg.decoder_kernel_size, cfg.precision, prec_code(cfg.precision)
+        nbt = self._box_tiles() if box_later else 0
         p = decoder_plan(cfg, self.fold_proj, self.share_fp_half, self.reuse_image_work, feats is not None, U, B,
-                         unit_image, box_later, self._box_tiles() if box_later else 0)
+                         unit_image, box_later, nbt, box_later and feats is not None and
+                         self._fp_at_points_wanted(B, H, W, nbt, feats.shape[1], ks, U))
         Cfp = fp.shape[1] if cfg.fusion else 0
         wp, bias, N, Cw, hw, hb, split, wbias = self._fused_decoders(Cfp if p.share else 0, p.fold)
         if Cw != Cfp + C1:
@@ -325,24 +328,26 @@
                 xp0 = pack_split_up(feats, cfg.feature_upsample, ks, prec, xmax0, ones=False) if p.fold else \
                     pack_split_x(fp, ks, prec, xmax0)
         xp1 = pack_split_x(f_tm, ks, prec, xmax1)
+        fph, ntiles = None, (N + 127) // 128
         if p.share:
             wp_fp, wp, zero_b = split
             if acc0 is None:
                 acc0 = torch.empty(size("acc", B, N, H, W), device=dev, dtype=torch.float32)
-                call("tmr_split_conv", ptr(xp0), C0, None, None, 0, B, H, W, ks, pc, ptr(wp_fp[0]), ptr(wp_fp[1]),
-                     ptr(xmax0), ptr(zero_b), N, 0, None, ptr(bplane), ptr(acc0), p.fp_flags, stream())
+                fph = FpHalf(xp0, C0, B, H, W, ks, pc, wp_fp, xmax0, zero_b, N, bplane, acc0)
+                fph.run(p.fp_store_flags(ntiles))
                 if p.fold and self.reuse_image_work:
                     self._acc0_store(feats, split, H, W, acc0)
         part = torch.empty(size("heads_partials", N, U, H, W), device=dev, dtype=torch.float32)
         heads = HeadsLaunch(xp0=None if p.share else xp0, C0=0 if p.share else C0, ui=ui, xp1=xp1, C1=C1, U=U, H=H, W=W,
                             ks=ks, pc=pc, wp=wp, xmax1=xmax1, bias=bias, N=N, hw=hw, hb=hb,
-                            a0=acc0 if p.share else bplane, part=part, plan=p)
-        first, count = p.window((N + 127) // 128)
+                            a0=acc0 if p.share else bplane, part=part, plan=p, fp=fph if p.fp_late else None)
+        first, count = p.window(ntiles)
         with _timed(self.decoder_events):
             heads.run(first, count)
         n_run = 128 * count if box_later else N
         self.last_decoder_flops = 2.0 * H * W * n_run * (heads.C0 + C1) * ks ** 2 * U
-        self.last_shared_flops = 2.0 * H * W * N * C0 * ks ** 2 * B if p.share else 0.0
+        n_fp = N - 128 * nbt if p.fp_late else N
+        self.last_shared_flops = 2.0 * H * W * n_fp * C0 * ks ** 2 * B if p.share else 0.0
         self.last_decoder_algo = "split"
         ob = torch.empty(U * (5 if cfg.box_reg else 1) * H * W, device=dev, dtype=torch.float32)
         o = ob[:U * H * W].view(U, 1, H, W)
@@ -374,6 +379,27 @@
     box_at_peaks = "auto"
     BOX_POINTS_CROSSOVER = {"fp32": 0.57, "bf16": 0.47, "f16": 0.47}
 
+    box_fp_at_points = "auto"
+    FP_CHAIN_NS_PER_POINT = 12.0
+    FP_STORE_NS_PER_PIXEL = 9.3
+    FP_AT_POINTS_FLOOR_MACS = 6.1e11
+
+    def _fp_at_points_wanted(self, B: int, H: int, W: int, nbt: int, C0: int, ks: int, U: int = 0) -> bool:
+        mode = self.box_fp_at_points
+        if mode not in ("auto", "always", "never"):
+            raise TMRError("box_fp_at_points must be 'auto', 'always' or 'never'")
+        return mode == "always" or \
+            (mode == "auto" and fp_late_bound_macs(B, H, W, nbt, C0, ks) >= self.FP_AT_POINTS_FLOOR_MACS and
+             not self._fp_late_lost.get((B, U, H, W), False))
+
+    def _fp_chain_wins(self, points: int, B: int, H: int, W: int) -> bool:
+        return points * self.FP_CHAIN_NS_PER_POINT < B * H * W * self.FP_STORE_NS_PER_PIXEL
+
+    def _fp_late_note(self, B: int, U: int, H: int, W: int, wins: bool) -> None:
+        if len(self._fp_late_lost) >= 64:
+            self._fp_late_lost.clear()
+        self._fp_late_lost[(B, U, H, W)] = not wins
+
     def _box_tiles(self) -> int:
         return int(self.P["decoder_b.layer.0.weight"].shape[0]) // 128
 
@@ -391,6 +417,15 @@
         if len(tiles):
             td = _h2d(np.ascontiguousarray(tiles, np.int32).reshape(-1), box.device)
             self._box_ctx.run_points(box, td, len(tiles))
+
+    def box_chain_at_points(self, box: torch.Tensor, tiles: np.ndarray) -> None:
+        if len(tiles):
+            td = _h2d(np.ascontiguousarray(tiles, np.int32).reshape(-1), box.device)
+            self._box_ctx.run_points_chain(box, td, len(tiles))
+
+    def box_late_store(self) -> None:
+        h = self._box_ctx
+        h.fp.run(h.plan.fp_store_flags((h.N + 127) // 128, late=True))
 
     def box_dense(self) -> None:
         h = self._box_ctx
@@ -410,15 +445,25 @@
         self.last_points = int(need.sum())
         dense = self.box_at_peaks == "auto" and \
             self.last_points > self.BOX_POINTS_CROSSOVER[self.cfg.precision] * U * H * W
-        self.last_box_route = "dense" if dense else "points"
+        h = self._box_ctx
+        nbt = h.plan.skip_tiles
+        nimg = feats.shape[0]
+        wins = not dense and self._fp_chain_wins(self.last_points, nimg, H, W)
+        if self.box_fp_at_points == "auto":
+            self._fp_late_note(nimg, U, H, W, wins)
+        chain = h.plan.fp_late and not dense and (self.box_fp_at_points == "always" or wins)
+        self.last_box_route = "dense" if dense else "points_chain" if chain else "points"
+        if h.plan.fp_late and not chain:
+            self.box_late_store()
+            self.last_shared_flops += 2.0 * H * W * 128 * nbt * h.fp.C0 * h.ks ** 2 * h.fp.B
         if dense:
             self.box_dense()
             self.last_points_flops = 0.0
         else:
             tiles = host.point_tiles(need, POINTS_TILE)
-            self.box_at_points(box, tiles)
-            h = self._box_ctx
-            self.last_points_flops = 2.0 * 128 * h.plan.skip_tiles * (h.C0 + h.C1) * h.ks ** 2 * POINTS_TILE * len(tiles)
+            (self.box_chain_at_points if chain else self.box_at_points)(box, tiles)
+            cin = (h.fp.C0 if chain else h.C0) + h.C1
+            self.last_points_flops = 2.0 * 128 * nbt * cin * h.ks ** 2 * POINTS_TILE * len(tiles)
         self._box_ctx = None
         self.peaks(o, b, params, want_prob=False, phase="decode", found=(logits, box, ref, counts))
         return logits, box, ref, counts, counts_host
```

Result: faster. 777.3 images/s, median of 6 (+9.8%).
